# JohnVinyard/music-synthesis

Hardware: AMD Instinct MI355X
Metric: GAN train-step audio samples/sec (22.05 kHz, 8192-sample window) (higher is better)
Workload: dtype f32 storage and accumulate; multiplies on the 16-bit matrix pipe with split fp32 operands: block-scaled fp16 x 2 (22 significand bits, 3 products per multiply) in the atoms, the k5 layer, the grouped convs, the stride-8 transposed forward and the atom weight gradients; exact bf16 x 3 (6 products) or; 1 GPU; stage-2 GAN train step: alternating D/G trainer calls, MelGAN generator + 3-scale discriminator + feature-matching loss (BASELINE.json configs[2]); per_gpu_batch=32, global_batch=32, window=8192, mels=80, optimizer=FlatAdam(1e-4,(0.5,0.9)), parallelism=dp1, hipgraph=True

## Files before the change

### include/msynth.h

```cpp
#ifndef MSYNTH_H
#define MSYNTH_H

#include <stddef.h>
#include <stdint.h>

#ifdef __cplusplus
extern "C" {
#endif

#define MSYNTH_VERSION 200

typedef void* ms_stream_t;

enum ms_status {
    MS_OK = 0,
    MS_ERR_INVALID_ARG = -1,
    MS_ERR_UNSUPPORTED = -2,
    MS_ERR_WORKSPACE = -3,
    MS_ERR_LAUNCH = -4,
    MS_ERR_COMM = -5
};

enum ms_act { MS_ACT_NONE = 0, MS_ACT_LRELU = 1, MS_ACT_TANH = 2 };
enum ms_pad_mode { MS_PAD_ZERO = 0, MS_PAD_REFLECT = 1 };

int ms_version(void);
const char* ms_status_string(int status);

typedef struct ms_conv1d_desc {
    int32_t B, Cin, Lin, Cout, K, stride, pad, dil, groups;
    int32_t pad_mode;
    int32_t act;
    float slope;
    int32_t in_act;
} ms_conv1d_desc;

int ms_conv1d_out_len(const ms_conv1d_desc* d);

int ms_conv1d_fwd(const ms_conv1d_desc* d, const float* x, const float* w, const float* bias,
                  const float* residual, float* y, float* y_act, void* workspace,
                  size_t workspace_bytes, ms_stream_t stream);

int ms_conv1d_bwd_data(const ms_conv1d_desc* d, const float* gy, const float* y_act,
                       const float* w, const float* gx_add, float* gx, void* workspace,
                       size_t workspace_bytes, ms_stream_t stream);

int ms_conv1d_bwd_weight(const ms_conv1d_desc* d, const float* x, const float* gy,
                         const float* y_act, float* gw, float* gb, float beta, void* workspace,
                         size_t workspace_bytes, ms_stream_t stream);

#define MS_CONV_PARTS_MAX 3
typedef struct ms_conv1d_parts {
    int32_t count;
    int32_t reserved;
    int32_t B[MS_CONV_PARTS_MAX];
    int32_t Lin[MS_CONV_PARTS_MAX];
    const float* x[MS_CONV_PARTS_MAX];
    float* y[MS_CONV_PARTS_MAX];
    const float* gy[MS_CONV_PARTS_MAX];
    const float* y_act[MS_CONV_PARTS_MAX];
    const float* gx_add[MS_CONV_PARTS_MAX];
    float* gx[MS_CONV_PARTS_MAX];
} ms_conv1d_parts;
int ms_conv1d_parts_launches(const ms_conv1d_desc* d, const ms_conv1d_parts* parts, int which, int with_image);
size_t ms_conv1d_parts_workspace_bytes(const ms_conv1d_desc* d, const ms_conv1d_parts* parts, int which, int with_image);
int ms_conv1d_parts_fwd(const ms_conv1d_desc* d, const ms_conv1d_parts* parts, const float* w, const float* bias,
                        const void* image, void* workspace, size_t workspace_bytes, ms_stream_t stream);
int ms_conv1d_parts_bwd_data(const ms_conv1d_desc* d, const ms_conv1d_parts* parts, const float* w, const void* image_bwd,
                             void* workspace, size_t workspace_bytes, ms_stream_t stream);
int ms_conv1d_parts_bwd_weight(const ms_conv1d_desc* d, const ms_conv1d_parts* parts, float* gw, float* gb, float beta,
                               void* workspace, size_t workspace_bytes, ms_stream_t stream);

#define MS_WGRAD_MULTI_MAX 8
typedef struct ms_wgrad_multi_desc {
    int32_t count;
    int32_t reserved;
    ms_conv1d_desc conv[MS_WGRAD_MULTI_MAX];
    const float* x[MS_WGRAD_MULTI_MAX];
    const float* gy[MS_WGRAD_MULTI_MAX];
    const float* y_act[MS_WGRAD_MULTI_MAX];
    float* gw[MS_WGRAD_MULTI_MAX];
    float* gb[MS_WGRAD_MULTI_MAX];
    float beta[MS_WGRAD_MULTI_MAX];
    const float* xmax[MS_WGRAD_MULTI_MAX];
    const float* gmax[MS_WGRAD_MULTI_MAX];
    const uint16_t* y_signs[MS_WGRAD_MULTI_MAX];
} ms_wgrad_multi_desc;
size_t ms_conv1d_bwd_weight_multi_workspace_bytes(const ms_wgrad_multi_desc* d);
int ms_conv1d_bwd_weight_multi(const ms_wgrad_multi_desc* d, void* workspace, size_t workspace_bytes,
                               ms_stream_t stream);

typedef struct ms_atom_desc {
    int32_t B, C, L, dil;
    float slope;
} ms_atom_desc;
#define MS_ATOM_PACK_MAX 16
typedef struct ms_atom_pack_desc {
    int32_t count;
    int32_t reserved;
    int32_t C[MS_ATOM_PACK_MAX];
    const float* w0[MS_ATOM_PACK_MAX];
    const float* w1[MS_ATOM_PACK_MAX];
    void* image[MS_ATOM_PACK_MAX];
    int32_t backward[MS_ATOM_PACK_MAX];
} ms_atom_pack_desc;
size_t ms_residual_atom_image_bytes(int32_t C);
int ms_residual_atom_supported(const ms_atom_desc* d);
int ms_residual_atom_pack_multi(const ms_atom_pack_desc* d, ms_stream_t stream);
#define MS_ATOM_AMAX_N 1024
int ms_residual_atom_publishes_amax(void);
int ms_residual_atom_fwd(const ms_atom_desc* d, const float* x, const void* image, const float* b0, const float* b1,
                         float* y, float* t, float* y_act, float* amax, ms_stream_t stream);
int ms_residual_atom_bwd_supported(const ms_atom_desc* d);
int ms_residual_atom_bwd_data(const ms_atom_desc* d, const float* gy, const float* y_act, const float* t,
                              const void* image_bwd, float* gt, float* gx, float* amax, ms_stream_t stream);
// ... 225 lines not shown
```

### music-synthesis_amd/csrc/api.hip

```cpp
#include "ms_common.h"
#include <stdarg.h>
#include <stdio.h>
#include <stdlib.h>
#include <string.h>
#include <execinfo.h>
#include <signal.h>
#include <unistd.h>
#include "conv_mfma.h"
#include "gconv_mfma.h"
#include "conv_thin.h"

static thread_local int g_prof_on = 0, g_prof_launches = 0, g_prof_products = 0;
static thread_local double g_prof_us = 0.0;
static thread_local char g_prof_kernel[MS_PROFILE_NAME_MAX] = "";

void ms_note_kernel(int products, const char* fmt, ...) {
    if (!g_prof_on) return;
    va_list ap;
    va_start(ap, fmt);
    vsnprintf(g_prof_kernel, sizeof(g_prof_kernel), fmt, ap);
    va_end(ap);
    g_prof_products = products;
}

bool ms_name_or_note(char* name, int products, const char* fmt, ...) {
    if (!name && !g_prof_on) return false;
    va_list ap;
    va_start(ap, fmt);
    vsnprintf(name ? name : g_prof_kernel, MS_PROFILE_NAME_MAX, fmt, ap);
    va_end(ap);
    if (!name) g_prof_products = products;
    return name != nullptr;
}

bool ms_prof_on() { return g_prof_on != 0; }

void ms_prof_add(hipEvent_t e0, hipEvent_t e1) {
    float ms = 0.f;
    if (e0 && e1 && hipEventSynchronize(e1) == hipSuccess && hipEventElapsedTime(&ms, e0, e1) == hipSuccess) {
        g_prof_us += 1e3 * (double)ms;
        ++g_prof_launches;
    }
    if (e0) (void)hipEventDestroy(e0);
    if (e1) (void)hipEventDestroy(e1);
}

namespace {

bool make_conv(const ms_conv1d_desc* d, ConvP* p) {
    if (!d) return false;
    if (d->B <= 0 || d->Cin <= 0 || d->Lin <= 0 || d->Cout <= 0 || d->K <= 0 || d->stride <= 0 ||
        d->pad < 0 || d->dil <= 0 || d->groups <= 0)
        return false;
    if (d->Cin % d->groups || d->Cout % d->groups) return false;
    if (d->pad_mode != MS_PAD_ZERO && d->pad_mode != MS_PAD_REFLECT) return false;
    if (d->pad_mode == MS_PAD_REFLECT && d->pad >= d->Lin) return false;
    if (d->act < MS_ACT_NONE || d->act > MS_ACT_TANH) return false;
    const int eff = d->Lin + 2 * d->pad - d->dil * (d->K - 1) - 1;
    if (eff < 0) return false;
    p->B = d->B; p->Cin = d->Cin; p->Lin = d->Lin; p->Cout = d->Cout; p->K = d->K;
    p->stride = d->stride; p->pad = d->pad; p->dil = d->dil; p->groups = d->groups;
    p->Cg = d->Cin / d->groups; p->Og = d->Cout / d->groups;
// ... 275 lines not shown
            q.act = p.act;
            return pl.add(TD_CONV_MFMA, q, ws);
        }
        return pl.add(TD_CONV_DIRECT, q);
    }
    const size_t tail = msk_channel_sum_ws(p.Cin) + 32;
    if (mst_convt1_applicable(p)) pl.add(TW_THIN, p, mst_convt1_wgrad_ws(p) + tail, SHORT_WS);
    if (mswt8_applicable(p)) pl.add(TW_8, p, mswt8_ws(p) + tail, SHORT_WS | UNSUPPORTED);
    if (mswt2s_applicable(p)) pl.add(TW_2S, p, mswt2s_ws(p) + tail, SHORT_WS | UNSUPPORTED);
    if (msm_convt_bwd_applicable(p)) return pl.add(TW_MFMA, p, msm_convt_bwd_weight_ws(p) + tail);
    if (msm_bwd_weight_applicable(p)) return pl.add(TW_CONV_MFMA, p, msm_bwd_weight_ws(p) + tail);
    return pl.add(TW_CONV_DIRECT, p, msk_conv1d_bwd_weight_ws(p) + tail);
}

bool parts_ok(const ms_conv1d_desc* d, const ms_conv1d_parts* parts, ConvP* c) {
    if (!d || !parts || parts->count < 1 || parts->count > MS_CONV_PARTS_MAX) return false;
    ms_conv1d_desc d0 = *d;
    for (int i = 0; i < parts->count; ++i) {
        d0.B = parts->B[i]; d0.Lin = parts->Lin[i];
        ConvP p;
        if (!make_conv(&d0, &p)) return false;
        if (i == 0) *c = p;
    }
    return true;
}

ms_conv1d_desc part_desc(const ms_conv1d_desc* d, const ms_conv1d_parts* parts, int i) {
    ms_conv1d_desc di = *d;
    di.B = parts->B[i]; di.Lin = parts->Lin[i];
    return di;
}

Plan parts_plan(const ms_conv1d_desc* d, const ConvP& c, const ms_conv1d_parts* parts, int which, bool w, bool image) {
    Plan pl;
    if (parts->count >= 2 && !c.in_act) {
        if (w && msd_parts_applicable(c, parts, which))
            return pl.add(P_DISC, c, which == 2 ? msd_parts_bwd_weight_ws(c, parts) : 0);
        if (w && msg4_parts_applicable(c, parts)) return pl.add(P_G4, c);
        if (which == 2 && msw5_parts_applicable(c, parts)) return pl.add(P_K5, c, msw5_parts_ws(c, parts));
        if (which < 2 && image && ms5_parts_applicable(c, parts, which == 1))
            return pl.add(P_K5_IMG, c, ms5_parts_ws(c, parts, which == 1));
        if (which == 0 && w && msg3_parts_fwd_applicable(c, parts)) return pl.add(P_G3, c);
        if (which == 1 && w && msg3_parts_bwd_data_applicable(c, parts)) return pl.add(P_G3, c);
        if (which == 2 && msg3_parts_bwd_weight_applicable(c, parts)) return pl.add(P_G3, c, msg3_parts_bwd_weight_ws(c, parts));
    }
    size_t n = 0;
    for (int i = 0; i < parts->count; ++i) {
        const ms_conv1d_desc di = part_desc(d, parts, i);
        const size_t m = image && which < 2 && ms_conv1d_img_bytes(&di) ? ms_conv1d_img_workspace_bytes(&di, which)
                                                                        : ms_conv1d_workspace_bytes(&di, which);
        if (m > n) n = m;
    }
    return pl.add(P_EACH, c, n);
}

const char* route_name(Kind k, const ConvP& g) {
    switch (k) {
        case F_THIN_SHORT: case F_THIN: return mst_fwd_name(g);
        case F_SMALL: return mss_conv_name(g);
        case F_PAD4: case F_MFMA: return msm_fwd_name(g);
        case TD_CONV_MFMA: { ConvP c = g; c.act = MS_ACT_NONE; return msm_fwd_name(c, g.act); }
        case F_G4: return msg4_parts_name(0);
        case F_G3: return msg3_fwd_name(g);
        case F_G: return msg_fwd_name(g);
        case F_DIRECT: case TD_CONV_DIRECT: return msk_conv1d_fwd_direct_name(g);
        case D_PAD4: case D_MFMA: return msm_bwd_data_name(g);
        case D_G4: return msg4_parts_name(1);
        case D_G3: return msg3_bwd_data_name(g);
        case D_G: return msg_bwd_data_name(g);
        case D_THIN: return mst_bwd_data_name(g);
        case D_DIRECT: case TF_DIRECT: return msk_conv1d_bwd_data_direct_name(g);
        case W_THIN: return mst_bwd_weight_name(g);
        case W_SHORT: return msws_name(g);
        case W_32: return msw32_name(g);
        case W_K5: return msw5_name(g);
        case W_ROWS: return msw_bwd_weight_name(g);
        case W_MFMA: case TW_CONV_MFMA: return msm_bwd_weight_name(g);
        case W_G4: return msg4_parts_name(2);
        case W_G3: return msg3_bwd_weight_name(g);
        case W_G: return msg_bwd_weight_name(g);
        case W_DIRECT: case TW_CONV_DIRECT: return msk_conv1d_bwd_weight_direct_name(g);
        case TF_THIN: return mst_convt1_fwd_name();
        case TF_LANES: return mss_convt_name(g.stride);
        case TF_MFMA: return msm_convt_fwd_name(g);
        case TD_MFMA: return msm_convt_bwd_data_name(g);
        case TW_THIN: return mst_convt1_wgrad_name();
        case TW_8: return mswt8_name(g);
        case TW_2S: return mswt2s_name(g);
        case TW_MFMA: return msm_convt_bwd_weight_name(g);
        default: return "";
    }
}

template <class Launch>
int run(const Plan& pl, const void* ws, size_t ws_bytes, Launch launch) {
    for (int i = 0; i < pl.n; ++i) {
        const Route& r = pl.r[i];
        if ((r.declines & SHORT_WS) && (!ws || ws_bytes < r.ws)) continue;
        if ((r.declines & ALIGNED_WS) && (((uintptr_t)ws) & 15)) continue;
        if (ms_prof_on()) ms_note_kernel(0, "%s", route_name(r.kind, r.g));
        const int rc = launch(r.kind, r.g);
        if (rc != MS_ERR_UNSUPPORTED || !(r.declines & UNSUPPORTED)) return rc;
    }
    return MS_ERR_UNSUPPORTED;
}

// ... 68 lines not shown
    });
    if (rc != MS_OK || p.pad_mode != MS_PAD_REFLECT) return rc;
    p.pad_mode = MS_PAD_ZERO;
    return msk_reflect_fold_bwd(p, gy, y_act, w, gx, s);
}

int ms_conv1d_bwd_weight(const ms_conv1d_desc* d, const float* x, const float* gy,
                         const float* y_act, float* gw, float* gb, float beta, void* workspace,
                         size_t workspace_bytes, ms_stream_t stream) {
    ConvP p;
    if (!make_conv(d, &p) || !x || !gy || !gw) return MS_ERR_INVALID_ARG;
    if (beta != 0.f && beta != 1.f) return MS_ERR_INVALID_ARG;
    hipStream_t s = (hipStream_t)stream;
    const float* xa = p.in_act ? x : nullptr;
    const int xk = p.in_act ? MS_MOD_LRELU_FWD : 0;
    return run(conv_plan(p, 2, false, false), workspace, workspace_bytes, [&](Kind k, const ConvP& g) {
        switch (k) {
            case W_THIN: return mst_conv1d_bwd_weight(g, x, gy, y_act, gw, gb, beta, workspace, workspace_bytes, s);
            case W_SHORT: return msws_bwd_weight(g, x, gy, y_act, gw, gb, beta, workspace, workspace_bytes, s);
            case W_32: return msw32_bwd_weight(g, x, gy, y_act, gw, gb, beta, workspace, workspace_bytes, s);
            case W_K5: return msw5_bwd_weight(g, x, gy, y_act, gw, gb, beta, workspace, workspace_bytes, s);
            case W_ROWS: return msw_conv1d_bwd_weight(g, x, gy, y_act, gw, gb, beta, workspace, workspace_bytes, s);
            case W_MFMA:
                return msm_conv1d_bwd_weight(g, x, xa, xk, gy, y_act, g.act, gw, gb, beta, workspace, workspace_bytes, s);
            case W_G4: {
                const ms_conv1d_parts q = one_part(g, x, nullptr, gy, y_act);
                return msg4_parts_bwd_weight(g, &q, gw, gb, beta, s);
            }
            case W_G3: return msg3_conv1d_bwd_weight(g, x, gy, y_act, gw, gb, beta, workspace, workspace_bytes, s);
            case W_G: return msg_conv1d_bwd_weight(g, x, gy, y_act, gw, gb, beta, workspace, workspace_bytes, s);
            default:
                return msk_conv1d_bwd_weight_direct(g, x, xa, xk, gy, y_act, g.act, gw, gb, beta, workspace, workspace_bytes, s);
        }
    });
}

size_t ms_conv1d_workspace_bytes(const ms_conv1d_desc* d, int which) {
    ConvP p;
    if (!make_conv(d, &p) || which < 0 || which > 2) return 0;
    const size_t a = conv_plan(p, which, false, false).ws(), b = conv_plan(p, which, true, true).ws();
    return a > b ? a : b;
}

const char* ms_conv1d_kernel_name(const ms_conv1d_desc* d, int which) {
    ConvP p;
    if (!make_conv(d, &p) || which < 0 || which > 2) return "";
    const Plan pl = conv_plan(p, which, false, false);
    return pl.n ? route_name(pl.r[0].kind, pl.r[0].g) : "";
}

int ms_conv1d_parts_launches(const ms_conv1d_desc* d, const ms_conv1d_parts* parts, int which, int with_image) {
    ConvP c;
    if (!parts_ok(d, parts, &c) || which < 0 || which > 2) return MS_ERR_INVALID_ARG;
    return parts_plan(d, c, parts, which, true, with_image != 0).r[0].kind == P_EACH ? parts->count : 1;
}

size_t ms_conv1d_parts_workspace_bytes(const ms_conv1d_desc* d, const ms_conv1d_parts* parts, int which, int with_image) {
    ConvP c;
    if (!parts_ok(d, parts, &c) || which < 0 || which > 2) return 0;
    return parts_plan(d, c, parts, which, true, with_image != 0).ws();
}

int ms_conv1d_parts_fwd(const ms_conv1d_desc* d, const ms_conv1d_parts* parts, const float* w, const float* bias,
                        const void* image, void* workspace, size_t workspace_bytes, ms_stream_t stream) {
    ConvP c;
    if (!parts_ok(d, parts, &c) || (!w && !image)) return MS_ERR_INVALID_ARG;
    hipStream_t s = (hipStream_t)stream;
    return run(parts_plan(d, c, parts, 0, w, image), workspace, workspace_bytes, [&](Kind k, const ConvP&) {
        switch (k) {
            case P_DISC: return msd_parts_fwd(c, parts, w, bias, s);
            case P_G4: return msg4_parts_fwd(c, parts, w, bias, s);
            case P_K5_IMG: return ms5_parts_fwd(c, parts, image, bias, workspace, workspace_bytes, s);
            case P_G3: return msg3_parts_fwd(c, parts, w, bias, s);
            default: break;
        }
        for (int i = 0; i < parts->count; ++i) {
            const ms_conv1d_desc di = part_desc(d, parts, i);
            int rc = MS_ERR_UNSUPPORTED;
            if (image && ms_conv1d_img_bytes(&di))
                rc = ms_conv1d_img_fwd(&di, parts->x[i], image, bias, parts->y[i], workspace, workspace_bytes, stream);
            else if (w)
                rc = ms_conv1d_fwd(&di, parts->x[i], w, bias, nullptr, parts->y[i], nullptr, workspace, workspace_bytes, stream);
            if (rc != MS_OK) return rc;
        }
        return (int)MS_OK;
    });
}

int ms_conv1d_parts_bwd_data(const ms_conv1d_desc* d, const ms_conv1d_parts* parts, const float* w, const void* image_bwd,
                             void* workspace, size_t workspace_bytes, ms_stream_t stream) {
    ConvP c;
    if (!parts_ok(d, parts, &c) || (!w && !image_bwd)) return MS_ERR_INVALID_ARG;
    hipStream_t s = (hipStream_t)stream;
    return run(parts_plan(d, c, parts, 1, w, image_bwd), workspace, workspace_bytes, [&](Kind k, const ConvP&) {
        switch (k) {
            case P_DISC: return msd_parts_bwd_data(c, parts, w, s);
            case P_G4: return msg4_parts_bwd_data(c, parts, w, s);
            case P_K5_IMG: return ms5_parts_bwd_data(c, parts, image_bwd, workspace, workspace_bytes, s);
            case P_G3: return msg3_parts_bwd_data(c, parts, w, s);
            default: break;
        }
        for (int i = 0; i < parts->count; ++i) {
            const ms_conv1d_desc di = part_desc(d, parts, i);
            const float* ya = d->act == MS_ACT_NONE ? nullptr : parts->y_act[i];
            int rc = MS_ERR_UNSUPPORTED;
            if (image_bwd && ms_conv1d_img_bytes(&di))
                rc = ms_conv1d_img_bwd_data(&di, parts->gy[i], ya, image_bwd, parts->gx_add[i], parts->gx[i], workspace,
                                            workspace_bytes, stream);
            else if (w)
                rc = ms_conv1d_bwd_data(&di, parts->gy[i], ya, w, parts->gx_add[i], parts->gx[i], workspace, workspace_bytes,
                                        stream);
            if (rc != MS_OK) return rc;
        }
        return (int)MS_OK;
    });
}

int ms_conv1d_parts_bwd_weight(const ms_conv1d_desc* d, const ms_conv1d_parts* parts, float* gw, float* gb, float beta,
                               void* workspace, size_t workspace_bytes, ms_stream_t stream) {
    ConvP c;
    if (!parts_ok(d, parts, &c) || !gw || (beta != 0.f && beta != 1.f)) return MS_ERR_INVALID_ARG;
    hipStream_t s = (hipStream_t)stream;
    return run(parts_plan(d, c, parts, 2, true, false), workspace, workspace_bytes, [&](Kind k, const ConvP&) {
        switch (k) {
            case P_DISC: return msd_parts_bwd_weight(c, parts, gw, gb, beta, workspace, workspace_bytes, s);
            case P_G4: return msg4_parts_bwd_weight(c, parts, gw, gb, beta, s);
            case P_K5: return msw5_parts_bwd_weight(c, parts, gw, gb, beta, workspace, workspace_bytes, s);
            case P_G3: return msg3_parts_bwd_weight(c, parts, gw, gb, beta, workspace, workspace_bytes, s);
            default: break;
        }
        for (int i = 0; i < parts->count; ++i) {
            const ms_conv1d_desc di = part_desc(d, parts, i);
            const float* ya = d->act == MS_ACT_NONE ? nullptr : parts->y_act[i];
            const int rc = ms_conv1d_bwd_weight(&di, parts->x[i], parts->gy[i], ya, gw, gb, i == 0 ? beta : 1.f, workspace,
                                                workspace_bytes, stream);
            if (rc != MS_OK) return rc;
        }
        return (int)MS_OK;
    });
}

static int multi_convs(const ms_wgrad_multi_desc* d, ConvP* cs) {
    if (!d || d->count <= 0 || d->count > MS_WGRAD_MULTI_MAX) return 0;
    for (int i = 0; i < d->count; ++i)
        if (!make_conv(&d->conv[i], &cs[i])) return 0;
    return d->count;
}

size_t ms_conv1d_bwd_weight_multi_workspace_bytes(const ms_wgrad_multi_desc* d) {
    ConvP cs[MS_WGRAD_MULTI_MAX];
    const int n = multi_convs(d, cs);
    size_t need = n ? msw_multi_ws(cs, n) : 0;
    if (n && msw32_multi_ws(cs, n) > need) need = msw32_multi_ws(cs, n);
    for (int i = 0; i < n; ++i) {
        const size_t one = ms_conv1d_workspace_bytes(&d->conv[i], 2);
        if (one > need) need = one;
    }
    return need;
}

int ms_conv1d_bwd_weight_multi(const ms_wgrad_multi_desc* d, void* workspace, size_t workspace_bytes,
                               ms_stream_t stream) {
    ConvP cs[MS_WGRAD_MULTI_MAX];
    const int n = multi_convs(d, cs);
    if (!n) return MS_ERR_INVALID_ARG;
    for (int i = 0; i < n; ++i)
        if (!d->x[i] || !d->gy[i] || !d->gw[i] || (d->beta[i] != 0.f && d->beta[i] != 1.f)) return MS_ERR_INVALID_ARG;
    int nsig = 0;
    for (int i = 0; i < n; ++i) nsig += d->y_signs[i] ? 1 : 0;
    if (nsig != 0 && nsig != n) return MS_ERR_INVALID_ARG;
    const float* ya[MS_WGRAD_MULTI_MAX];
    for (int i = 0; i < n; ++i) ya[i] = nsig ? reinterpret_cast<const float*>(d->y_signs[i]) : d->y_act[i];
    int rc = msw_conv1d_bwd_weight_multi(cs, n, d->x, d->gy, ya, d->gw, d->gb, d->beta, d->xmax, d->gmax, nsig ? 1 : 0, workspace,
                                         workspace_bytes, (hipStream_t)stream);
    if (rc != MS_ERR_UNSUPPORTED) return rc;
    rc = msw32_bwd_weight_multi(cs, n, d->x, d->gy, ya, d->gw, d->gb, d->beta, nsig ? 1 : 0, workspace, workspace_bytes,
// ... 109 lines not shown
```

### music-synthesis_amd/csrc/disc_parts.hip

```cpp
#include "operand_split.h"
#include "gconv_mfma.h"
#include <stdint.h>
#include <stdlib.h>

namespace {

constexpr int NP = MS_CONV_PARTS_MAX;

struct DParts {
    int count, wg0[NP + 1];
    int B[NP], L[NP], tiles[NP];
    const float* a[NP];
    const float* b[NP];
    const float* c[NP];
    float* o[NP];
};

struct DPart {
    int B, L, tiles, wg;
    const float* a;
    const float* b;
    const float* c;
    float* o;
};
__device__ __forceinline__ DPart pick_part(const DParts& q, int wg) {
    DPart p{q.B[0], q.L[0], q.tiles[0], wg, q.a[0], q.b[0], q.c[0], q.o[0]};
#pragma unroll
    for (int k = 1; k < NP; ++k)
        if (k < q.count && wg >= q.wg0[k]) p = DPart{q.B[k], q.L[k], q.tiles[k], wg - q.wg0[k], q.a[k], q.b[k], q.c[k], q.o[k]};
    return p;
}

__device__ __forceinline__ float lrelu_grad(float g, float y, float slope) { return y > 0.f ? g : g * slope; }

constexpr int FK = 15, FPAD = 7, FC = 16, FT = 1024;

__device__ __forceinline__ void stage_thin_window(float* xs, const float* x, int B, int L, int b, int tile_t) {
    const auto rs = __builtin_amdgcn_make_buffer_rsrc(const_cast<float*>(x), 0, 4u * (unsigned)(B * L), 0x00020000);
    for (int i = threadIdx.x; i < (FT + 16) / 4; i += 256) {
        const int t = tile_t - 8 + 4 * i;
        *reinterpret_cast<f32x4*>(xs + 4 * i) = load_row4(rs, (unsigned)(b * L), t, L);
    }
    __syncthreads();
}

__global__ __launch_bounds__(256) void k_dfirst_fwd(DParts q, const float* __restrict__ w, const float* __restrict__ bias,
                                                   float slope) {
    __shared__ __attribute__((aligned(16))) float xs[FT + 16];
    const DPart p = pick_part(q, blockIdx.x);
    const int b = p.wg / p.tiles, tile_t = (p.wg - b * p.tiles) * FT;
    stage_thin_window(xs, p.a, p.B, p.L, b, tile_t);
    const int t0 = tile_t + 4 * threadIdx.x;
    if (t0 >= p.L) return;
    float win[20];
#pragma unroll
    for (int i = 0; i < 5; ++i) {
        const f32x4 v = *reinterpret_cast<const f32x4*>(xs + 4 * threadIdx.x + 4 * i);
        win[4 * i] = v[0]; win[4 * i + 1] = v[1]; win[4 * i + 2] = v[2]; win[4 * i + 3] = v[3];
    }
    const bool whole = t0 + 3 < p.L;
#pragma unroll 4
    for (int co = 0; co < FC; ++co) {
        float v[4];
        const float bv = bias ? bias[co] : 0.f;
#pragma unroll
        for (int e = 0; e < 4; ++e) v[e] = bv;
#pragma unroll
        for (int k = 0; k < FK; ++k) {
            const float wk = w[co * FK + k];
#pragma unroll
            for (int e = 0; e < 4; ++e) v[e] = fmaf(wk, win[1 + e + k], v[e]);
        }
#pragma unroll
        for (int e = 0; e < 4; ++e) v[e] = fmaxf(v[e], v[e] * slope);
        float* yr = p.o + ((size_t)b * FC + co) * p.L + t0;
        if (whole) {
            *reinterpret_cast<f32x4u*>(yr) = (f32x4u){v[0], v[1], v[2], v[3]};
        } else {
#pragma unroll
            for (int e = 0; e < 4; ++e)
                if (t0 + e < p.L) yr[e] = v[e];
        }
    }
}

__global__ __launch_bounds__(256) void k_dfirst_bwd_data(DParts q, const float* __restrict__ w, float slope) {
    __shared__ float red[4][256 + 4];
    const DPart p = pick_part(q, blockIdx.x);
    const int lane = threadIdx.x & 63, wid = threadIdx.x >> 6;
    const int b = p.wg / p.tiles, tile_t = (p.wg - b * p.tiles) * 256;
    const int t0 = tile_t + 4 * lane;
    const unsigned bytes = 4u * (unsigned)(p.B * FC * p.L);
    const auto rsG = __builtin_amdgcn_make_buffer_rsrc(const_cast<float*>(p.a), 0, bytes, 0x00020000);
    const auto rsY = __builtin_amdgcn_make_buffer_rsrc(const_cast<float*>(p.b), 0, bytes, 0x00020000);
    float acc[4] = {0.f, 0.f, 0.f, 0.f};
#pragma unroll
    for (int cc = 0; cc < 4; ++cc) {
        const int co = wid * 4 + cc;
        const unsigned row = (unsigned)((b * FC + co) * p.L);
        float win[20];
#pragma unroll
        for (int i = 0; i < 5; ++i) {
            const f32x4 g = load_row4(rsG, row, t0 - 8 + 4 * i, p.L);
            const f32x4 y = load_row4(rsY, row, t0 - 8 + 4 * i, p.L);
#pragma unroll
            for (int e = 0; e < 4; ++e) win[4 * i + e] = lrelu_grad(g[e], y[e], slope);
        }
#pragma unroll
        for (int k = 0; k < FK; ++k) {
            const float wk = w[co * FK + k];
#pragma unroll
            for (int e = 0; e < 4; ++e) acc[e] = fmaf(wk, win[8 + e + FPAD - k], acc[e]);
        }
    }
#pragma unroll
    for (int e = 0; e < 4; ++e) red[wid][4 * lane + e] = acc[e];
    __syncthreads();
    const int to = tile_t + threadIdx.x;
    if (to < p.L) {
        const int i = threadIdx.x;
        float v = (red[0][i] + red[1][i]) + (red[2][i] + red[3][i]);
        if (p.c) v += p.c[(size_t)b * p.L + to];
        p.o[(size_t)b * p.L + to] = v;
    }
}

__global__ __launch_bounds__(256) void k_dfirst_wgrad(DParts q, float slope, float* __restrict__ partial) {
    __shared__ __attribute__((aligned(16))) float xs[FT + 16];
    const int lane = threadIdx.x & 63, wid = threadIdx.x >> 6;
    float acc[4][FK], bsum[4];
#pragma unroll
    for (int cc = 0; cc < 4; ++cc) {
        bsum[cc] = 0.f;
#pragma unroll
        for (int k = 0; k < FK; ++k) acc[cc][k] = 0.f;
    }
    const int nunits = q.wg0[q.count];
    for (int unit = blockIdx.x; unit < nunits; unit += gridDim.x) {
        const DPart p = pick_part(q, unit);
        const int b = p.wg / p.tiles, tile_t = (p.wg - b * p.tiles) * FT;
        __syncthreads();
        stage_thin_window(xs, p.a, p.B, p.L, b, tile_t);
        const unsigned bytes = 4u * (unsigned)(p.B * FC * p.L);
        const auto rsG = __builtin_amdgcn_make_buffer_rsrc(const_cast<float*>(p.b), 0, bytes, 0x00020000);
        const auto rsY = __builtin_amdgcn_make_buffer_rsrc(const_cast<float*>(p.c), 0, bytes, 0x00020000);
#pragma unroll 1
        for (int pass = 0; pass < FT / 256; ++pass) {
            const int sl = pass * 256 + 4 * lane, t0 = tile_t + sl;
            if (tile_t + pass * 256 >= p.L) break;
            float win[20];
#pragma unroll
            for (int i = 0; i < 5; ++i) {
                const f32x4 v = *reinterpret_cast<const f32x4*>(xs + sl + 4 * i);
                win[4 * i] = v[0]; win[4 * i + 1] = v[1]; win[4 * i + 2] = v[2]; win[4 * i + 3] = v[3];
            }
            f32x4 g[4], y[4];
#pragma unroll
            for (int cc = 0; cc < 4; ++cc) {
                const unsigned row = (unsigned)((b * FC + wid * 4 + cc) * p.L);
                g[cc] = load_row4(rsG, row, t0, p.L);
                y[cc] = load_row4(rsY, row, t0, p.L);
            }
#pragma unroll
            for (int cc = 0; cc < 4; ++cc)
#pragma unroll
                for (int e = 0; e < 4; ++e) {
                    const float v = lrelu_grad(g[cc][e], y[cc][e], slope);
                    bsum[cc] += v;
#pragma unroll
                    for (int k = 0; k < FK; ++k) acc[cc][k] = fmaf(v, win[1 + e + k], acc[cc][k]);
                }
        }
    }
    float* prow = partial + (size_t)blockIdx.x * (FC * FK + FC);
#pragma unroll
    for (int cc = 0; cc < 4; ++cc) {
        const int co = wid * 4 + cc;
#pragma unroll
        for (int k = 0; k < FK; ++k) {
            const float r = ms_wave_sum(acc[cc][k]);
            if (lane == 0) prow[co * FK + k] = r;
        }
        const float r = ms_wave_sum(bsum[cc]);
        if (lane == 0) prow[FC * FK + co] = r;
    }
}

__global__ __launch_bounds__(256) void k_dparts_reduce(const float* __restrict__ partial, int nslabs, int stride, int nw,
                                                      int nb, float* __restrict__ gw, float* __restrict__ gb, float beta) {
    const int lane = threadIdx.x & 63, i = blockIdx.x * 4 + (threadIdx.x >> 6);
    if (i >= nw + nb) return;
    float s = 0.f;
    for (int z = lane; z < nslabs; z += 64) s += partial[(size_t)z * stride + i];
    s = ms_wave_sum(s);
    if (lane == 0 && (i < nw || gb)) {
        float* dst = i < nw ? gw + i : gb + (i - nw);
        *dst = (beta != 0.f ? beta * *dst : 0.f) + s;
    }
}

constexpr int JL = 32, JP = 33;

__device__ __forceinline__ void stage_rows(float* lds, const float* __restrict__ src, int L) {
    const int nv = 64 * L;
    const float invL = 1.f / (float)L;
    for (int v = threadIdx.x; v < nv; v += 256) {
        const f32x4 x = *reinterpret_cast<const f32x4*>(src + 4 * v);
        int r = (int)(((float)(4 * v) + 0.5f) * invL);
        int t = 4 * v - r * L;
#pragma unroll
        for (int e = 0; e < 4; ++e) {
            lds[r * JP + t] = x[e];
            if (++t == L) { t = 0; ++r; }
        }
    }
}

__global__ __launch_bounds__(256) void k_djudge_fwd(DParts q, int C, const float* __restrict__ w, const float* __restrict__ bias) {
    __shared__ __attribute__((aligned(16))) float rows[256 * JP];
    __shared__ float red[4][JL];
    const DPart p = pick_part(q, blockIdx.x);
    const int b = p.wg, L = p.L, tid = threadIdx.x, lane = tid & 63, wid = tid >> 6;
    float acc[JL];
#pragma unroll
    for (int t = 0; t < JL; ++t) acc[t] = 0.f;
    for (int c0 = 0; c0 < C; c0 += 256) {
        __syncthreads();
        stage_rows(rows, p.a + ((size_t)b * C + c0) * L, L);
        __syncthreads();
        const float w0 = w[(c0 + tid) * 3], w1 = w[(c0 + tid) * 3 + 1], w2 = w[(c0 + tid) * 3 + 2];
        float v[JL + 2];
        v[0] = 0.f;
#pragma unroll
        for (int t = 0; t < JL; ++t) v[t + 1] = t < L ? rows[tid * JP + t] : 0.f;
        v[JL + 1] = 0.f;
#pragma unroll
        for (int t = 0; t < JL; ++t) acc[t] = fmaf(w2, v[t + 2], fmaf(w1, v[t + 1], fmaf(w0, v[t], acc[t])));
    }
// ... 39 lines not shown
    __shared__ float gj[JL + 2];
    __shared__ float red[4];
    const int chunks = C / 256, tid = threadIdx.x;
    const int chunk = blockIdx.x % chunks, slab = blockIdx.x / chunks;
    const int c0 = chunk * 256;
    float a0 = 0.f, a1 = 0.f, a2 = 0.f, bs = 0.f;
    const int nrows = q.wg0[q.count];
    for (int row = slab; row < nrows; row += nslabs) {
        const DPart p = pick_part(q, row);
        const int b = p.wg, L = p.L;
        __syncthreads();
        stage_rows(rows, p.a + ((size_t)b * C + c0) * L, L);
        if (tid < JL + 2) {
            const int t = tid - 1;
            gj[tid] = (t >= 0 && t < L) ? p.b[(size_t)b * L + t] : 0.f;
        }
        __syncthreads();
        for (int t = 0; t < L; ++t) {
            const float x = rows[tid * JP + t];
            a0 = fmaf(x, gj[t + 2], a0);
            a1 = fmaf(x, gj[t + 1], a1);
            a2 = fmaf(x, gj[t], a2);
        }
        if (chunk == 0 && tid < L) bs += gj[tid + 1];
    }
    float* prow = partial + (size_t)slab * (C * 3 + 1);
    prow[(c0 + tid) * 3] = a0; prow[(c0 + tid) * 3 + 1] = a1; prow[(c0 + tid) * 3 + 2] = a2;
    if (chunk == 0) {
        const float tot = ms_block_sum(bs, red);
        if (tid == 0) prow[C * 3] = tot;
    }
}

bool is_first(const ConvP& c) {
    return c.groups == 1 && c.stride == 1 && c.dil == 1 && c.pad_mode == MS_PAD_ZERO && !c.in_act && c.Cin == 1 && c.Cout == FC &&
           c.K == FK && c.pad == FPAD && c.act == MS_ACT_LRELU && c.slope >= 0.f && c.slope <= 1.f;
}
bool is_judge(const ConvP& c) {
    return c.groups == 1 && c.stride == 1 && c.dil == 1 && c.pad_mode == MS_PAD_ZERO && !c.in_act && c.Cout == 1 && c.K == 3 &&
           c.pad == 1 && c.act == MS_ACT_NONE && c.Cin % 256 == 0 && c.Cin >= 256 && c.Cin <= 4096;
}

bool table(const ConvP& c, const ms_conv1d_parts* parts, int tile, int chan, DParts* q) {
    if (!parts || parts->count < 1 || parts->count > NP) return false;
    q->count = parts->count;
    q->wg0[0] = 0;
    for (int i = 0; i < NP; ++i) {
        const bool on = i < parts->count;
        if (on && (parts->B[i] <= 0 || parts->Lin[i] <= 0)) return false;
        if (on && (long long)parts->B[i] * chan * parts->Lin[i] * 4 >= (1ll << 31)) return false;
        q->B[i] = on ? parts->B[i] : 0; q->L[i] = on ? parts->Lin[i] : 1;
        q->tiles[i] = on ? (tile ? ms_ceil_div(parts->Lin[i], tile) : 1) : 1;
        q->wg0[i + 1] = q->wg0[i] + q->B[i] * q->tiles[i];
        q->a[i] = q->b[i] = q->c[i] = nullptr; q->o[i] = nullptr;
    }
    return true;
}

constexpr int FIRST_WGS = 512;
constexpr int JUDGE_SLABS = 48;

}

bool msd_parts_applicable(const ConvP& c, const ms_conv1d_parts* parts, int which) {
    if (!ms_switch_on("MSYNTH_DTHIN")) return false;
    if (!parts || parts->count < 1 || parts->count > NP) return false;
    if (is_first(c)) return true;
    if (!is_judge(c)) return false;
    for (int i = 0; i < parts->count; ++i) {
        if (parts->Lin[i] > JL) return false;
        const uintptr_t a = which == 1 ? (uintptr_t)parts->gx[i] | (uintptr_t)parts->gx_add[i] : (uintptr_t)parts->x[i];
        if (a & 15) return false;
    }
    return true;
}

size_t msd_parts_bwd_weight_ws(const ConvP& c, const ms_conv1d_parts* parts) {
    (void)parts;
    if (is_first(c)) return (size_t)FIRST_WGS * (FC * FK + FC) * sizeof(float);
    return (size_t)JUDGE_SLABS * (c.Cin * 3 + 1) * sizeof(float);
}

int msd_parts_fwd(const ConvP& c, const ms_conv1d_parts* parts, const float* w, const float* bias, hipStream_t s) {
    DParts q;
    const bool first = is_first(c);
    if (!table(c, parts, first ? FT : 0, first ? FC : c.Cin, &q)) return MS_ERR_INVALID_ARG;
    for (int i = 0; i < q.count; ++i) {
        if (!parts->x[i] || !parts->y[i]) return MS_ERR_INVALID_ARG;
        q.a[i] = parts->x[i]; q.o[i] = parts->y[i];
    }
    if (first) {
        ms_note_kernel(0, "k_dfirst_fwd");
        hipLaunchKernelGGL(k_dfirst_fwd, dim3(q.wg0[q.count]), dim3(256), 0, s, q, w, bias, c.slope);
    } else {
        ms_note_kernel(0, "k_djudge_fwd");
        hipLaunchKernelGGL(k_djudge_fwd, dim3(q.wg0[q.count]), dim3(256), 0, s, q, c.Cin, w, bias);
    }
    MS_CHECK_LAUNCH();
    return MS_OK;
}

int msd_parts_bwd_data(const ConvP& c, const ms_conv1d_parts* parts, const float* w, hipStream_t s) {
    DParts q;
    const bool first = is_first(c);
    if (!table(c, parts, first ? 256 : 0, first ? FC : c.Cin, &q)) return MS_ERR_INVALID_ARG;
    for (int i = 0; i < q.count; ++i) {
        if (!parts->gy[i] || !parts->gx[i] || (first && !parts->y_act[i])) return MS_ERR_INVALID_ARG;
        q.a[i] = parts->gy[i]; q.b[i] = parts->y_act[i]; q.c[i] = parts->gx_add[i]; q.o[i] = parts->gx[i];
    }
    if (first) {
        ms_note_kernel(0, "k_dfirst_bwd_data");
        hipLaunchKernelGGL(k_dfirst_bwd_data, dim3(q.wg0[q.count]), dim3(256), 0, s, q, w, c.slope);
    } else {
        const int chunks = c.Cin / 256;
        for (int i = 0; i < NP; ++i) q.wg0[i + 1] = q.wg0[i] + q.B[i] * chunks;
        ms_note_kernel(0, "k_djudge_bwd_data");
        hipLaunchKernelGGL(k_djudge_bwd_data, dim3(q.wg0[q.count]), dim3(256), 0, s, q, c.Cin, w);
    }
    MS_CHECK_LAUNCH();
    return MS_OK;
}

int msd_parts_bwd_weight(const ConvP& c, const ms_conv1d_parts* parts, float* gw, float* gb, float beta, void* ws,
                         size_t ws_bytes, hipStream_t s) {
    DParts q;
    const bool first = is_first(c);
    if (!ws || ws_bytes < msd_parts_bwd_weight_ws(c, parts)) return MS_ERR_WORKSPACE;
    if (!table(c, parts, first ? FT : 0, first ? FC : c.Cin, &q)) return MS_ERR_INVALID_ARG;
    float* partial = (float*)ws;
    if (first) {
        for (int i = 0; i < q.count; ++i) {
            if (!parts->x[i] || !parts->gy[i] || !parts->y_act[i]) return MS_ERR_INVALID_ARG;
            q.a[i] = parts->x[i]; q.b[i] = parts->gy[i]; q.c[i] = parts->y_act[i];
        }
        const int units = q.wg0[q.count];
        const int grid = units < FIRST_WGS ? units : FIRST_WGS;
        ms_note_kernel(0, "k_dfirst_wgrad");
        hipLaunchKernelGGL(k_dfirst_wgrad, dim3(grid), dim3(256), 0, s, q, c.slope, partial);
        MS_CHECK_LAUNCH();
        const int nw = FC * FK, nb = FC;
        hipLaunchKernelGGL(k_dparts_reduce, dim3(ms_ceil_div(nw + nb, 4)), dim3(256), 0, s, partial, grid, nw + nb, nw, nb, gw, gb,
                           beta);
    } else {
        for (int i = 0; i < q.count; ++i) {
            if (!parts->x[i] || !parts->gy[i]) return MS_ERR_INVALID_ARG;
            q.a[i] = parts->x[i]; q.b[i] = parts->gy[i];
        }
        const int rows = q.wg0[q.count], chunks = c.Cin / 256;
        const int slabs = rows < JUDGE_SLABS ? rows : JUDGE_SLABS;
        ms_note_kernel(0, "k_djudge_wgrad");
        hipLaunchKernelGGL(k_djudge_wgrad, dim3(slabs * chunks), dim3(256), 0, s, q, c.Cin, slabs, partial);
        MS_CHECK_LAUNCH();
        const int nw = c.Cin * 3, nb = 1;
        hipLaunchKernelGGL(k_dparts_reduce, dim3(ms_ceil_div(nw + nb, 4)), dim3(256), 0, s, partial, slabs, nw + nb, nw, nb, gw, gb,
                           beta);
    }
    MS_CHECK_LAUNCH();
    return MS_OK;
}
```

### music-synthesis_amd/csrc/gconv_mfma.h

```cpp
#pragma once
#include "ms_common.h"

bool msg_fwd_applicable(const ConvP& p);
const char* msg_fwd_name(const ConvP& p);
int msg_conv1d_fwd(const ConvP& p, const float* x, const float* w, const float* bias, float* y,
                   hipStream_t s);

bool msg_bwd_data_applicable(const ConvP& p);
const char* msg_bwd_data_name(const ConvP& p);
int msg_conv1d_bwd_data(const ConvP& p, const float* gy, const float* y_act, const float* w,
                        const float* gx_add, float* gx, hipStream_t s);

bool msg_bwd_weight_applicable(const ConvP& p);
size_t msg_bwd_weight_ws(const ConvP& p);
const char* msg_bwd_weight_name(const ConvP& p);
int msg_conv1d_bwd_weight(const ConvP& p, const float* x, const float* gy, const float* y_act,
                          float* gw, float* gb, float beta, void* ws, size_t ws_bytes, hipStream_t s);
int msg_wgrad_gridx(const ConvP& p);
int msg_reduce_slabs(const ConvP& p, const float* partial, size_t stride, int nslabs, float* gw, float* gb,
                     float beta, hipStream_t s);

bool msg3_fwd_applicable(const ConvP& p);
const char* msg3_fwd_name(const ConvP& p);
int msg3_conv1d_fwd(const ConvP& p, const float* x, const float* w, const float* bias, float* y,
                    hipStream_t s);
const char* msg3_bwd_weight_name(const ConvP& p);
bool msg3_bwd_weight_applicable(const ConvP& p);
int msg3_conv1d_bwd_weight(const ConvP& p, const float* x, const float* gy, const float* y_act,
                           float* gw, float* gb, float beta, void* ws, size_t ws_bytes, hipStream_t s);
bool msg3_bwd_data_applicable(const ConvP& p);
const char* msg3_bwd_data_name(const ConvP& p);
int msg3_conv1d_bwd_data(const ConvP& p, const float* gy, const float* y_act, const float* w,
                         const float* gx_add, float* gx, hipStream_t s);

bool msg3_parts_fwd_applicable(const ConvP& c, const ms_conv1d_parts* parts);
int msg3_parts_fwd(const ConvP& c, const ms_conv1d_parts* parts, const float* w, const float* bias, hipStream_t s);
bool msg3_parts_bwd_data_applicable(const ConvP& c, const ms_conv1d_parts* parts);
int msg3_parts_bwd_data(const ConvP& c, const ms_conv1d_parts* parts, const float* w, hipStream_t s);
bool msg3_parts_bwd_weight_applicable(const ConvP& c, const ms_conv1d_parts* parts);
size_t msg3_parts_bwd_weight_ws(const ConvP& c, const ms_conv1d_parts* parts);
int msg3_parts_bwd_weight(const ConvP& c, const ms_conv1d_parts* parts, float* gw, float* gb, float beta, void* ws,
                          size_t ws_bytes, hipStream_t s);
bool ms5_parts_applicable(const ConvP& c, const ms_conv1d_parts* parts, bool backward);
size_t ms5_parts_ws(const ConvP& c, const ms_conv1d_parts* parts, bool backward);
int ms5_parts_fwd(const ConvP& c, const ms_conv1d_parts* parts, const void* image, const float* bias, void* ws, size_t ws_bytes,
                  hipStream_t s);
int ms5_parts_bwd_data(const ConvP& c, const ms_conv1d_parts* parts, const void* image_bwd, void* ws, size_t ws_bytes,
                       hipStream_t s);
bool msw5_parts_applicable(const ConvP& c, const ms_conv1d_parts* parts);
size_t msw5_parts_ws(const ConvP& c, const ms_conv1d_parts* parts);
int msw5_parts_bwd_weight(const ConvP& c, const ms_conv1d_parts* parts, float* gw, float* gb, float beta, void* ws,
                          size_t ws_bytes, hipStream_t s);
bool msd_parts_applicable(const ConvP& c, const ms_conv1d_parts* parts, int which);
size_t msd_parts_bwd_weight_ws(const ConvP& c, const ms_conv1d_parts* parts);
int msd_parts_fwd(const ConvP& c, const ms_conv1d_parts* parts, const float* w, const float* bias, hipStream_t s);
int msd_parts_bwd_data(const ConvP& c, const ms_conv1d_parts* parts, const float* w, hipStream_t s);
int msd_parts_bwd_weight(const ConvP& c, const ms_conv1d_parts* parts, float* gw, float* gb, float beta, void* ws,
                         size_t ws_bytes, hipStream_t s);
bool msg4_parts_applicable(const ConvP& c, const ms_conv1d_parts* parts);
const char* msg4_parts_name(int which);
int msg4_parts_fwd(const ConvP& c, const ms_conv1d_parts* parts, const float* w, const float* bias, hipStream_t s);
int msg4_parts_bwd_data(const ConvP& c, const ms_conv1d_parts* parts, const float* w, hipStream_t s);
int msg4_parts_bwd_weight(const ConvP& c, const ms_conv1d_parts* parts, float* gw, float* gb, float beta, hipStream_t s);
```

### music-synthesis_amd/csrc/gconv_split.hip

```cpp
#include "operand_split.h"
#include "gconv_mfma.h"
#include <stdint.h>
#include <stdlib.h>

namespace {

constexpr int GK = 41, GS = 4, GCG = 4;

__device__ __forceinline__ float wave_max_dpp(float m) {
    m = fmaxf(m, __builtin_bit_cast(float, __builtin_amdgcn_update_dpp(0, __builtin_bit_cast(int, m), 0xB1, 0xF, 0xF, true)));
    m = fmaxf(m, __builtin_bit_cast(float, __builtin_amdgcn_update_dpp(0, __builtin_bit_cast(int, m), 0x4E, 0xF, 0xF, true)));
    m = fmaxf(m, __builtin_bit_cast(float, __builtin_amdgcn_update_dpp(0, __builtin_bit_cast(int, m), 0x141, 0xF, 0xF, true)));
    m = fmaxf(m, __builtin_bit_cast(float, __builtin_amdgcn_update_dpp(0, __builtin_bit_cast(int, m), 0x140, 0xF, 0xF, true)));
    const int b = __builtin_bit_cast(int, m);
    const float r0 = __builtin_bit_cast(float, __builtin_amdgcn_readlane(b, 0)), r1 = __builtin_bit_cast(float, __builtin_amdgcn_readlane(b, 16));
    const float r2 = __builtin_bit_cast(float, __builtin_amdgcn_readlane(b, 32)), r3 = __builtin_bit_cast(float, __builtin_amdgcn_readlane(b, 48));
    return fmaxf(fmaxf(r0, r1), fmaxf(r2, r3));
}
constexpr int NG = 6;

template <int RB>
struct GF {
    static constexpr int NR = 16 / RB;
    static constexpr int TS = 64 / RB;
    static constexpr int SUBP = NR + 3;
    static constexpr int NQR = 4 * SUBP;
    static constexpr int RP = RB == 1 ? 80 : (RB == 2 ? 56 : 28);
    static constexpr int ROWS = 4 * RB;
    static constexpr int PIECE_BYTES = ROWS * RP * 8;
    static constexpr int WAVE_BYTES = 2 * PIECE_BYTES;
    static constexpr int NIT = (ROWS * NQR + 63) / 64;
    static_assert(NQR <= RP, "row pitch");
    static_assert(NQR < RP || (ROWS * NQR) % 64 == 0, "a spare quad for the lanes without an item");
};

extern __shared__ __attribute__((aligned(16))) unsigned char g3_smem[];

template <int RB, bool VEC, bool VOUT>
__device__ __forceinline__ void gconv_fwd_body(const ConvP& p, int spr, int nseg, int nunits,
                                               const float* __restrict__ x,
                                               const float* __restrict__ w,
                                               const float* __restrict__ bias,
                                               float* __restrict__ y, int bx, int nbx) {
    using C = GF<RB>;
    unsigned char* const lds = g3_smem;
    const int tid = threadIdx.x, lane = tid & 63, wid = tid >> 6;
    const int g = blockIdx.y;
    const int n = lane & 15, kg = lane >> 4;
    const int sgl = n / C::NR, np = n % C::NR;
    const unsigned wv_off = wid * C::WAVE_BYTES;
    const unsigned lw = (unsigned)(uintptr_t)lds + wv_off;
    const unsigned rb0 = lw + ((kg * RB + sgl) * C::RP + np) * 8;

    int it_lds[C::NIT];
    unsigned it_x[C::NIT];
    int it_qs[C::NIT];
    unsigned it_c[C::NIT];
#pragma unroll
    for (int i = 0; i < C::NIT; ++i) {
        const int idx = lane + 64 * i;
        const int row = idx / C::NQR, Q = idx - row * C::NQR;
        const int sg = row >> 2, ci = row & 3;
        const bool act = row < C::ROWS;
        it_lds[i] = act ? ((ci * RB + sg) * C::RP + (Q & 3) * C::SUBP + (Q >> 2)) * 8 : C::NQR * 8;
        it_x[i] = (unsigned)(ci * p.Lin);
        it_qs[i] = act ? 4 * Q + sg : -4;
        it_c[i] = act ? (unsigned)(ci * p.Lin + 4 * Q) * 4u : 0xF0000000u;
    }
    const int wstride = nbx * 4;
    const int sstride = wstride * RB;
    const int dsb = sstride / spr, dst = sstride - dsb * spr;
    struct Cur { int seg, b, ts; };
    auto advance = [&](Cur& c) {
        c.seg += sstride; c.b += dsb; c.ts += dst;
        if (c.ts >= spr) { c.ts -= spr; ++c.b; }
    };

    const auto rsX = __builtin_amdgcn_make_buffer_rsrc(const_cast<float*>(x), 0, 4u * (unsigned)(p.B * p.Cin * p.Lin), 0x00020000);
    auto gload = [&](auto& xr, const Cur& c) {
        if (RB == 1) {
            const int s0 = c.ts * (C::TS * GS) - p.pad;
            if (c.seg < nseg && s0 >= 0 && s0 + 4 * C::NQR <= p.Lin) {
                const unsigned ub = (unsigned)__builtin_amdgcn_readfirstlane(((c.b * p.Cin + g * GCG) * p.Lin + s0) * 4);
#pragma unroll
                for (int i = 0; i < C::NIT; ++i)
                    xr[i] = __builtin_bit_cast(f32x4, __builtin_amdgcn_raw_buffer_load_b128(rsX, it_c[i], ub, 0));
                return;
            }
        }
#pragma unroll
        for (int i = 0; i < C::NIT; ++i) {
            const int sg = RB == 1 ? 0 : (it_qs[i] & 3), Q4 = it_qs[i] & ~3;
            int ts = c.ts + sg, b = c.b;
            if (spr == 1) { b += ts; ts = 0; }
            else if (ts >= spr) { ts -= spr; ++b; }
            const bool segok = c.seg + sg < nseg && it_qs[i] >= 0;
// ... 77 lines not shown
    _Pragma("unroll") for (int par = 0; par < 2; ++par) {                                                       \
        const int c0 = 2 * (H_) + par, c1 = c0 + 1;                                                             \
        _Pragma("unroll") for (int pc = 0; pc < 2; ++pc)                                                        \
            asm volatile("ds_read2_b64 %0, %1 offset0:%2 offset1:%3"                                            \
                         : "=v"(f[buf][par][pc])                                                                \
                         : "v"(rbo[pc]), "n"((c0 & 3) * C::SUBP + (c0 >> 2)), "n"((c1 & 3) * C::SUBP + (c1 >> 2))); \
    }
        MS_G3_READ(0, 0);
#pragma unroll
        for (int H = 0; H <= NG; ++H) {
            const int cur = H & 1;
            if (H < NG) {
                MS_G3_READ(H + 1, cur ^ 1);
                asm volatile("s_waitcnt lgkmcnt(4)"
                             : "+v"(f[cur][0][0]), "+v"(f[cur][0][1]), "+v"(f[cur][1][0]), "+v"(f[cur][1][1]));
            } else {
                asm volatile("s_waitcnt lgkmcnt(0)"
                             : "+v"(f[cur][0][0]), "+v"(f[cur][0][1]), "+v"(f[cur][1][0]), "+v"(f[cur][1][1]));
            }
            const f16x8 f0h = __builtin_bit_cast(f16x8, f[cur][0][0]), f0l = __builtin_bit_cast(f16x8, f[cur][0][1]);
            const f16x8 f1h = __builtin_bit_cast(f16x8, f[cur][1][0]), f1l = __builtin_bit_cast(f16x8, f[cur][1][1]);
            if (H < NG) {
                acc[0] = __builtin_amdgcn_mfma_f32_16x16x32_f16(A[H][0], f0l, acc[0], 0, 0, 0);
                acc[1] = __builtin_amdgcn_mfma_f32_16x16x32_f16(A[H][0], f1l, acc[1], 0, 0, 0);
            }
            if (H >= 1) {
                acc[2] = __builtin_amdgcn_mfma_f32_16x16x32_f16(A[H - 1][0], f0l, acc[2], 0, 0, 0);
                acc[3] = __builtin_amdgcn_mfma_f32_16x16x32_f16(A[H - 1][0], f1l, acc[3], 0, 0, 0);
            }
            if (H < NG) {
                acc[0] = __builtin_amdgcn_mfma_f32_16x16x32_f16(A[H][0], f0h, acc[0], 0, 0, 0);
                acc[1] = __builtin_amdgcn_mfma_f32_16x16x32_f16(A[H][0], f1h, acc[1], 0, 0, 0);
            }
            if (H >= 1) {
                acc[2] = __builtin_amdgcn_mfma_f32_16x16x32_f16(A[H - 1][0], f0h, acc[2], 0, 0, 0);
                acc[3] = __builtin_amdgcn_mfma_f32_16x16x32_f16(A[H - 1][0], f1h, acc[3], 0, 0, 0);
            }
            if (H < NG) {
                acc[0] = __builtin_amdgcn_mfma_f32_16x16x32_f16(A[H][1], f0h, acc[0], 0, 0, 0);
                acc[1] = __builtin_amdgcn_mfma_f32_16x16x32_f16(A[H][1], f1h, acc[1], 0, 0, 0);
            }
            if (H >= 1) {
                acc[2] = __builtin_amdgcn_mfma_f32_16x16x32_f16(A[H - 1][1], f0h, acc[2], 0, 0, 0);
                acc[3] = __builtin_amdgcn_mfma_f32_16x16x32_f16(A[H - 1][1], f1h, acc[3], 0, 0, 0);
            }
        }
#undef MS_G3_READ

        int ets = ep.ts + sgl, eb = ep.b;
        if (spr == 1) { eb += ets; ets = 0; }
        else if (ets >= spr) { ets -= spr; ++eb; }
        const bool eok = ep.seg + sgl < nseg;
        const int t = ets * C::TS + 4 * np;
        if (eok && t < p.Lout) {
            float* yr = y + ((size_t)eb * p.Cout + (size_t)g * p.Og + kg * 4) * p.Lout + t;
#pragma unroll
            for (int r = 0; r < 4; ++r) {
                if (!rok[r]) continue;
                float v[4];
#pragma unroll
                for (int s = 0; s < 4; ++s) {
                    const float pre = fmaf(acc[s][r], kscale, bq[r]);
                    v[s] = fmaxf(pre, pre * eslope);
                }
                if (VOUT) {
                    *reinterpret_cast<float4*>(yr + (size_t)r * p.Lout) = make_float4(v[0], v[1], v[2], v[3]);
                } else if (t + 3 < p.Lout) {
                    *reinterpret_cast<f32x4u*>(yr + (size_t)r * p.Lout) = (f32x4u){v[0], v[1], v[2], v[3]};
                } else {
#pragma unroll
                    for (int s = 0; s < 4; ++s)
                        if (t + s < p.Lout) yr[(size_t)r * p.Lout + s] = v[s];
                }
            }
        }
        advance(ep);
    };

    for (; unit < nunits; unit += wstride) {
        float um = 0.f;
#pragma unroll
        for (int i = 0; i < C::NIT; ++i)
#pragma unroll
            for (int e = 0; e < 4; ++e) um = fmaxf(um, fabsf(xp[i][e]));
        float S, invS;
        block_scale(wave_max_dpp(um), S, invS);
#pragma unroll
        for (int i = 0; i < C::NIT; ++i) stage_item(xp[i], it_lds[i], S);
        __builtin_amdgcn_fence(__ATOMIC_RELEASE, "wavefront");
        __builtin_amdgcn_wave_barrier();
        if (unit + wstride < nunits) gload(xp, ld);
        advance(ld);
        unit_mfma_store(invS * iWS);
        __builtin_amdgcn_fence(__ATOMIC_ACQ_REL, "wavefront");
        __builtin_amdgcn_wave_barrier();
    }
}

template <int RB, bool VEC, bool VOUT>
__global__ __launch_bounds__(256, 2) void k_gconv_split_fwd(ConvP p, int spr, int nseg, int nunits,
                                                           const float* __restrict__ x,
                                                           const float* __restrict__ w,
                                                           const float* __restrict__ bias,
                                                           float* __restrict__ y) {
    gconv_fwd_body<RB, VEC, VOUT>(p, spr, nseg, nunits, x, w, bias, y, blockIdx.x, gridDim.x);
}

struct G3Parts {
    ConvP p;
    int count, bx0[MS_CONV_PARTS_MAX + 1];
    int B[MS_CONV_PARTS_MAX], Lin[MS_CONV_PARTS_MAX], Lout[MS_CONV_PARTS_MAX];
    int u0[MS_CONV_PARTS_MAX], u1[MS_CONV_PARTS_MAX], u2[MS_CONV_PARTS_MAX];
    const float* a[MS_CONV_PARTS_MAX];
    const float* b[MS_CONV_PARTS_MAX];
    const float* c[MS_CONV_PARTS_MAX];
    float* o[MS_CONV_PARTS_MAX];
};

__device__ __forceinline__ int g3_part_of(const G3Parts& q, int bx) {
    int i = 0;
#pragma unroll
    for (int k = 1; k < MS_CONV_PARTS_MAX; ++k)
        if (k < q.count && bx >= q.bx0[k]) i = k;
    return __builtin_amdgcn_readfirstlane(i);
}

__device__ __forceinline__ ConvP g3_part_conv(const G3Parts& q, int i) {
    ConvP p = q.p;
    p.B = q.B[i]; p.Lin = q.Lin[i]; p.Lout = q.Lout[i];
    return p;
}

template <int RB0, int RB1, int RB2>
__global__ __launch_bounds__(256, 2) void k_gconv_split_fwd_parts(G3Parts q, const float* __restrict__ w,
                                                                 const float* __restrict__ bias) {
    const int bx = blockIdx.x, i = g3_part_of(q, bx);
    const ConvP p = g3_part_conv(q, i);
    const int rbx = bx - q.bx0[i], nbx = q.bx0[i + 1] - q.bx0[i];
    if (i == 0) gconv_fwd_body<RB0, true, true>(p, q.u0[0], q.u1[0], q.u2[0], q.a[0], w, bias, q.o[0], rbx, nbx);
    else if (i == 1) gconv_fwd_body<RB1, false, false>(p, q.u0[1], q.u1[1], q.u2[1], q.a[1], w, bias, q.o[1], rbx, nbx);
    else gconv_fwd_body<RB2, false, false>(p, q.u0[2], q.u1[2], q.u2[2], q.a[2], w, bias, q.o[2], rbx, nbx);
}

constexpr int WU = 64;
constexpr int WXQ = 75;
constexpr int WXROW = 608;
constexpr int WX_PIECE = GCG * WXROW;
constexpr int WG_PIECE = 8 * 16 * 16;
constexpr int W_WAVE = 3 * (WG_PIECE + WX_PIECE);
constexpr int WNP = 2;
constexpr int NKT = 3;

template <bool VEC>
__device__ __forceinline__ void gconv_wgrad_body(const ConvP& p, const float* __restrict__ x,
                                                 const float* __restrict__ gy,
                                                 const float* __restrict__ y_act,
                                                 float* __restrict__ partial, size_t partial_stride, int bx, int nbx, int slab) {
    unsigned char* const lds = g3_smem;
    const int tid = threadIdx.x, lane = tid & 63, wid = tid >> 6;
    const int g = blockIdx.y;
    const int kind = y_act ? p.act : MS_ACT_NONE;
    unsigned char* gimg = lds + wid * W_WAVE;
    unsigned char* ximg = gimg + WNP * WG_PIECE;

    const int tq = lane & 15, co0 = lane >> 4;
    const int g_tb = tq >> 1;
    int x_lds[5];
    unsigned x_c[5];
#pragma unroll
    for (int i = 0; i < 5; ++i) {
        const int idx = lane + 64 * i;
        const int ci = idx / WXQ, Q = idx - ci * WXQ;
        const bool act = ci < GCG;
        x_lds[i] = act ? ci * WXROW + Q * 8 : 3 * WXROW + WXQ * 8;
        x_c[i] = act ? (unsigned)(ci * p.Lin + 4 * Q) : 0x3C000000u;
    }
    const unsigned g_bytes = 4u * (unsigned)(p.B * p.Cout * p.Lout);
    const auto rsX = __builtin_amdgcn_make_buffer_rsrc(const_cast<float*>(x), 0, 4u * (unsigned)(p.B * p.Cin * p.Lin), 0x00020000);
    const auto rsG = __builtin_amdgcn_make_buffer_rsrc(const_cast<float*>(gy), 0, g_bytes, 0x00020000);
    const auto rsA = __builtin_amdgcn_make_buffer_rsrc(const_cast<float*>(y_act ? y_act : gy), 0, g_bytes, 0x00020000);

    const int tiles = (p.Lout + WU - 1) / WU;
    const int nunits = p.B * tiles;
    const int ustride = nbx * 4;
    const int db = ustride / tiles, dt = ustride - db * tiles;

    unsigned g_c[4];
#pragma unroll
    for (int i = 0; i < 4; ++i) g_c[i] = co0 + 4 * i < p.Og ? (unsigned)((co0 + 4 * i) * p.Lout + 4 * tq) * 4u : OOB;
    f32x4 gv[4], ga[4], xv[5];
    auto gload = [&](int b, int ti) {
        const int t0 = ti * WU, u0 = t0 * GS - p.pad;
        const unsigned gbase = (unsigned)((b * p.Cout + g * p.Og) * p.Lout + t0);
        const unsigned xbase = (unsigned)((b * p.Cin + g * GCG) * p.Lin);
        if (t0 + WU <= p.Lout && u0 >= 0 && u0 + 4 * WXQ <= p.Lin) {
            const unsigned gs = (unsigned)__builtin_amdgcn_readfirstlane((int)(gbase * 4u));
            const unsigned xs = (unsigned)__builtin_amdgcn_readfirstlane((int)((xbase + (unsigned)u0) * 4u));
#pragma unroll
            for (int i = 0; i < 4; ++i) {
                gv[i] = __builtin_bit_cast(f32x4, __builtin_amdgcn_raw_buffer_load_b128(rsG, g_c[i], gs, 0));
                ga[i] = __builtin_bit_cast(f32x4, __builtin_amdgcn_raw_buffer_load_b128(rsA, g_c[i], gs, 0));
            }
#pragma unroll
            for (int i = 0; i < 5; ++i)
                xv[i] = __builtin_bit_cast(f32x4, __builtin_amdgcn_raw_buffer_load_b128(
                                                      rsX, x_c[i] < 0x3C000000u ? x_c[i] * 4u : OOB, xs, 0));
            return;
        }
#pragma unroll
        for (int i = 0; i < 4; ++i) {
            const int co = co0 + 4 * i;
            const unsigned off = gbase + (unsigned)(co * p.Lout + 4 * tq);
            if (VEC) {
                const bool ok = co < p.Og && t0 + 4 * tq < p.Lout;
                const unsigned vo = ok ? off * 4u : OOB;
                gv[i] = __builtin_bit_cast(f32x4, __builtin_amdgcn_raw_buffer_load_b128(rsG, vo, 0, 0));
                ga[i] = __builtin_bit_cast(f32x4, __builtin_amdgcn_raw_buffer_load_b128(rsA, vo, 0, 0));
            } else {
                const bool ok = co < p.Og && t0 + 4 * tq < p.Lout;
                const unsigned vo = ok ? off * 4u : OOB;
                gv[i] = __builtin_bit_cast(f32x4, __builtin_amdgcn_raw_buffer_load_b128(rsG, vo, 0, 0));
                ga[i] = __builtin_bit_cast(f32x4, __builtin_amdgcn_raw_buffer_load_b128(rsA, vo, 0, 0));
#pragma unroll
                for (int e = 1; e < 4; ++e)
                    if (t0 + 4 * tq + e >= p.Lout) { gv[i][e] = 0.f; ga[i][e] = 0.f; }
            }
        }
#pragma unroll
        for (int i = 0; i < 5; ++i) {
            const int Q4 = 4 * ((lane + 64 * i) % WXQ);
            const int sidx = u0 + Q4;
            if (VEC) {
                const bool ok = x_c[i] < 0x3C000000u && sidx >= 0 && sidx < p.Lin;
                xv[i] = __builtin_bit_cast(f32x4, __builtin_amdgcn_raw_buffer_load_b128(
                                                      rsX, ok ? (xbase + x_c[i] + (unsigned)u0) * 4u : OOB, 0, 0));
            } else {
                const bool ok = x_c[i] < 0x3C000000u && sidx >= 0 && sidx < p.Lin;
                xv[i] = __builtin_bit_cast(f32x4, __builtin_amdgcn_raw_buffer_load_b128(
                                                      rsX, ok ? (xbase + x_c[i] + (unsigned)u0) * 4u : OOB, 0, 0));
#pragma unroll
                for (int e = 1; e < 4; ++e) xv[i][e] = sidx + e < p.Lin ? xv[i][e] : 0.f;
            }
        }
    };

    f32x4 acc[GCG][NKT];
#pragma unroll
    for (int c = 0; c < GCG; ++c)
#pragma unroll
        for (int j = 0; j < NKT; ++j) acc[c][j] = (f32x4){0.f, 0.f, 0.f, 0.f};
    float Sg = 0.f, Sx = 0.f;
    float Sg_lo = 0.f, Sx_lo = 0.f;
    float bsum[4] = {0.f, 0.f, 0.f, 0.f};

    const int m = lane & 15, kg = lane >> 4;
    const unsigned char* a_rd0 = gimg + (kg * 16 + (m ^ kg)) * 16;
    const unsigned char* a_rd1 = gimg + 1024 + (kg * 16 + (m ^ kg ^ 4)) * 16;
    const unsigned b_rd = (unsigned)(uintptr_t)ximg + 64 * kg + 8 * ((lane & 15) >> 2) + 8 * (lane & 3);

    int unit = bx * 4 + wid;
    int b = unit / tiles, ti = unit - b * tiles;
    if (unit < nunits) gload(b, ti);
    for (; unit < nunits; unit += ustride) {
        {
            float mg = 0.f, mx = 0.f;
#pragma unroll
            for (int i = 0; i < 4; ++i)
#pragma unroll
                for (int k = 0; k < 4; ++k) mg = fmaxf(mg, fabsf(gv[i][k]));
#pragma unroll
            for (int i = 0; i < 5; ++i)
#pragma unroll
                for (int k = 0; k < 4; ++k) mx = fmaxf(mx, fabsf(xv[i][k]));
            mg = wave_max_dpp(mg); mx = wave_max_dpp(mx);
            float nSg = Sg, nSx = Sx, inv;
            if (mg > 0.f && !(mg * Sg >= 256.f && mg * Sg < 32768.f)) block_scale(mg * 4.f, nSg, inv);
            if (mx > 0.f && !(mx * Sx >= 256.f && mx * Sx < 32768.f)) block_scale(mx * 4.f, nSx, inv);
            if (nSg == 0.f) nSg = 1.f;
            if (nSx == 0.f) nSx = 1.f;
            if (Sg_lo != 0.f) nSg = fminf(nSg, Sg_lo * 0x1p30f);
            if (Sx_lo != 0.f) nSx = fminf(nSx, Sx_lo * 0x1p30f);
            if (mg > 0.f) Sg_lo = Sg_lo == 0.f ? nSg : fminf(Sg_lo, nSg);
            if (mx > 0.f) Sx_lo = Sx_lo == 0.f ? nSx : fminf(Sx_lo, nSx);
            if ((nSg != Sg || nSx != Sx) && Sg != 0.f) {
                const float ratio = (nSg / Sg) * (nSx / Sx);
#pragma unroll
                for (int c = 0; c < GCG; ++c)
#pragma unroll
                    for (int j = 0; j < NKT; ++j) acc[c][j] *= ratio;
            }
            Sg = nSg; Sx = nSx;
        }
#pragma unroll
        for (int i = 0; i < 4; ++i) {
            float e[4];
#pragma unroll
            for (int k = 0; k < 4; ++k) e[k] = ms_act_grad(gv[i][k], ga[i][k], kind, p.slope);
            bsum[i] += (e[0] + e[1]) + (e[2] + e[3]);
            unsigned h0, l0, h1, l1;
            split_pair(e[0] * Sg, e[1] * Sg, h0, l0);
            split_pair(e[2] * Sg, e[3] * Sg, h1, l1);
            unsigned char* d = gimg + (g_tb * 16 + ((co0 + 4 * i) ^ g_tb)) * 16 + (tq & 1) * 8;
            *reinterpret_cast<uint2*>(d) = make_uint2(h0, h1);
            *reinterpret_cast<uint2*>(d + WG_PIECE) = make_uint2(l0, l1);
        }
#pragma unroll
        for (int i = 0; i < 5; ++i) {
            unsigned h0, l0, h1, l1;
            split_pair(xv[i][0] * Sx, xv[i][1] * Sx, h0, l0);
            split_pair(xv[i][2] * Sx, xv[i][3] * Sx, h1, l1);
            unsigned char* d = ximg + x_lds[i];
            *reinterpret_cast<uint2*>(d) = make_uint2(h0, h1);
            *reinterpret_cast<uint2*>(d + WX_PIECE) = make_uint2(l0, l1);
        }
        __builtin_amdgcn_fence(__ATOMIC_RELEASE, "wavefront");
        __builtin_amdgcn_wave_barrier();
        const int tvalid = min(WU, p.Lout - ti * WU);
        int nb = b + db, nti = ti + dt;
        if (nti >= tiles) { nti -= tiles; ++nb; }
        if (unit + ustride < nunits) gload(nb, nti);

        const int niter = tvalid > 32 ? 2 * GCG : GCG;
        f16x8 A[2][WNP];
#pragma unroll
        for (int step = 0; step < 2; ++step)
#pragma unroll
            for (int pc = 0; pc < WNP; ++pc)
                A[step][pc] = *reinterpret_cast<const f16x8*>((step ? a_rd1 : a_rd0) + pc * WG_PIECE);
        u32x2 Bl[2][WNP][NKT], Bh[2][WNP][NKT];
#define MS_W3_READ(it_, pc)                                                                                   \
    _Pragma("unroll") for (int j = 0; j < NKT; ++j) {                                                         \
        asm volatile("ds_read_b64_tr_b16 %0, %1 offset:%2"                                                    \
                     : "=v"(Bl[(it_) & 1][pc][j])                                                             \
                     : "v"(b_rd), "n"((pc) * WX_PIECE + ((it_) & 3) * WXROW + ((it_) >> 2) * 256 + j * 32));  \
        asm volatile("ds_read_b64_tr_b16 %0, %1 offset:%2"                                                    \
                     : "=v"(Bh[(it_) & 1][pc][j])                                                             \
                     : "v"(b_rd), "n"((pc) * WX_PIECE + ((it_) & 3) * WXROW + ((it_) >> 2) * 256 + j * 32 + 32)); \
    }
#define MS_W3_WAIT(cnt, it_, pc)                                                                              \
    asm volatile("s_waitcnt lgkmcnt(" #cnt ")"                                                                \
                 : "+v"(Bl[(it_) & 1][pc][0]), "+v"(Bl[(it_) & 1][pc][1]), "+v"(Bl[(it_) & 1][pc][2]),        \
                   "+v"(Bh[(it_) & 1][pc][0]), "+v"(Bh[(it_) & 1][pc][1]), "+v"(Bh[(it_) & 1][pc][2]))
#define MS_W3_MMA(dst, it_, pa, pb)                                                                           \
    _Pragma("unroll") for (int j = 0; j < NKT; ++j) {                                                         \
        const u32x4 bv = {Bl[(it_) & 1][pb][j][0], Bl[(it_) & 1][pb][j][1], Bh[(it_) & 1][pb][j][0],          \
                          Bh[(it_) & 1][pb][j][1]};                                                           \
        dst[(it_) & 3][j] = __builtin_amdgcn_mfma_f32_16x16x32_f16(                                           \
            A[(it_) >> 2][pa], __builtin_bit_cast(f16x8, bv), dst[(it_) & 3][j], 0, 0, 0);                    \
    }
#define MS_W3_ITER(it_)                                                                                       \
// ... 28 lines not shown
#pragma unroll
        for (int c = 0; c < GCG; ++c)
#pragma unroll
            for (int j = 0; j < NKT; ++j)
#pragma unroll
                for (int r = 0; r < 4; ++r) acc[c][j][r] *= kfin;
    }
    __syncthreads();
    static_assert((4 * GCG * NKT * 4 * 64 + 64) * 4 <= 4 * W_WAVE, "reduction scratch fits the staging images");
    float* red = reinterpret_cast<float*>(lds);
#pragma unroll
    for (int c = 0; c < GCG; ++c)
#pragma unroll
        for (int j = 0; j < NKT; ++j)
#pragma unroll
            for (int r = 0; r < 4; ++r) red[(((wid * GCG + c) * NKT + j) * 4 + r) * 64 + lane] = acc[c][j][r];
    float* redb = red + 4 * GCG * NKT * 4 * 64;
#pragma unroll
    for (int i = 0; i < 4; ++i) {
        float v = bsum[i];
        v += __shfl_xor(v, 1, 64);
        v += __shfl_xor(v, 2, 64);
        v += __shfl_xor(v, 4, 64);
        v += __shfl_xor(v, 8, 64);
        if ((lane & 15) == 0) redb[wid * 16 + co0 + 4 * i] = v;
    }
    __syncthreads();
    float* part = partial + (size_t)slab * partial_stride;
    const int J = GCG * GK;
    {
        const int c = wid;
#pragma unroll
        for (int j = 0; j < NKT; ++j) {
            const int kk = j * 16 + (lane & 15);
#pragma unroll
            for (int r = 0; r < 4; ++r) {
                float v = 0.f;
#pragma unroll
                for (int wv = 0; wv < 4; ++wv) v += red[(((wv * GCG + c) * NKT + j) * 4 + r) * 64 + lane];
                const int co = (lane >> 4) * 4 + r;
                if (kk < GK && co < p.Og) part[(size_t)(g * p.Og + co) * J + c * GK + kk] = v;
            }
        }
    }
    if (wid == 0 && lane < 16 && lane < p.Og)
        part[(size_t)p.Cout * J + g * p.Og + lane] = (redb[lane] + redb[16 + lane]) + (redb[32 + lane] + redb[48 + lane]);
}

template <bool VEC>
__global__ __launch_bounds__(256, 2) void k_gconv_split_wgrad(ConvP p, const float* __restrict__ x,
                                                             const float* __restrict__ gy,
                                                             const float* __restrict__ y_act,
                                                             float* __restrict__ partial, size_t partial_stride) {
    gconv_wgrad_body<VEC>(p, x, gy, y_act, partial, partial_stride, blockIdx.x, gridDim.x, blockIdx.x);
}

__global__ __launch_bounds__(256, 2) void k_gconv_split_wgrad_parts(G3Parts q, float* __restrict__ partial, size_t partial_stride) {
    const int bx = blockIdx.x, i = g3_part_of(q, bx);
    const ConvP p = g3_part_conv(q, i);
    const int rbx = bx - q.bx0[i], nbx = q.bx0[i + 1] - q.bx0[i];
    if (i == 0) gconv_wgrad_body<true>(p, q.a[0], q.b[0], q.c[0], partial, partial_stride, rbx, nbx, bx);
    else gconv_wgrad_body<false>(p, q.a[i], q.b[i], q.c[i], partial, partial_stride, rbx, nbx, bx);
}

constexpr int BQ = 48;
constexpr int BNP = 64;
constexpr int BOCT = BNP * 16 + 32;
constexpr int B_PIECE = 2 * BOCT;
constexpr int B_WAVE = 2 * B_PIECE;
constexpr int BJ = 6;

template <bool VEC, bool VOUT>
__device__ __forceinline__ void gconv_bwd_data_body(const ConvP& p, int tiles, int nunits,
                                                    const float* __restrict__ gy,
                                                    const float* __restrict__ y_act,
                                                    const float* __restrict__ w,
                                                    const float* __restrict__ gx_add,
                                                    float* __restrict__ gx, int bx, int nbx) {
    unsigned char* const lds = g3_smem;
    const int tid = threadIdx.x, lane = tid & 63, wid = tid >> 6;
    const int g = blockIdx.y;
    const int kind = y_act ? p.act : MS_ACT_NONE;
    unsigned char* img = lds + wid * B_WAVE;
    const int n = lane & 15, kg = lane >> 4;
    const int oct = kg >> 1, tp = kg & 1;
    const int wstride = nbx * 4;
    const int db = wstride / tiles, dt = wstride - db * tiles;

    const int cq = lane & 3, pq = lane >> 2;
    unsigned char* wr = img + (cq >> 1) * BOCT + (4 * pq) * 16 + (cq & 1) * 8;
    const unsigned g_bytes = 4u * (unsigned)(p.B * p.Cout * p.Lout);
    const auto rsG = __builtin_amdgcn_make_buffer_rsrc(const_cast<float*>(gy), 0, g_bytes, 0x00020000);
    const auto rsA = __builtin_amdgcn_make_buffer_rsrc(const_cast<float*>(y_act ? y_act : gy), 0, g_bytes, 0x00020000);
    unsigned g_c[4];
#pragma unroll
    for (int k = 0; k < 4; ++k) g_c[k] = (unsigned)((4 * cq + k) * p.Lout + 4 * pq) * 4u;
    f32x4 gv[4], ga[4];
    auto gload = [&](int b, int ti) {
        const int ws = ti * BQ - 8;
        const unsigned base = (unsigned)((b * p.Cout + g * 16) * p.Lout);
        if (ws >= 0 && ws + BNP <= p.Lout) {
            const unsigned sb = (unsigned)__builtin_amdgcn_readfirstlane((int)((base + (unsigned)ws) * 4u));
#pragma unroll
            for (int k = 0; k < 4; ++k) {
                gv[k] = __builtin_bit_cast(f32x4, __builtin_amdgcn_raw_buffer_load_b128(rsG, g_c[k], sb, 0));
                ga[k] = __builtin_bit_cast(f32x4, __builtin_amdgcn_raw_buffer_load_b128(rsA, g_c[k], sb, 0));
            }
            return;
        }
        const int t = ws + 4 * pq;
#pragma unroll
        for (int k = 0; k < 4; ++k) {
            const unsigned off = base + (unsigned)((4 * cq + k) * p.Lout);
            if (VEC) {
                const unsigned vo = (t >= 0 && t < p.Lout) ? (off + (unsigned)t) * 4u : OOB;
                gv[k] = __builtin_bit_cast(f32x4, __builtin_amdgcn_raw_buffer_load_b128(rsG, vo, 0, 0));
                ga[k] = __builtin_bit_cast(f32x4, __builtin_amdgcn_raw_buffer_load_b128(rsA, vo, 0, 0));
            } else {
                const unsigned vo = (t >= 0 && t < p.Lout) ? (off + (unsigned)t) * 4u : OOB;
                gv[k] = __builtin_bit_cast(f32x4, __builtin_amdgcn_raw_buffer_load_b128(rsG, vo, 0, 0));
                ga[k] = __builtin_bit_cast(f32x4, __builtin_amdgcn_raw_buffer_load_b128(rsA, vo, 0, 0));
#pragma unroll
                for (int e = 1; e < 4; ++e)
                    if (t + e >= p.Lout) { gv[k][e] = 0.f; ga[k][e] = 0.f; }
            }
        }
    };
    int unit = bx * 4 + wid;
    int b = unit / tiles, ti = unit - b * tiles;
    if (unit < nunits) gload(b, ti);

    f16x8 A[BJ][2];
    float iWS = 1.f;
    {
        const int ci = n >> 2, r = n & 3;
        float wall[BJ][8];
        float wm = 0.f;
#pragma unroll
        for (int J = 0; J < BJ; ++J) {
            const int tap = r + 4 * (2 * J + tp);
            const bool ok = tap < GK;
#pragma unroll
            for (int e = 0; e < 8; ++e) {
                const float v = w[((size_t)(g * 16 + 8 * oct + e) * GCG + ci) * GK + (ok ? tap : 0)];
                wall[J][e] = ok ? v : 0.f;
                wm = fmaxf(wm, fabsf(wall[J][e]));
            }
        }
        float WS;
        weight_scale(wave_max_dpp(wm), WS, iWS);
#pragma unroll
        for (int J = 0; J < BJ; ++J) {
            u32x4 h, l;
#pragma unroll
            for (int q = 0; q < 4; ++q) {
                unsigned hh, ll;
                split_pair(wall[J][2 * q] * WS, wall[J][2 * q + 1] * WS, hh, ll);
                h[q] = hh; l[q] = ll;
            }
            A[J][0] = __builtin_bit_cast(f16x8, h);
            A[J][1] = __builtin_bit_cast(f16x8, l);
        }
    }
    const unsigned rd = (unsigned)(uintptr_t)img + oct * BOCT + (n + 3 - tp) * 16;
    const int Lq = (p.Lin + GS - 1) / GS;

    for (; unit < nunits; unit += wstride) {
        float um = 0.f;
#pragma unroll
        for (int k = 0; k < 4; ++k)
#pragma unroll
            for (int j = 0; j < 4; ++j) um = fmaxf(um, fabsf(gv[k][j]));
        float S, invS;
        block_scale(wave_max_dpp(um), S, invS);
#pragma unroll
        for (int j = 0; j < 4; ++j) {
            float e[4];
#pragma unroll
            for (int k = 0; k < 4; ++k) e[k] = ms_act_grad(gv[k][j], ga[k][j], kind, p.slope) * S;
            unsigned h0, l0, h1, l1;
            split_pair(e[0], e[1], h0, l0);
            split_pair(e[2], e[3], h1, l1);
            *reinterpret_cast<uint2*>(wr + j * 16) = make_uint2(h0, h1);
            *reinterpret_cast<uint2*>(wr + j * 16 + B_PIECE) = make_uint2(l0, l1);
        }
        __builtin_amdgcn_fence(__ATOMIC_RELEASE, "wavefront");
        __builtin_amdgcn_wave_barrier();
        const int q0 = ti * BQ;
        const size_t rowoff = ((size_t)b * p.Cin + (size_t)g * GCG + kg) * p.Lin;
        f32x4 addv[3];
        if (VOUT && gx_add) {
#pragma unroll
            for (int tq = 0; tq < 3; ++tq) {
                const int sidx = (q0 + tq * 16 + n) * GS;
                addv[tq] = *reinterpret_cast<const f32x4*>(gx_add + (sidx < p.Lin ? rowoff + sidx : 0));
            }
        }
        int nb = b + db, nti = ti + dt;
        if (nti >= tiles) { nti -= tiles; ++nb; }
        if (unit + wstride < nunits) gload(nb, nti);

        f32x4 acc[3];
#pragma unroll
        for (int tq = 0; tq < 3; ++tq) acc[tq] = (f32x4){0.f, 0.f, 0.f, 0.f};
        u32x4 Bf[2][2][3];
#define MS_B3_READ(J_, pc)                                                                                    \
    _Pragma("unroll") for (int tq = 0; tq < 3; ++tq)                                                          \
        asm volatile("ds_read_b128 %0, %1 offset:%2"                                                          \
                     : "=v"(Bf[(J_) & 1][pc][tq])                                                             \
                     : "v"(rd), "n"((pc) * B_PIECE + tq * 256 + (BJ - 1 - (J_)) * 32));
#define MS_B3_WAIT(cnt, J_, pc)                                                                               \
    asm volatile("s_waitcnt lgkmcnt(" #cnt ")"                                                                \
                 : "+v"(Bf[(J_) & 1][pc][0]), "+v"(Bf[(J_) & 1][pc][1]), "+v"(Bf[(J_) & 1][pc][2]))
#define MS_B3_MMA(dst, J_, pa, pb)                                                                            \
    _Pragma("unroll") for (int tq = 0; tq < 3; ++tq)                                                          \
        dst[tq] = __builtin_amdgcn_mfma_f32_16x16x32_f16(                                                     \
            A[J_][pa], __builtin_bit_cast(f16x8, Bf[(J_) & 1][pb][tq]), dst[tq], 0, 0, 0);
#define MS_B3_STEP(J_, last)                                                                                  \
    MS_B3_WAIT(3, J_, 1);                                                                                     \
    MS_B3_MMA(acc, J_, 0, 1);                                                                                 \
    if (!(last)) { MS_B3_READ((J_) + 1, 1); MS_B3_WAIT(3, J_, 0); } else { MS_B3_WAIT(0, J_, 0); }            \
    MS_B3_MMA(acc, J_, 1, 0);                                                                                 \
    MS_B3_MMA(acc, J_, 0, 0);                                                                                 \
    if (!(last)) { MS_B3_READ((J_) + 1, 0); }
        MS_B3_READ(0, 1);
        MS_B3_READ(0, 0);
        MS_B3_STEP(0, false) MS_B3_STEP(1, false) MS_B3_STEP(2, false)
        MS_B3_STEP(3, false) MS_B3_STEP(4, false) MS_B3_STEP(5, true)
#undef MS_B3_STEP
#undef MS_B3_MMA
#undef MS_B3_WAIT
#undef MS_B3_READ
        const float kscale = invS * iWS;
#pragma unroll
        for (int tq = 0; tq < 3; ++tq)
#pragma unroll
            for (int rr = 0; rr < 4; ++rr) acc[tq][rr] *= kscale;
        __builtin_amdgcn_fence(__ATOMIC_ACQ_REL, "wavefront");
        __builtin_amdgcn_wave_barrier();
#pragma unroll
        for (int tq = 0; tq < 3; ++tq) {
            const int sidx = (q0 + tq * 16 + n) * GS;
            if (q0 + tq * 16 + n >= Lq || sidx >= p.Lin) continue;
            if (VOUT) {
                f32x4 v = acc[tq];
                if (gx_add) v += addv[tq];
                *reinterpret_cast<f32x4*>(gx + rowoff + sidx) = v;
            } else if (sidx + 3 < p.Lin) {
                f32x4 v = acc[tq];
                if (gx_add) {
                    const f32x4u a4 = *reinterpret_cast<const f32x4u*>(gx_add + rowoff + sidx);
                    v += (f32x4){a4[0], a4[1], a4[2], a4[3]};
                }
                *reinterpret_cast<f32x4u*>(gx + rowoff + sidx) = (f32x4u){v[0], v[1], v[2], v[3]};
            } else {
#pragma unroll
                for (int rr = 0; rr < 4; ++rr) {
                    if (sidx + rr < p.Lin) {
                        float v = acc[tq][rr];
                        if (gx_add) v += gx_add[rowoff + sidx + rr];
                        gx[rowoff + sidx + rr] = v;
                    }
                }
            }
        }
        b = nb; ti = nti;
    }
}

template <bool VEC, bool VOUT>
__global__ __launch_bounds__(256, 2) void k_gconv_split_bwd_data(ConvP p, int tiles, int nunits,
                                                                const float* __restrict__ gy,
                                                                const float* __restrict__ y_act,
                                                                const float* __restrict__ w,
                                                                const float* __restrict__ gx_add,
                                                                float* __restrict__ gx) {
    gconv_bwd_data_body<VEC, VOUT>(p, tiles, nunits, gy, y_act, w, gx_add, gx, blockIdx.x, gridDim.x);
}

__global__ __launch_bounds__(256, 2) void k_gconv_split_bwd_data_parts(G3Parts q, const float* __restrict__ w) {
    const int bx = blockIdx.x, i = g3_part_of(q, bx);
    const ConvP p = g3_part_conv(q, i);
    const int rbx = bx - q.bx0[i], nbx = q.bx0[i + 1] - q.bx0[i];
    if (i == 0) gconv_bwd_data_body<true, true>(p, q.u0[0], q.u1[0], q.a[0], q.b[0], w, q.c[0], q.o[0], rbx, nbx);
    else gconv_bwd_data_body<false, false>(p, q.u0[i], q.u1[i], q.a[i], q.b[i], w, q.c[i], q.o[i], rbx, nbx);
}

int pick_rb(int Lout) {
    if (Lout <= 16) return 4;
    if (Lout <= 32) return 2;
    if (Lout <= 64) return 1;
    const int w64 = ms_ceil_div(Lout, 64) * 64, w32 = ms_ceil_div(Lout, 32) * 32, w16 = ms_ceil_div(Lout, 16) * 16;
    if (w64 * 100 <= w16 * 106) return 1;
    if (w32 * 100 <= w16 * 106) return 2;
    return 4;
}

}

bool msg3_fwd_applicable(const ConvP& p) {
    return ms_switch_on("MSYNTH_GCONV3") && p.K == GK && p.stride == GS && p.Cg == GCG && p.dil == 1 && p.pad_mode == MS_PAD_ZERO &&
           p.Og <= 16 && p.groups <= 65535 &&
           (p.act == MS_ACT_NONE || (p.act == MS_ACT_LRELU && p.slope >= 0.f && p.slope <= 1.f)) &&
           (long long)p.B * p.Cin * p.Lin * 4 < (1ll << 31) &&
           (long long)p.B * p.Cout * p.Lout < (1ll << 31);
}

const char* msg3_fwd_name(const ConvP&) { return "k_gconv_split_fwd"; }

template <int RB>
constexpr size_t g3_fwd_lds() { return 4 * (size_t)GF<RB>::WAVE_BYTES; }
static size_t g3_fwd_lds_rt(int rb) { return rb == 1 ? g3_fwd_lds<1>() : (rb == 2 ? g3_fwd_lds<2>() : g3_fwd_lds<4>()); }

int msg3_conv1d_fwd(const ConvP& p, const float* x, const float* w, const float* bias, float* y,
                    hipStream_t s) {
    const int rb = pick_rb(p.Lout);
    const int ts = 64 / rb;
    const int spr = ms_ceil_div(p.Lout, ts), nseg = p.B * spr, nunits = ms_ceil_div(nseg, rb);
    const int target_waves = 2048;
    const long long total_units = (long long)nunits * p.groups;
    const int upw = (int)((total_units + target_waves - 1) / target_waves);
    const int gxn = ms_ceil_div(nunits, 4 * (upw > 0 ? upw : 1));
    const dim3 grid(gxn, p.groups);
    const bool vec = p.Lin % 4 == 0 && p.pad % 4 == 0 && (((uintptr_t)x) & 15) == 0;
    const bool vout = p.Lout % 4 == 0 && (((uintptr_t)y) & 15) == 0;
#define MS_G3(RBV, V, VO)                                                                                                    \
    do {                                                                                                                     \
        ms_note_kernel(3, "k_gconv_split_fwd<%d, %s, %s>", RBV, V ? "true" : "false", VO ? "true" : "false");               \
        hipLaunchKernelGGL((k_gconv_split_fwd<RBV, V, VO>), grid, dim3(256), g3_fwd_lds<RBV>(), s, p, spr, nseg, nunits, x, w, \
                           bias, y);                                                                                         \
    } while (0)
#define MS_G3V(RBV)                                   \
    do {                                              \
        if (vec && vout) MS_G3(RBV, true, true);      \
        else if (vec) MS_G3(RBV, true, false);        \
        else if (vout) MS_G3(RBV, false, true);       \
        else MS_G3(RBV, false, false);                \
    } while (0)
    if (rb == 1) MS_G3V(1);
    else if (rb == 2) MS_G3V(2);
    else MS_G3V(4);
#undef MS_G3V
#undef MS_G3
    MS_CHECK_LAUNCH();
    return MS_OK;
}

namespace {

bool g3_parts_table(const ConvP& c, const ms_conv1d_parts* parts, G3Parts* q) {
    if (!parts || parts->count < 2 || parts->count > MS_CONV_PARTS_MAX) return false;
    q->p = c;
    q->count = parts->count;
    for (int i = 0; i < parts->count; ++i) {
        if (parts->B[i] <= 0 || parts->Lin[i] <= 0) return false;
        const int eff = parts->Lin[i] + 2 * c.pad - c.dil * (c.K - 1) - 1;
        if (eff < 0) return false;
        q->B[i] = parts->B[i]; q->Lin[i] = parts->Lin[i]; q->Lout[i] = eff / c.stride + 1;
    }
    for (int i = parts->count; i < MS_CONV_PARTS_MAX; ++i) {
        q->B[i] = q->Lin[i] = q->Lout[i] = q->u0[i] = q->u1[i] = q->u2[i] = 0;
        q->a[i] = q->b[i] = q->c[i] = nullptr; q->o[i] = nullptr;
    }
    return true;
}

ConvP g3_host_part(const ConvP& c, const G3Parts& q, int i) {
    ConvP p = c;
    p.B = q.B[i]; p.Lin = q.Lin[i]; p.Lout = q.Lout[i];
    return p;
}

bool al16(const void* a) { return (((uintptr_t)a) & 15) == 0; }

}

bool msg3_parts_fwd_applicable(const ConvP& c, const ms_conv1d_parts* parts) {
    G3Parts q;
    if (!g3_parts_table(c, parts, &q) || q.count != 3) return false;
    for (int i = 0; i < q.count; ++i)
        if (!msg3_fwd_applicable(g3_host_part(c, q, i)) || !parts->x[i] || !parts->y[i]) return false;
    if (q.Lin[0] % 4 || c.pad % 4 || q.Lout[0] % 4 || !al16(parts->x[0]) || !al16(parts->y[0])) return false;
    const int r0 = pick_rb(q.Lout[0]), r1 = pick_rb(q.Lout[1]), r2 = pick_rb(q.Lout[2]);
    return (r0 == 1 && r1 == 1 && r2 == 2) || (r0 == 1 && r1 == 2 && r2 == 4) || (r0 == 1 && r1 == 4 && r2 == 1) ||
           (r0 == 2 && r1 == 2 && r2 == 4);
}

int msg3_parts_fwd(const ConvP& c, const ms_conv1d_parts* parts, const float* w, const float* bias, hipStream_t s) {
    G3Parts q;
    if (!g3_parts_table(c, parts, &q)) return MS_ERR_INVALID_ARG;
    int rb[MS_CONV_PARTS_MAX], nunits[MS_CONV_PARTS_MAX];
    long long total_units = 0;
    size_t lds = 0;
    for (int i = 0; i < q.count; ++i) {
        rb[i] = pick_rb(q.Lout[i]);
        const int ts = 64 / rb[i];
        const int spr = ms_ceil_div(q.Lout[i], ts), nseg = q.B[i] * spr;
        nunits[i] = ms_ceil_div(nseg, rb[i]);
        q.u0[i] = spr; q.u1[i] = nseg; q.u2[i] = nunits[i];
        q.a[i] = parts->x[i]; q.o[i] = parts->y[i];
        total_units += (long long)nunits[i] * c.groups;
        if (g3_fwd_lds_rt(rb[i]) > lds) lds = g3_fwd_lds_rt(rb[i]);
    }
    const int upw = (int)((total_units + 2047) / 2048);
    q.bx0[0] = 0;
    for (int i = 0; i < q.count; ++i) q.bx0[i + 1] = q.bx0[i] + ms_ceil_div(nunits[i], 4 * (upw > 0 ? upw : 1));
    for (int i = q.count; i < MS_CONV_PARTS_MAX; ++i) q.bx0[i + 1] = q.bx0[q.count];
    const dim3 grid(q.bx0[q.count], c.groups);
    ms_note_kernel(3, "k_gconv_split_fwd_parts<%d, %d, %d>", rb[0], rb[1], rb[2]);
#define MS_G3P(A, B_, C_) \
    hipLaunchKernelGGL((k_gconv_split_fwd_parts<A, B_, C_>), grid, dim3(256), lds, s, q, w, bias)
    if (rb[0] == 1 && rb[1] == 1 && rb[2] == 2) MS_G3P(1, 1, 2);
    else if (rb[0] == 1 && rb[1] == 2 && rb[2] == 4) MS_G3P(1, 2, 4);
    else if (rb[0] == 1 && rb[1] == 4 && rb[2] == 1) MS_G3P(1, 4, 1);
    else if (rb[0] == 2 && rb[1] == 2 && rb[2] == 4) MS_G3P(2, 2, 4);
    else return MS_ERR_UNSUPPORTED;
#undef MS_G3P
    MS_CHECK_LAUNCH();
    return MS_OK;
}

bool msg3_bwd_weight_applicable(const ConvP& p) {
    return ms_switch_on("MSYNTH_GCONV3") && p.K == GK && p.stride == GS && p.Cg == GCG && p.dil == 1 && p.pad_mode == MS_PAD_ZERO &&
           p.Og <= 16 && p.groups <= 65535 && (long long)p.B * p.Cin * p.Lin * 4 < (1ll << 30) &&
           (long long)p.B * p.Cout * p.Lout * 4 < (1ll << 31);
}

const char* msg3_bwd_weight_name(const ConvP&) { return "k_gconv_split_wgrad"; }

int msg3_conv1d_bwd_weight(const ConvP& p, const float* x, const float* gy, const float* y_act,
                           float* gw, float* gb, float beta, void* ws, size_t ws_bytes, hipStream_t s) {
    if (!ws || ws_bytes < msg_bwd_weight_ws(p)) return MS_ERR_WORKSPACE;
    const int gxn = msg_wgrad_gridx(p);
    const size_t stride = (size_t)p.Cout * GCG * GK + p.Cout;
    float* partial = (float*)ws;
    const bool vec = p.Lin % 4 == 0 && p.pad % 4 == 0 && p.Lout % 4 == 0 && (((uintptr_t)x) & 15) == 0 &&
                     (((uintptr_t)gy) & 15) == 0 && (!y_act || (((uintptr_t)y_act) & 15) == 0);
    ms_note_kernel(3, "k_gconv_split_wgrad<%s>", vec ? "true" : "false");
    if (vec) hipLaunchKernelGGL((k_gconv_split_wgrad<true>), dim3(gxn, p.groups), dim3(256), 4 * W_WAVE, s, p, x, gy, y_act, partial, stride);
    else hipLaunchKernelGGL((k_gconv_split_wgrad<false>), dim3(gxn, p.groups), dim3(256), 4 * W_WAVE, s, p, x, gy, y_act, partial, stride);
    MS_CHECK_LAUNCH();
    return msg_reduce_slabs(p, partial, stride, gxn, gw, gb, beta, s);
}

namespace {
int g3_wgrad_parts_columns(const ConvP& c, const G3Parts& q, int* cols) {
    const size_t slab = ((size_t)c.Cout * GCG * GK + c.Cout) * sizeof(float);
    long long chunks[MS_CONV_PARTS_MAX], total = 0;
    for (int i = 0; i < q.count; ++i) {
        chunks[i] = ms_ceil_div(q.B[i] * ms_ceil_div(q.Lout[i], WU), 4);
        total += chunks[i];
    }
    int gx = ms_ceil_div(512, c.groups);
    const size_t cap = (size_t)32 << 20;
    while (gx > q.count && (size_t)gx * slab > cap) --gx;
    if (gx < q.count) gx = q.count;
    int sum = 0;
    for (int i = 0; i < q.count; ++i) {
        long long n = (chunks[i] * gx + total - 1) / total;
        if (n < 1) n = 1;
        if (n > chunks[i]) n = chunks[i];
        cols[i] = (int)n;
        sum += cols[i];
    }
    return sum;
}
}

bool msg3_parts_bwd_weight_applicable(const ConvP& c, const ms_conv1d_parts* parts) {
    G3Parts q;
    if (!g3_parts_table(c, parts, &q)) return false;
    for (int i = 0; i < q.count; ++i)
        if (!msg3_bwd_weight_applicable(g3_host_part(c, q, i)) || !parts->x[i] || !parts->gy[i]) return false;
    return q.Lin[0] % 4 == 0 && c.pad % 4 == 0 && q.Lout[0] % 4 == 0 && al16(parts->x[0]) && al16(parts->gy[0]) &&
           (!parts->y_act[0] || al16(parts->y_act[0]));
}

size_t msg3_parts_bwd_weight_ws(const ConvP& c, const ms_conv1d_parts* parts) {
    G3Parts q;
    int cols[MS_CONV_PARTS_MAX];
    if (!g3_parts_table(c, parts, &q)) return 0;
    return (size_t)g3_wgrad_parts_columns(c, q, cols) * ((size_t)c.Cout * GCG * GK + c.Cout) * sizeof(float);
}

int msg3_parts_bwd_weight(const ConvP& c, const ms_conv1d_parts* parts, float* gw, float* gb, float beta, void* ws,
                          size_t ws_bytes, hipStream_t s) {
    G3Parts q;
    int cols[MS_CONV_PARTS_MAX];
    if (!g3_parts_table(c, parts, &q)) return MS_ERR_INVALID_ARG;
    const int gxn = g3_wgrad_parts_columns(c, q, cols);
    const size_t stride = (size_t)c.Cout * GCG * GK + c.Cout;
    if (!ws || ws_bytes < (size_t)gxn * stride * sizeof(float)) return MS_ERR_WORKSPACE;
    q.bx0[0] = 0;
    for (int i = 0; i < q.count; ++i) {
        q.bx0[i + 1] = q.bx0[i] + cols[i];
        q.a[i] = parts->x[i]; q.b[i] = parts->gy[i]; q.c[i] = c.act == MS_ACT_NONE ? nullptr : parts->y_act[i];
    }
    for (int i = q.count; i < MS_CONV_PARTS_MAX; ++i) q.bx0[i + 1] = q.bx0[q.count];
    ms_note_kernel(3, "k_gconv_split_wgrad_parts");
    hipLaunchKernelGGL(k_gconv_split_wgrad_parts, dim3(gxn, c.groups), dim3(256), 4 * W_WAVE, s, q, (float*)ws, stride);
    MS_CHECK_LAUNCH();
    return msg_reduce_slabs(c, (float*)ws, stride, gxn, gw, gb, beta, s);
}

bool msg3_bwd_data_applicable(const ConvP& p) {
    return ms_switch_on("MSYNTH_GCONV3") && p.K == GK && p.stride == GS && p.Cg == GCG && p.dil == 1 && p.pad == 20 &&
           p.pad_mode == MS_PAD_ZERO && p.Og == 16 && p.groups <= 65535 &&
           (long long)p.B * p.Cout * p.Lout * 4 < (1ll << 31);
}

const char* msg3_bwd_data_name(const ConvP&) { return "k_gconv_split_bwd_data"; }

int msg3_conv1d_bwd_data(const ConvP& p, const float* gy, const float* y_act, const float* w,
                         const float* gx_add, float* gx, hipStream_t s) {
    const int Lq = ms_ceil_div(p.Lin, GS);
    const int tiles = ms_ceil_div(Lq, BQ), nunits = p.B * tiles;
    const long long total_units = (long long)nunits * p.groups;
    const int upw = (int)((total_units + 2047) / 2048);
    const int gxn = ms_ceil_div(nunits, 4 * (upw > 0 ? upw : 1));
    const dim3 grid(gxn, p.groups);
    const bool vec = p.Lout % 4 == 0 && (((uintptr_t)gy) & 15) == 0 && (!y_act || (((uintptr_t)y_act) & 15) == 0);
    const bool vout = p.Lin % 4 == 0 && (((uintptr_t)gx) & 15) == 0 && (!gx_add || (((uintptr_t)gx_add) & 15) == 0);
#define MS_B3(V, VO)                                                                                                              \
    do {                                                                                                                          \
        ms_note_kernel(3, "k_gconv_split_bwd_data<%s, %s>", V ? "true" : "false", VO ? "true" : "false");                        \
        hipLaunchKernelGGL((k_gconv_split_bwd_data<V, VO>), grid, dim3(256), 4 * B_WAVE, s, p, tiles, nunits, gy, y_act, w, gx_add, \
                           gx);                                                                                                   \
    } while (0)
    if (vec && vout) MS_B3(true, true);
    else if (vec) MS_B3(true, false);
    else if (vout) MS_B3(false, true);
    else MS_B3(false, false);
#undef MS_B3
    MS_CHECK_LAUNCH();
    return MS_OK;
}

bool msg3_parts_bwd_data_applicable(const ConvP& c, const ms_conv1d_parts* parts) {
    G3Parts q;
    if (!g3_parts_table(c, parts, &q)) return false;
    for (int i = 0; i < q.count; ++i)
        if (!msg3_bwd_data_applicable(g3_host_part(c, q, i)) || !parts->gy[i] || !parts->gx[i]) return false;
    return q.Lout[0] % 4 == 0 && q.Lin[0] % 4 == 0 && al16(parts->gy[0]) && al16(parts->gx[0]) &&
           (!parts->y_act[0] || al16(parts->y_act[0])) && (!parts->gx_add[0] || al16(parts->gx_add[0]));
}

int msg3_parts_bwd_data(const ConvP& c, const ms_conv1d_parts* parts, const float* w, hipStream_t s) {
    G3Parts q;
    if (!g3_parts_table(c, parts, &q)) return MS_ERR_INVALID_ARG;
    int nunits[MS_CONV_PARTS_MAX];
    long long total_units = 0;
    for (int i = 0; i < q.count; ++i) {
        const int Lq = ms_ceil_div(q.Lin[i], GS);
        const int tiles = ms_ceil_div(Lq, BQ);
        nunits[i] = q.B[i] * tiles;
        q.u0[i] = tiles; q.u1[i] = nunits[i]; q.u2[i] = 0;
        q.a[i] = parts->gy[i]; q.b[i] = c.act == MS_ACT_NONE ? nullptr : parts->y_act[i]; q.c[i] = parts->gx_add[i];
        q.o[i] = parts->gx[i];
        total_units += (long long)nunits[i] * c.groups;
    }
    const int upw = (int)((total_units + 2047) / 2048);
    q.bx0[0] = 0;
    for (int i = 0; i < q.count; ++i) q.bx0[i + 1] = q.bx0[i] + ms_ceil_div(nunits[i], 4 * (upw > 0 ? upw : 1));
    for (int i = q.count; i < MS_CONV_PARTS_MAX; ++i) q.bx0[i + 1] = q.bx0[q.count];
    ms_note_kernel(3, "k_gconv_split_bwd_data_parts");
    hipLaunchKernelGGL(k_gconv_split_bwd_data_parts, dim3(q.bx0[q.count], c.groups), dim3(256), 4 * B_WAVE, s, q, w);
    MS_CHECK_LAUNCH();
    return MS_OK;
}
```

### music-synthesis_amd/csrc/operand_split.h

```cpp
#pragma once
#include "ms_common.h"

namespace {

typedef float f32x16 __attribute__((ext_vector_type(16)));
typedef float f32x4 __attribute__((ext_vector_type(4)));
typedef float f32x4u __attribute__((ext_vector_type(4), aligned(4)));
typedef float f32x2 __attribute__((ext_vector_type(2)));
typedef __bf16 bf16x2 __attribute__((ext_vector_type(2)));
typedef __bf16 bf16x8 __attribute__((ext_vector_type(8)));
typedef _Float16 f16x2 __attribute__((ext_vector_type(2)));
typedef _Float16 f16x8 __attribute__((ext_vector_type(8)));
typedef unsigned u32x4 __attribute__((ext_vector_type(4)));
typedef unsigned u32x2 __attribute__((ext_vector_type(2)));

template <int NP> __host__ __device__ constexpr int xrs() { return NP * 32 + 16; }

__host__ __device__ __forceinline__ void split_pair(float a, float b, unsigned& h, unsigned& m, unsigned& l) {
    const f32x2 v = {a, b};
    const bf16x2 hi = __builtin_convertvector(v, bf16x2);
    const f32x2 r1 = v - __builtin_convertvector(hi, f32x2);
    const bf16x2 mi = __builtin_convertvector(r1, bf16x2);
    const f32x2 r2 = r1 - __builtin_convertvector(mi, f32x2);
    const bf16x2 lo = __builtin_convertvector(r2, bf16x2);
// ... 24 lines not shown
        o[1] = make_uint2(m0, m1);
        o[2] = make_uint2(l0, l1);
    } else {
        unsigned a[2], b[2];
        split_pair(e[0], e[1], a[0], a[1]);
        split_pair(e[2], e[3], b[0], b[1]);
        o[0] = make_uint2(a[0], b[0]);
        o[1] = make_uint2(a[1], b[1]);
    }
}

template <int TOP>
__host__ __device__ __forceinline__ void pow2_scale(float m, float& S, float& invS) {
    const unsigned eb = (__builtin_bit_cast(unsigned, m) >> 23) & 0xFFu;
    const bool ok = eb >= 16u && eb <= 250u;
    S = ok ? __builtin_bit_cast(float, (254u + TOP - eb) << 23) : 1.f;
    invS = ok ? __builtin_bit_cast(float, (eb - TOP) << 23) : 1.f;
}
__host__ __device__ __forceinline__ void block_scale(float m, float& S, float& invS) { pow2_scale<14>(m, S, invS); }
__host__ __device__ __forceinline__ void weight_scale(float m, float& S, float& invS) { pow2_scale<12>(m, S, invS); }

__device__ __forceinline__ float wave_max(float v) {
#pragma unroll
    for (int o = 32; o > 0; o >>= 1) v = fmaxf(v, __shfl_xor(v, o, 64));
    return v;
}

__device__ __forceinline__ float weight_max16(const float* __restrict__ pm) {
    float m = 0.f;
#pragma unroll
    for (int i = 0; i < 16; ++i) m = fmaxf(m, pm[i]);
    return m;
}
__device__ __forceinline__ float weight_max256(const float* __restrict__ pm) {
    __shared__ float wmax_s;
    if (threadIdx.x < 64) {
        const float m = wave_max(fmaxf(fmaxf(pm[threadIdx.x], pm[threadIdx.x + 64]), fmaxf(pm[threadIdx.x + 128], pm[threadIdx.x + 192])));
        if (threadIdx.x == 0) wmax_s = m;
    }
    __syncthreads();
    return wmax_s;
}

constexpr unsigned OOB = 0xF0000000u;

__device__ __forceinline__ f32x4 load_row4(__amdgpu_buffer_rsrc_t rs, unsigned row_elems, int t, int L) {
    const bool any = t >= 0 && t < L;
    f32x4 v = __builtin_bit_cast(f32x4, __builtin_amdgcn_raw_buffer_load_b128(rs, any ? (row_elems + (unsigned)t) * 4u : OOB, 0, 0));
#pragma unroll
    for (int e = 1; e < 4; ++e) v[e] = t + e < L ? v[e] : 0.f;
    return v;
}

}
```

### music-synthesis_amd/featuresynth/_ops/graph.py

```python
import contextlib
import os

import torch

from . import lib as L
from . import prims as P

G_UPSAMPLE = ((8, 4), (8, 4), (2, 1), (2, 1))
DILATIONS = (1, 3, 9)
G_NPARAMS = 2 + 4 * (2 + 12) + 2
D_LAYERS = ((1, 7, 1), (4, 20, 4), (4, 20, 16), (4, 20, 64), (4, 20, 256), (1, 2, 1))
D_NPARAMS = 14


class GradSink:

    def __init__(self, n, dests=None, acc=None):
        self.t = list(dests) if dests is not None else [None] * n
        self.acc = list(acc) if acc is not None else [False] * n

    def pair(self, i):
        return self.t[i], self.t[i + 1], (self.acc[i] and self.t[i] is not None)

    def put(self, i, gw, gb):
# ... 318 lines not shown
        fn()
    fork.join()
    if fork_b is not fork:
        fork_b.join()
    assert i == 0
    return sink, gx



def pack_k5_image(x_shape, params, backward=False):
    w = params[10]
    B = x_shape[0]
    if tuple(w.shape[1:]) != (w.shape[0], 5) or params[11].data_ptr() % 16:
        return None
    d = L.ConvDesc(B, w.shape[1], 32, w.shape[0], 5, 1, 2, 1, 1, L.PAD_ZERO, L.ACT_LRELU, P.SLOPE, L.ACT_NONE)
    if not P.conv_img_bytes(d):
        return None
    return P.conv_img_pack(d, w, backward=backward)


def pack_k5_image_pair(x_shape, params):
    w = params[10]
    if tuple(w.shape[1:]) != (w.shape[0], 5) or params[11].data_ptr() % 16:
        return None, None
    d = L.ConvDesc(x_shape[0], w.shape[1], 32, w.shape[0], 5, 1, 2, 1, 1, L.PAD_ZERO, L.ACT_LRELU, P.SLOPE, L.ACT_NONE)
    if not P.conv_img_bytes(d):
        return None, None
    return P.conv_img_pack2(d, w)


def fork_aux(device):
    if not _may_fork(device):
        return False
    aux_stream(device).wait_stream(torch.cuda.current_stream(device))
    return True


def pack_k5_images_aside(x_shape, params, device, forked_at=None):
    if not (_may_fork(device) if forked_at is None else forked_at):
        return pack_k5_image_pair(x_shape, params) + (None,)
    main, aux = torch.cuda.current_stream(device), aux_stream(device)
    if forked_at is None:
        aux.wait_stream(main)
    with forked(aux):
        f, b = pack_k5_image_pair(x_shape, params)
        ev = torch.cuda.Event()
        ev.record(aux)
    for t in (f, b):
        if t is not None:
            t.record_stream(main)
    return f, b, ev


D_HEAD_PARAM = 10


_SIDE_STREAMS = {}


def aux_stream(device):
    key = (device.index, "aux")
    if key not in _SIDE_STREAMS:
        _SIDE_STREAMS[key] = torch.cuda.Stream(device=device)
    return _SIDE_STREAMS[key]


def _side_streams(device, n):
    key = (device.index, n, _FORK_DEPTH)
    if key not in _SIDE_STREAMS:
        _SIDE_STREAMS[key] = [torch.cuda.Stream(device=device) for _ in range(n)]
    return _SIDE_STREAMS[key]


def begin_step():
    _FORKED_SINCE_JOIN.clear()


def join_side_streams(device):
    main = torch.cuda.current_stream(device)
    capturing = torch.cuda.is_current_stream_capturing()
    for st in list(_FORKED_SINCE_JOIN):
        if st.device != device:
            continue
        _FORKED_SINCE_JOIN.discard(st)
        if st == main:
            continue
        if capturing:
            with torch.cuda.stream(st):
                if not torch.cuda.is_current_stream_capturing():
                    continue
        main.wait_stream(st)


def _on_aux(device):
    return _FORK_DEPTH == 0 and torch.cuda.current_stream(device) == aux_stream(device)


def _concurrent_scales():
    return os.environ.get("MSYNTH_STREAMS", "1") != "0"


def melgan_forward(x, params, scales=2, k5_image=None):
    if len(params) != D_NPARAMS:
        raise RuntimeError("discriminator expects %d parameter tensors, got %d" % (D_NPARAMS, len(params)))
    L.require(x, "discriminator input")
    if x.dim() != 3 or x.shape[1] != 1:
        raise RuntimeError("discriminator input must be (B, 1, L), got %s" % (tuple(x.shape),))
    xs = [x]
    for s in range(scales):
        xs.append(P.avg_pool_fwd(xs[-1]))
    n = len(xs)
    if k5_image is None:
        k5_image = pack_k5_image(x.shape, params)
    feats, tapes = [[] for _ in range(n)], [[] for _ in range(n)]
    hs = xs
    for li, (stride, pad, groups) in enumerate(D_LAYERS):
        w, b = params[2 * li], params[2 * li + 1]
        ds = [P.conv_desc(h.shape, w.shape, stride=stride, pad=pad, groups=groups, act=L.ACT_LRELU)[0] for h in hs]
        img = k5_image if (li == 5 and k5_image is not None and P.conv_img_bytes(ds[0])) else None
        ys = P.conv1d_parts_fwd(hs, w, b, ds[0], image=img)
        for s in range(n):
            tapes[s].append((ds[s], hs[s], ys[s]))
            feats[s].append(ys[s])
        hs = ys
    w, b = params[12], params[13]
    djs = [P.conv_desc(h.shape, w.shape, pad=1)[0] for h in hs]
    js = P.conv1d_parts_fwd(hs, w, b, djs[0])
    for s in range(n):
        tapes[s].append((djs[s], hs[s], js[s]))
    return feats, js, (tapes, xs)


def melgan_backward(ctx, params, g_feats, g_judges, sink=None, need_gx=True, need_wgrad=True, cut=None,
                          k5_image_bwd=None):
    tapes, xs = ctx
    n = len(tapes)
    sink = sink if sink is not None else GradSink(D_NPARAMS)
    k5_bwd = k5_image_bwd if k5_image_bwd is not None else pack_k5_image(xs[0].shape, params, backward=True)

    def own(s, li):
        return g_feats[s][li] if (g_feats is not None and g_feats[s] is not None and li >= 0) else None

    mode = os.environ.get("MSYNTH_DWGSTREAM", "2")
    fork = _WgradFork(xs[0].device) if (need_wgrad and mode != "0") else None
    fork2 = _WgradFork(xs[0].device, 1) if (fork is not None and mode == "2" and cut is None) else None

    def wgrad(slot, live, xs_, gys, yas, d, w_shape):
        gw, gb, acc = sink.pair(slot)
        a, b_, c = [xs_[s] for s in live], [gys[s] for s in live], (None if yas is None else [yas[s] for s in live])

        def go():
            sink.put(slot, *P.conv1d_parts_bwd_weight(a, b_, c, d, w_shape, gw, gb, acc))
        if fork is not None:
            (fork2 if (fork2 is not None and slot < D_HEAD_PARAM) else fork).run(go, *(a + b_ + (c or [])))
        else:
            go()

    g = [None] * n
    live = [s for s in range(n) if g_judges is not None and g_judges[s] is not None]
    if live:
        dj = tapes[live[0]][6][0]
        h5 = [tapes[s][6][1] for s in range(n)]
        if need_wgrad:
            wgrad(12, live, h5, g_judges, None, dj, params[12].shape)
        outs = P.conv1d_parts_bwd_data([g_judges[s] for s in live], None, params[12], dj, [h5[s].shape for s in live],
                                       gx_adds=[own(s, 5) for s in live])
        for s, o in zip(live, outs):
            g[s] = o
    for s in range(n):
        if g[s] is None:
            g[s] = own(s, 5)
    for li in range(5, -1, -1):
        live = [s for s in range(n) if g[s] is not None]
        prev = [own(s, li - 1) if li > 0 else None for s in range(n)]
        if live:
            d = tapes[live[0]][li][0]
            hin = [tapes[s][li][1] for s in range(n)]
            h = [tapes[s][li][2] for s in range(n)]
            if need_wgrad:
                wgrad(2 * li, live, hin, g, h, d, params[2 * li].shape)
            if li > 0 or need_gx:
                img = k5_bwd if (li == 5 and k5_bwd is not None and P.conv_img_bytes(d)) else None
                outs = P.conv1d_parts_bwd_data([g[s] for s in live], [h[s] for s in live], params[2 * li], d,
                                               [hin[s].shape for s in live], gx_adds=[prev[s] for s in live], image_bwd=img)
                for s, o in zip(live, outs):
                    g[s] = o
            else:
                for s in live:
                    g[s] = None
        for s in range(n):
            if s not in live:
                g[s] = prev[s]
        if li == 5 and cut is not None:
            if fork is not None:
                fork.join()
            cut()
    if fork is not None:
        fork.join()
    if fork2 is not None:
        fork2.join()
    gx_next = None
    for s in range(n - 1, -1, -1):
        gx = g[s]
        if gx_next is not None and need_gx:
            B = gx_next.shape[0]
            gx = P.avg_pool_bwd(gx_next, (B,) + tuple(xs[s].shape[1:]), gx_add=gx)
        gx_next = gx
    return (gx_next if need_gx else None), sink
```

### music-synthesis_amd/featuresynth/_ops/lib.py

```python
import ctypes
import os

import torch

_HERE = os.path.dirname(os.path.abspath(__file__))
LIB_PATH = os.environ.get("MSYNTH_LIB") or os.path.join(os.path.dirname(_HERE), "_lib", "libmsynth_hip.so")

ACT_NONE, ACT_LRELU, ACT_TANH = 0, 1, 2
PAD_ZERO, PAD_REFLECT = 0, 1

_c_int = ctypes.c_int32
_c_i64 = ctypes.c_int64
_c_f = ctypes.c_float
_vp = ctypes.c_void_p
_sz = ctypes.c_size_t


class ConvDesc(ctypes.Structure):
    _fields_ = [(n, _c_int) for n in ("B", "Cin", "Lin", "Cout", "K", "stride", "pad", "dil",
                                      "groups", "pad_mode", "act")] + [("slope", _c_f), ("in_act", _c_int)]


class ConvTDesc(ctypes.Structure):
    _fields_ = [(n, _c_int) for n in ("B", "Cin", "Lin", "Cout", "K", "stride", "pad", "act")] + \
               [("slope", _c_f), ("in_act", _c_int)]


L1_MULTI_MAX = 24


class L1MultiDesc(ctypes.Structure):
    _fields_ = [("count", _c_int), ("reserved", _c_int),
                ("r", _vp * L1_MULTI_MAX), ("f", _vp * L1_MULTI_MAX), ("gf", _vp * L1_MULTI_MAX),
                ("n", ctypes.c_int64 * L1_MULTI_MAX), ("w", _c_f * L1_MULTI_MAX)]


JUDGE_MULTI_MAX = 8
JUDGE_MULTI_NMAX = 1 << 20
JUDGE_HINGE_D, JUDGE_NEG_MEAN = 0, 1


class JudgeMultiDesc(ctypes.Structure):
    _fields_ = [("count", _c_int), ("kind", _c_int),
                ("r", _vp * JUDGE_MULTI_MAX), ("f", _vp * JUDGE_MULTI_MAX),
                ("gr", _vp * JUDGE_MULTI_MAX), ("gf", _vp * JUDGE_MULTI_MAX),
                ("n", ctypes.c_int64 * JUDGE_MULTI_MAX)]


CONV_PARTS_MAX = 3


class ConvParts(ctypes.Structure):
    _fields_ = [("count", _c_int), ("reserved", _c_int), ("B", _c_int * CONV_PARTS_MAX), ("Lin", _c_int * CONV_PARTS_MAX),
                ("x", _vp * CONV_PARTS_MAX), ("y", _vp * CONV_PARTS_MAX), ("gy", _vp * CONV_PARTS_MAX),
                ("y_act", _vp * CONV_PARTS_MAX), ("gx_add", _vp * CONV_PARTS_MAX), ("gx", _vp * CONV_PARTS_MAX)]


WGRAD_MULTI_MAX = 8


class WgradMultiDesc(ctypes.Structure):
    _fields_ = [("count", _c_int), ("reserved", _c_int),
                ("conv", ConvDesc * WGRAD_MULTI_MAX),
                ("x", _vp * WGRAD_MULTI_MAX), ("gy", _vp * WGRAD_MULTI_MAX), ("y_act", _vp * WGRAD_MULTI_MAX),
                ("gw", _vp * WGRAD_MULTI_MAX), ("gb", _vp * WGRAD_MULTI_MAX),
                ("beta", _c_f * WGRAD_MULTI_MAX),
                ("xmax", _vp * WGRAD_MULTI_MAX), ("gmax", _vp * WGRAD_MULTI_MAX), ("y_signs", _vp * WGRAD_MULTI_MAX)]


ATOM_AMAX_N = 1024


ATOM_PACK_MAX = 16


class AtomDesc(ctypes.Structure):
    _fields_ = [("B", _c_int), ("C", _c_int), ("L", _c_int), ("dil", _c_int), ("slope", _c_f)]


STACK_MAX = 3


class StackDesc(ctypes.Structure):
    _fields_ = [("B", _c_int), ("C", _c_int), ("L", _c_int), ("count", _c_int), ("dil", _c_int * STACK_MAX),
                ("slope", _c_f)]


class AtomPackDesc(ctypes.Structure):
    _fields_ = [("count", _c_int), ("reserved", _c_int), ("C", _c_int * ATOM_PACK_MAX),
                ("w0", _vp * ATOM_PACK_MAX), ("w1", _vp * ATOM_PACK_MAX), ("image", _vp * ATOM_PACK_MAX),
                ("backward", _c_int * ATOM_PACK_MAX)]


LINES_MAX_PHASES, LINES_MAX_TAPS = 2, 3


class LinesDesc(ctypes.Structure):
    _fields_ = [("B", _c_int), ("H", _c_int), ("C", _c_int), ("W", _c_int), ("phases", _c_int), ("taps", _c_int),
                ("dy", _c_int * (LINES_MAX_PHASES * LINES_MAX_TAPS))]


WN_MULTI_MAX = 64


class WnMultiDesc(ctypes.Structure):
    _fields_ = [("count", _c_int), ("reserved", _c_int),
                ("v", _vp * WN_MULTI_MAX), ("g", _vp * WN_MULTI_MAX), ("out", _vp * WN_MULTI_MAX),
                ("gv", _vp * WN_MULTI_MAX), ("gg", _vp * WN_MULTI_MAX),
# ... 86 lines not shown
    "ms_l1_mean_fwd": (_c_int, [_vp, _vp, _c_i64, _vp, _vp, _sz, _vp]),
    "ms_l1_mean_bwd": (_c_int, [_vp, _vp, _c_i64, _vp, _c_f, _vp, _c_int, _vp]),
    "ms_l1_mean_multi_workspace_bytes": (_sz, [ctypes.POINTER(L1MultiDesc)]),
    "ms_l1_mean_multi_fwd": (_c_int, [ctypes.POINTER(L1MultiDesc), _vp, _vp, _sz, _vp]),
    "ms_l1_mean_multi_bwd": (_c_int, [ctypes.POINTER(L1MultiDesc), _vp, _c_f, _vp]),
    "ms_l1_mean_multi_fwd_bwd_workspace_bytes": (_sz, [ctypes.POINTER(L1MultiDesc)]),
    "ms_l1_mean_multi_fwd_bwd": (_c_int, [ctypes.POINTER(L1MultiDesc), _vp, _c_f, _vp, _sz, _vp]),
    "ms_ls_g_fwd": (_c_int, [_vp, _c_i64, _vp, _vp, _sz, _vp]),
    "ms_ls_g_bwd": (_c_int, [_vp, _c_i64, _vp, _c_f, _vp, _vp]),
    "ms_ls_d_fwd": (_c_int, [_vp, _vp, _c_i64, _vp, _vp, _sz, _vp]),
    "ms_ls_d_bwd": (_c_int, [_vp, _vp, _c_i64, _vp, _c_f, _vp, _vp, _vp]),
    "ms_weighted_sum": (_c_int, [_vp, _vp, _c_int, _vp, _vp]),
    "ms_adam_step": (_c_int, [_vp, _vp, _vp, _vp, _c_i64, _c_f, _c_f, _c_f, _c_f, _c_f, _vp, _vp]),
    "ms_audio2mel_frames": (_c_int, [_c_int, _c_int, _c_int]),
    "ms_audio2mel_fwd": (_c_int, [_vp, _c_int, _c_int, _vp, _c_int, _c_int, _vp, _c_int, _vp, _vp]),
    "ms_audio2mel_bwd_workspace_bytes": (_sz, [_c_int, _c_int, _c_int, _c_int]),
    "ms_audio2mel_bwd": (_c_int, [_vp, _c_int, _c_int, _vp, _c_int, _c_int, _vp, _c_int, _vp, _vp, _vp, _sz, _vp]),
    "ms_stft_frames": (_c_int, [_c_int, _c_int, _c_int]),
    "ms_stft_mag_fwd": (_c_int, [_vp, _c_int, _c_int, _vp, _c_int, _c_int, _c_f, _vp, _vp]),
    "ms_stft_mag_bwd_workspace_bytes": (_sz, [_c_int, _c_int, _c_int, _c_int]),
    "ms_stft_mag_bwd": (_c_int, [_vp, _c_int, _c_int, _vp, _c_int, _c_int, _c_f, _vp, _vp, _vp, _sz, _vp]),
    "ms_stft_pair_loss_workspace_bytes": (_sz, [_c_i64]),
    "ms_stft_pair_loss_target": (_c_int, [_vp, _c_i64, _vp, _vp, _sz, _vp]),
    "ms_stft_pair_loss_fwd": (_c_int, [_vp, _vp, _c_i64, _vp, _c_f, _c_f, _vp, _vp, _vp, _sz, _vp]),
    "ms_stft_pair_loss_bwd": (_c_int, [_vp, _vp, _c_i64, _vp, _vp, _c_f, _c_f, _vp, _vp]),
    "ms_resample_sinc_fwd": (_c_int, [_vp, _c_int, _c_int, _vp, _c_int, ctypes.c_double, _vp, _vp, _c_int, _c_int, _vp]),
    "ms_peak_normalize": (_c_int, [_vp, _c_int, _c_int, _c_f, _vp, _vp]),
    "ms_comm_unique_id": (_c_int, [_vp]),
    "ms_comm_init": (_c_int, [_vp, _c_int, _c_int, ctypes.POINTER(_vp)]),
    "ms_comm_world": (_c_int, [_vp]),
    "ms_comm_rank": (_c_int, [_vp]),
    "ms_allreduce_f32": (_c_int, [_vp, _vp, _c_i64, _vp]),
    "ms_comm_destroy": (_c_int, [_vp]),
    "ms_comm_last_error": (ctypes.c_char_p, []),
}
COMM_ID_BYTES = 128

BAND_MAX = 8


class BandDesc(ctypes.Structure):
    _fields_ = [("count", _c_int), ("lowest", _c_int), ("size", _c_int * BAND_MAX), ("data", _vp * BAND_MAX)]


BAND_SIGNATURES = {
    "ms_band_supported": (_c_int, [_c_int, ctypes.POINTER(BandDesc)]),
    "ms_band_workspace_bytes": (_sz, [_c_int, _c_int, ctypes.POINTER(BandDesc)]),
    "ms_band_decompose_fwd": (_c_int, [_vp, _c_int, _c_int, ctypes.POINTER(BandDesc), _vp, _sz, _vp]),
    "ms_band_decompose_bwd": (_c_int, [ctypes.POINTER(BandDesc), _c_int, _c_int, _vp, _vp, _sz, _vp]),
    "ms_band_recompose_fwd": (_c_int, [ctypes.POINTER(BandDesc), _c_int, _c_int, _vp, _vp, _sz, _vp]),
    "ms_band_recompose_bwd": (_c_int, [_vp, _c_int, _c_int, ctypes.POINTER(BandDesc), _vp, _sz, _vp]),
}

_LIB = None


def load():
    global _LIB
    if _LIB is None:
        if not os.path.exists(LIB_PATH):
            raise RuntimeError(
                "featuresynth (MI355X build): %s is missing; build it with "
                "`make -C music-synthesis_amd/csrc` or __graft_entry__.build(). There is no CPU "
                "or PyTorch fallback for the hot path." % LIB_PATH)
        lib = ctypes.CDLL(LIB_PATH)
        for name, (res, args) in list(SIGNATURES.items()) + list(BAND_SIGNATURES.items()):
            fn = getattr(lib, name)
            fn.restype = res
            fn.argtypes = args
        _LIB = lib
    return _LIB


def check(rc, what):
    if rc != 0:
        msg = load().ms_status_string(rc)
        raise RuntimeError("%s failed: %s (ms_status %d)" % (what, msg.decode() if msg else "?", rc))


def ptr(t):
    return None if t is None else t.data_ptr()


def require(t, name):
    if not isinstance(t, torch.Tensor):
        raise RuntimeError("%s: expected a torch.Tensor, got %r" % (name, type(t)))
    if not t.is_cuda:
        raise RuntimeError(
            "%s: featuresynth (MI355X build) only runs on a HIP device tensor; got device %s. "
            "There is no CPU fallback." % (name, t.device))
    if t.dtype != torch.float32:
        raise RuntimeError("%s: expected float32, got %s" % (name, t.dtype))
    if not t.is_contiguous():
        raise RuntimeError("%s: expected a contiguous tensor" % name)
    return t


def stream():
    return torch.cuda.current_stream().cuda_stream


def workspace(nbytes, device):
    if nbytes <= 0:
        return None
    return torch.empty(int(nbytes), dtype=torch.uint8, device=device)


PROFILE = None


def profile_begin():
    global PROFILE
    PROFILE = []
    load().ms_profile_kernels(1)


def profile_end(calibrate=False):
    global PROFILE
    rec, PROFILE = PROFILE, None
# ... 40 lines not shown
```

### music-synthesis_amd/featuresynth/_ops/prims.py

```python
import os

import numpy as np
import ctypes

import torch

from . import lib as L
from .. import _workload as W


_WHICH = {"fwd": 0, "bwd_data": 1, "bwd_weight": 2}


def _ccost(d, which, **kw):
    return lambda: dict(W.conv_cost(d.B, d.Cin, d.Lin, d.Cout, d.K, d.stride, d.pad, d.dil, d.groups,
                                    which, **kw),
                        geom=(d.B, d.Cin, d.Lin, d.Cout, d.K, d.stride, d.dil, d.groups),
                        kernel=L.load().ms_conv1d_kernel_name(d, _WHICH[which]).decode())


def _tcost(d, which, abi_which, **kw):
    m = W.convt_as_conv(d.B, d.Cin, d.Lin, d.Cout, d.K, d.stride, d.pad)
    return lambda: dict(W.conv_cost(which=which, **m, **kw),
                        geom=(d.B, d.Cin, d.Lin, d.Cout, d.K, d.stride, 1, 1),
# ... 98 lines not shown
            continue
        md = L.WgradMultiDesc()
        md.count = len(chunk)
        costs = []
        keep = []
        for k, job in enumerate(chunk):
            (x, gy, ya, d, w_shape, gw, gb, acc), bounds = job[:8], job[8:]
            L.require(gy, "conv1d grad_output"); L.require(x, "conv1d input")
            if len(bounds) == 2 and bounds[0] is not None and bounds[1] is not None:
                md.xmax[k], md.gmax[k] = bounds[0].data_ptr(), bounds[1].data_ptr()
                keep += list(bounds)
            if gw is None:
                gw = torch.empty(tuple(w_shape), dtype=torch.float32, device=gy.device)
                acc = False
            if gb is None:
                gb = (torch.zeros if acc else torch.empty)((d.Cout,), dtype=torch.float32, device=gy.device)
            md.conv[k] = d
            md.x[k], md.gy[k] = x.data_ptr(), gy.data_ptr()
            if is_signs(ya):
                md.y_signs[k] = ya.data_ptr()
            else:
                md.y_act[k] = L.ptr(ya)
            md.gw[k], md.gb[k], md.beta[k] = gw.data_ptr(), gb.data_ptr(), 1.0 if acc else 0.0
            costs.append(_ccost(d, "bwd_weight", act_read=ya is not None))
            out.append((gw, gb))
        nws = lib.ms_conv1d_bwd_weight_multi_workspace_bytes(md)
        ws = L.workspace(nws, chunk[0][1].device)

        def cost(costs=costs):
            cs = [c() for c in costs]
            tot = dict(cs[0])
            tot["flops"] = sum(c["flops"] for c in cs)
            tot["bytes"] = sum(c["bytes"] for c in cs)
            tot["batched"] = len(cs)
            return tot
        L.call("ms_conv1d_bwd_weight_multi", cost, md, L.ptr(ws), nws, L.stream())
    return out


def _part_desc(d, B, Lin):
    return L.ConvDesc(B, d.Cin, Lin, d.Cout, d.K, d.stride, d.pad, d.dil, d.groups, d.pad_mode, d.act, d.slope, d.in_act)


def _parts_cost(d, shapes, which, name, **kw):
    def cost():
        cs = [W.conv_cost(B, d.Cin, Lin, d.Cout, d.K, d.stride, d.pad, d.dil, d.groups, which, **kw) for B, Lin in shapes]
        nw = 4 * (d.Cout * (d.Cin // d.groups) * d.K + d.Cout)
        return {"flops": sum(c["flops"] for c in cs), "bytes": sum(c["bytes"] for c in cs) - (len(cs) - 1) * nw,
                "geom": ("parts", tuple(shapes), d.Cin, d.Cout, d.K, d.stride, d.dil, d.groups),
                "kernel": L.load().ms_conv1d_kernel_name(_part_desc(d, *shapes[0]), _WHICH[which]).decode(), "parts": len(cs)}
    return cost


def conv1d_parts_fwd(xs, w, b, d, image=None):
    if not 1 <= len(xs) <= L.CONV_PARTS_MAX:
        raise RuntimeError("conv1d_parts: 1 .. %d parts" % L.CONV_PARTS_MAX)
    L.require(w, "conv1d weight")
    if b is not None:
        L.require(b, "conv1d bias")
    parts = L.ConvParts()
    parts.count = len(xs)
    ys, shapes = [], []
    for i, x in enumerate(xs):
        L.require(x, "conv1d input")
        if x.dim() != 3 or x.shape[1] != d.Cin:
            raise RuntimeError("conv1d_parts: input %d is %s, expected (B, %d, L)" % (i, tuple(x.shape), d.Cin))
        B, Lin = int(x.shape[0]), int(x.shape[2])
        lo = L.load().ms_conv1d_out_len(_part_desc(d, B, Lin))
        if lo <= 0:
            raise RuntimeError("conv1d_parts: invalid geometry for part %d: %s" % (i, tuple(x.shape)))
        y = torch.empty((B, d.Cout, lo), dtype=torch.float32, device=x.device)
        parts.B[i], parts.Lin[i], parts.x[i], parts.y[i] = B, Lin, x.data_ptr(), y.data_ptr()
        ys.append(y); shapes.append((B, Lin))
    lib = L.load()
    nws = lib.ms_conv1d_parts_workspace_bytes(d, parts, 0, 1 if image is not None else 0)
    ws = L.workspace(nws, xs[0].device)
    L.call("ms_conv1d_parts_fwd", _parts_cost(d, shapes, "fwd", "fwd"), d, parts, w.data_ptr(), L.ptr(b), L.ptr(image),
           L.ptr(ws), nws, L.stream())
    return ys


def conv1d_parts_bwd_data(gys, y_acts, w, d, in_shapes, gx_adds=None, image_bwd=None):
    n = len(gys)
    parts = L.ConvParts()
    parts.count = n
    gxs, shapes = [], []
    for i in range(n):
        gy = L.require(gys[i], "conv1d grad_output")
        B, Lin = int(gy.shape[0]), int(in_shapes[i][-1])
        ya = y_acts[i] if (y_acts is not None and d.act != L.ACT_NONE) else None
        if ya is not None:
            L.require(ya, "conv1d saved output")
            if ya.shape[0] < B or tuple(ya.shape[1:]) != tuple(gy.shape[1:]):
                raise RuntimeError("conv1d_parts: saved output %s does not cover gradient %s" % (tuple(ya.shape), tuple(gy.shape)))
        ga = gx_adds[i] if gx_adds is not None else None
        gx = torch.empty((B, d.Cin, Lin), dtype=torch.float32, device=gy.device)
        if ga is not None:
            L.require(ga, "conv1d gx_add")
            if ga.shape != gx.shape:
                raise RuntimeError("conv1d_parts: gx_add %s != input gradient %s" % (tuple(ga.shape), tuple(gx.shape)))
        parts.B[i], parts.Lin[i] = B, Lin
        parts.gy[i], parts.y_act[i], parts.gx_add[i], parts.gx[i] = gy.data_ptr(), L.ptr(ya), L.ptr(ga), gx.data_ptr()
        gxs.append(gx); shapes.append((B, Lin))
    lib = L.load()
    nws = lib.ms_conv1d_parts_workspace_bytes(d, parts, 1, 1 if image_bwd is not None else 0)
    ws = L.workspace(nws, gys[0].device)
    L.call("ms_conv1d_parts_bwd_data", _parts_cost(d, shapes, "bwd_data", "bwd_data", act_read=d.act != L.ACT_NONE,
                                                   extra_reads=int(gx_adds is not None and any(g is not None for g in gx_adds))),
           d, parts, w.data_ptr(), L.ptr(image_bwd), L.ptr(ws), nws, L.stream())
    return gxs


def conv1d_parts_bwd_weight(xs, gys, y_acts, d, w_shape, gw=None, gb=None, accumulate=False):
    n = len(gys)
    dev_ = gys[0].device
    if gw is None:
        gw = torch.empty(tuple(w_shape), dtype=torch.float32, device=dev_)
        accumulate = False
    if gb is None:
        gb = (torch.zeros if accumulate else torch.empty)((d.Cout,), dtype=torch.float32, device=dev_)
    parts = L.ConvParts()
    parts.count = n
    shapes = []
    for i in range(n):
        gy, x = L.require(gys[i], "conv1d grad_output"), L.require(xs[i], "conv1d input")
        B, Lin = int(gy.shape[0]), int(x.shape[2])
        if x.shape[0] < B or x.shape[1] != d.Cin:
            raise RuntimeError("conv1d_parts: input %s does not cover gradient %s" % (tuple(x.shape), tuple(gy.shape)))
        ya = y_acts[i] if (y_acts is not None and d.act != L.ACT_NONE) else None
        if ya is not None and (ya.shape[0] < B or tuple(ya.shape[1:]) != tuple(gy.shape[1:])):
            raise RuntimeError("conv1d_parts: saved output %s does not cover gradient %s" % (tuple(ya.shape), tuple(gy.shape)))
        parts.B[i], parts.Lin[i] = B, Lin
        parts.x[i], parts.gy[i], parts.y_act[i] = x.data_ptr(), gy.data_ptr(), L.ptr(ya)
        shapes.append((B, Lin))
    lib = L.load()
    nws = lib.ms_conv1d_parts_workspace_bytes(d, parts, 2, 0)
    ws = L.workspace(nws, dev_)
    L.call("ms_conv1d_parts_bwd_weight", _parts_cost(d, shapes, "bwd_weight", "bwd_weight", act_read=d.act != L.ACT_NONE),
           d, parts, gw.data_ptr(), gb.data_ptr(), 1.0 if accumulate else 0.0, L.ptr(ws), nws, L.stream())
    return gw, gb


def conv_img_bytes(d):
    return int(L.load().ms_conv1d_img_bytes(d))


def conv_img_pack(d, w, backward=False):
    L.require(w, "conv1d weight")
    img = torch.empty(conv_img_bytes(d), dtype=torch.uint8, device=w.device)
    L.call("ms_conv1d_img_pack", _scost(w.numel(), 1, 1.5), d, w.data_ptr(), 1 if backward else 0, img.data_ptr(), L.stream())
    return img


def conv_img_pack2(d, w):
    L.require(w, "conv1d weight")
    img = torch.empty(conv_img_bytes(d), dtype=torch.uint8, device=w.device)
    imgb = torch.empty(conv_img_bytes(d), dtype=torch.uint8, device=w.device)
    L.call("ms_conv1d_img_pack2", _scost(w.numel(), 1, 2.5), d, w.data_ptr(), img.data_ptr(), imgb.data_ptr(), L.stream())
    return img, imgb


def conv1d_img_fwd(x, image, b, d, lout, out=None):
    L.require(x, "conv1d input")
    y = _out(out, (d.B, d.Cout, lout), x.device, "conv1d output")
    nws = L.load().ms_conv1d_img_workspace_bytes(d, 0)
    ws = L.workspace(nws, x.device)

    def cost():
        return dict(W.conv_cost(d.B, d.Cin, d.Lin, d.Cout, d.K, d.stride, d.pad, d.dil, d.groups, "fwd"),
                    geom=(d.B, d.Cin, d.Lin, d.Cout, d.K, d.stride, d.dil, d.groups))
    L.call("ms_conv1d_img_fwd", cost, d, x.data_ptr(), image.data_ptr(), L.ptr(b), y.data_ptr(), L.ptr(ws), nws, L.stream())
    return y


def conv1d_img_bwd_data(gy, y_act, image_bwd, d, gx_add=None):
    L.require(gy, "conv1d grad_output")
    gx = torch.empty((d.B, d.Cin, d.Lin), dtype=torch.float32, device=gy.device)
    nws = L.load().ms_conv1d_img_workspace_bytes(d, 1)
    ws = L.workspace(nws, gy.device)

    def cost():
        return dict(W.conv_cost(d.B, d.Cin, d.Lin, d.Cout, d.K, d.stride, d.pad, d.dil, d.groups, "bwd_data",
                                act_read=y_act is not None, extra_reads=int(gx_add is not None)),
                    geom=(d.B, d.Cin, d.Lin, d.Cout, d.K, d.stride, d.dil, d.groups))
    L.call("ms_conv1d_img_bwd_data", cost, d, gy.data_ptr(), L.ptr(y_act), image_bwd.data_ptr(), L.ptr(gx_add), gx.data_ptr(),
           L.ptr(ws), nws, L.stream())
    return gx


def atom_supported(B, C, Lg, dil):
    return bool(L.load().ms_residual_atom_supported(L.AtomDesc(B, C, Lg, dil, SLOPE)))
# ... 721 lines not shown
```

### music-synthesis_amd/featuresynth/_workload.py

```python

G_UPS = ((512, 256, 16, 8, 4), (256, 128, 16, 8, 4), (128, 64, 4, 2, 1), (64, 32, 4, 2, 1))
D_MAIN = ((1, 16, 15, 1, 7, 1), (16, 64, 41, 4, 20, 4), (64, 256, 41, 4, 20, 16),
          (256, 1024, 41, 4, 20, 64), (1024, 1024, 41, 4, 20, 256), (1024, 1024, 5, 1, 2, 1))
F32 = 4


def conv_out_len(lin, k, stride, pad, dil=1):
    return (lin + 2 * pad - dil * (k - 1) - 1) // stride + 1


def conv_cost(B, Cin, Lin, Cout, K, stride, pad, dil, groups, which, extra_reads=0, extra_writes=0,
              act_read=False):
    Lout = conv_out_len(Lin, K, stride, pad, dil)
    macs = B * Cout * Lout * (Cin // groups) * K
    nin, nout, nw = B * Cin * Lin, B * Cout * Lout, Cout * (Cin // groups) * K + Cout
    if which == "fwd":
        elems = nin + nout + nw + (extra_reads + extra_writes) * nout
    elif which == "bwd_data":
        elems = nout + (nout if act_read else 0) + nin + nw + extra_reads * nin
    else:
        elems = nin + nout + (nout if act_read else 0) + nw
    return {"flops": 2 * macs, "bytes": F32 * elems}


def convt_as_conv(B, Cin, Lin, Cout, K, stride, pad):
    Lout = (Lin - 1) * stride - 2 * pad + K
    return dict(B=B, Cin=Cout, Lin=Lout, Cout=Cin, K=K, stride=stride, pad=pad, dil=1, groups=1)


def _atom(B, C, L, d, mode, out):
    c0 = dict(B=B, Cin=C, Lin=L, Cout=C, K=3, stride=1, pad=d, dil=d, groups=1)
    c1 = dict(B=B, Cin=C, Lin=L, Cout=C, K=3, stride=1, pad=1, dil=1, groups=1)
    if mode == "fwd":
        out.append(("atom%d.conv0.fwd" % C, conv_cost(which="fwd", **c0)))
        out.append(("atom%d.conv1.fwd" % C, conv_cost(which="fwd", extra_reads=1, **c1)))
    elif mode == "fwd_train":
        out.append(("atom%d.conv0.fwd" % C, conv_cost(which="fwd", **c0)))
        out.append(("atom%d.conv1.fwd" % C, conv_cost(which="fwd", extra_reads=1, extra_writes=1, **c1)))
    else:
        out.append(("atom%d.conv1.bwd_weight" % C, conv_cost(which="bwd_weight", act_read=True, **c1)))
        out.append(("atom%d.conv1.bwd_data" % C, conv_cost(which="bwd_data", act_read=True, **c1)))
        out.append(("atom%d.conv0.bwd_weight" % C, conv_cost(which="bwd_weight", act_read=True, **c0)))
        out.append(("atom%d.conv0.bwd_data" % C, conv_cost(which="bwd_data", act_read=True, extra_reads=1, **c0)))


def generator_launches(B, mels, T, mode):
    out = []
    L = T
    first = dict(B=B, Cin=mels, Lin=L, Cout=512, K=7, stride=1, pad=3, dil=1, groups=1)
    stages = []
    for cin, cout, k, s, p in G_UPS:
        stages.append((cin, cout, k, s, p, L))
        L = (L - 1) * s - 2 * p + k
    last = dict(B=B, Cin=32, Lin=L, Cout=1, K=7, stride=1, pad=3, dil=1, groups=1)
    if mode != "bwd":
        out.append(("g.first.fwd", conv_cost(which="fwd", **first)))
        for cin, cout, k, s, p, lin in stages:
            m = convt_as_conv(B, cin, lin, cout, k, s, p)
            out.append(("g.convT%d.fwd" % cout, conv_cost(which="bwd_data", **m)))
            for d in (1, 3, 9):
                _atom(B, cout, m["Lin"], d, mode, out)
        out.append(("g.last.fwd", conv_cost(which="fwd", **last)))
    else:
        out.append(("g.last.bwd_weight", conv_cost(which="bwd_weight", act_read=True, **last)))
        out.append(("g.last.bwd_data", conv_cost(which="bwd_data", act_read=True, **last)))
        for cin, cout, k, s, p, lin in reversed(stages):
            m = convt_as_conv(B, cin, lin, cout, k, s, p)
            for d in (9, 3, 1):
                _atom(B, cout, m["Lin"], d, "bwd", out)
            out.append(("g.convT%d.bwd_weight" % cout, conv_cost(which="bwd_weight", act_read=True, **m)))
            out.append(("g.convT%d.bwd_data" % cout, conv_cost(which="fwd", extra_reads=1, **m)))
        out.append(("g.first.bwd_weight", conv_cost(which="bwd_weight", act_read=True, **first)))
    return out


def discriminator_launches(B, L0, mode, need_gx=False, feat_grads=False):
    out = []
    L = L0
    for s in range(3):
        if s:
            lp = (L + 4 - 4) // 2 + 1
            out.append(("d.pool.%s" % mode, {"flops": 4 * B * lp, "bytes": F32 * B * (L + lp)}))
            L = lp
        l = L
        geo = []
        for cin, cout, k, st, p, g in D_MAIN:
            geo.append(dict(B=B, Cin=cin, Lin=l, Cout=cout, K=k, stride=st, pad=p, dil=1, groups=g))
            l = conv_out_len(l, k, st, p)
        judge = dict(B=B, Cin=1024, Lin=l, Cout=1, K=3, stride=1, pad=1, dil=1, groups=1)
        if mode == "fwd":
            for i, c in enumerate(geo):
                out.append(("d.main%d.fwd" % i, conv_cost(which="fwd", **c)))
            out.append(("d.judge.fwd", conv_cost(which="fwd", **judge)))
        else:
            out.append(("d.judge.bwd_data", conv_cost(which="bwd_data", extra_reads=int(feat_grads), **judge)))
            for i in range(5, -1, -1):
                if not need_gx or True:
                    pass
                if i > 0 or need_gx:
                    out.append(("d.main%d.bwd_data" % i,
                                conv_cost(which="bwd_data", act_read=True,
                                          extra_reads=int(feat_grads and i > 0), **geo[i])))
    return out


def discriminator_wgrad_launches(B, L0):
    out = []
    L = L0
    for s in range(3):
        if s:
            L = (L + 4 - 4) // 2 + 1
        l = L
        for i, (cin, cout, k, st, p, g) in enumerate(D_MAIN):
            out.append(("d.main%d.bwd_weight" % i,
                        conv_cost(B, cin, l, cout, k, st, p, 1, g, "bwd_weight", act_read=True)))
            l = conv_out_len(l, k, st, p)
        out.append(("d.judge.bwd_weight", conv_cost(B, 1024, l, 1, 3, 1, 1, 1, 1, "bwd_weight")))
    return out


def feature_elems(B, L0):
    tot, L = 0, L0
    for s in range(3):
        if s:
            L = (L + 4 - 4) // 2 + 1
        l = L
        for cin, cout, k, st, p, g in D_MAIN:
            l = conv_out_len(l, k, st, p)
            tot += B * cout * l
    return tot


def d_step_launches(B, mels=80, T=32):
    L0 = T * 256
    out = generator_launches(B, mels, T, "fwd")
    for _ in range(2):
        out += discriminator_launches(B, L0, "fwd")
    for _ in range(2):
        out += discriminator_launches(B, L0, "bwd", need_gx=False)
        out += discriminator_wgrad_launches(B, L0)
    nparam = 5637953
    out.append(("adam.D", {"flops": 12 * nparam, "bytes": 7 * F32 * nparam}))
    return out


def g_step_launches(B, mels=80, T=32):
    L0 = T * 256
    out = generator_launches(B, mels, T, "fwd_train")
    out += discriminator_launches(B, L0, "fwd")
    out += discriminator_launches(B, L0, "fwd")
    fe = feature_elems(B, L0)
    out.append(("loss.l1.fwd", {"flops": 3 * fe, "bytes": 2 * F32 * fe}))
    out.append(("loss.l1.bwd", {"flops": 2 * fe, "bytes": 3 * F32 * fe}))
    out += discriminator_launches(B, L0, "bwd", need_gx=True, feat_grads=True)
    out += generator_launches(B, mels, T, "bwd")
    nparam = 4519937 + (mels - 80) * 512 * 7
    out.append(("adam.G", {"flops": 12 * nparam, "bytes": 7 * F32 * nparam}))
    return out


SIGN_WORDS = 1.0 / 32
STACK_FUSED_MAX_C = 64


def _atom_fused(B, C, L, d, mode, out):
    n = B * C * L
    c0 = conv_cost(B, C, L, C, 3, 1, d, d, 1, "fwd")
    fl, wb = 2 * c0["flops"], F32 * 2 * (3 * C * C + C)
    if mode == "fwd":
        out.append(("atom%d.fwd" % C, {"flops": fl, "bytes": int(F32 * n * 2) + wb}))
    elif mode == "fwd_train":
        out.append(("atom%d.fwd_train" % C, {"flops": fl, "bytes": int(F32 * n * (3 + 2 * SIGN_WORDS)) + wb}))
    else:
        out.append(("atom%d.bwd_data" % C, {"flops": fl, "bytes": int(F32 * n * (3 + 2 * SIGN_WORDS)) + wb}))
        for nm in ("conv1", "conv0"):
            out.append(("atom%d.%s.bwd_weight" % (C, nm),
                        {"flops": c0["flops"], "bytes": int(F32 * n * (2 + SIGN_WORDS)) + wb // 2}))


def fused_generator_launches(B, mels, T, mode):
    out = []
    for name, c in generator_launches(B, mels, T, mode):
        if not name.startswith("atom"):
            out.append((name, c))
    L = T
    atoms = []
    for cin, cout, k, s, p in G_UPS:
        L = (L - 1) * s - 2 * p + k
        if mode == "fwd" and cout <= STACK_FUSED_MAX_C:
            n = B * cout * L
            fl = sum(2 * conv_cost(B, cout, L, cout, 3, 1, d, d, 1, "fwd")["flops"] for d in (1, 3, 9))
            atoms.append(("stack%d.fwd" % cout, {"flops": fl, "bytes": F32 * n * 2 + 3 * F32 * 2 * (3 * cout * cout + cout)}))
            continue
        for d in ((1, 3, 9) if mode != "bwd" else (9, 3, 1)):
            _atom_fused(B, cout, L, d, mode, atoms)
    return out + atoms


def fused_d_step_launches(B, mels=80, T=32):
    L0 = T * 256
    out = fused_generator_launches(B, mels, T, "fwd")
    out += discriminator_launches(2 * B, L0, "fwd")
    out += discriminator_launches(2 * B, L0, "bwd", need_gx=False)
    out += discriminator_wgrad_launches(2 * B, L0)
    nparam = 5637953
    out.append(("adam.D", {"flops": 12 * nparam, "bytes": 7 * F32 * nparam}))
    return out


def fused_g_step_launches(B, mels=80, T=32):
    L0 = T * 256
    out = fused_generator_launches(B, mels, T, "fwd_train")
    out += discriminator_launches(B, L0, "fwd")
    out += discriminator_launches(B, L0, "fwd")
    fe = feature_elems(B, L0)
    out.append(("loss.l1.fwd_bwd", {"flops": 5 * fe, "bytes": 3 * F32 * fe}))
    out += discriminator_launches(B, L0, "bwd", need_gx=True, feat_grads=True)
    out += fused_generator_launches(B, mels, T, "bwd")
    nparam = 4519937 + (mels - 80) * 512 * 7
    out.append(("adam.G", {"flops": 12 * nparam, "bytes": 7 * F32 * nparam}))
    return out


SURVEY_MB_PER_ELEMENT_PER_CALL = 135.0


REAL_UPS = ((512, 256, 16, 8, 4), (256, 128, 16, 8, 4), (128, 64, 4, 2, 1), (64, 32, 4, 2, 1))


def _resblock(B, C, L, d, mode, out):
    sc = dict(B=B, Cin=C, Lin=L, Cout=C, K=1, stride=1, pad=0, dil=1, groups=1)
    c3 = dict(B=B, Cin=C, Lin=L, Cout=C, K=3, stride=1, pad=d, dil=d, groups=1)
    if mode in ("fwd", "fwd_train"):
        out.append(("res%d.shortcut.fwd" % C, conv_cost(which="fwd", **sc)))
        out.append(("res%d.conv3.fwd" % C, conv_cost(which="fwd", **c3)))
        out.append(("res%d.conv1.fwd" % C, conv_cost(which="fwd", extra_reads=1, **sc)))
    else:
        out.append(("res%d.conv1.bwd_weight" % C, conv_cost(which="bwd_weight", **sc)))
        out.append(("res%d.conv1.bwd_data" % C, conv_cost(which="bwd_data", **sc)))
        out.append(("res%d.conv3.bwd_weight" % C, conv_cost(which="bwd_weight", act_read=True, **c3)))
        out.append(("res%d.conv3.bwd_data" % C, conv_cost(which="bwd_data", act_read=True, **c3)))
        out.append(("res%d.shortcut.bwd_weight" % C, conv_cost(which="bwd_weight", **sc)))
        out.append(("res%d.shortcut.bwd_data" % C, conv_cost(which="bwd_data", extra_reads=1, **sc)))


def real_generator_launches(B, mels, T, mode):
    out = []
    L = T
    first = dict(B=B, Cin=mels, Lin=L, Cout=512, K=7, stride=1, pad=3, dil=1, groups=1)
    stages = []
    for cin, cout, k, s, p in REAL_UPS:
        stages.append((cin, cout, k, s, p, L))
        L = (L - 1) * s - 2 * p + k
    last = dict(B=B, Cin=32, Lin=L, Cout=1, K=7, stride=1, pad=3, dil=1, groups=1)
    if mode != "bwd":
        out.append(("g.first.fwd", conv_cost(which="fwd", **first)))
        for cin, cout, k, s, p, lin in stages:
            m = convt_as_conv(B, cin, lin, cout, k, s, p)
            out.append(("g.convT%d.fwd" % cout, conv_cost(which="bwd_data", **m)))
            for d in (1, 3, 9):
                _resblock(B, cout, m["Lin"], d, mode, out)
        out.append(("g.last.fwd", conv_cost(which="fwd", **last)))
    else:
        out.append(("g.last.bwd_weight", conv_cost(which="bwd_weight", act_read=True, **last)))
        out.append(("g.last.bwd_data", conv_cost(which="bwd_data", act_read=True, **last)))
        for cin, cout, k, s, p, lin in reversed(stages):
            m = convt_as_conv(B, cin, lin, cout, k, s, p)
            for d in (9, 3, 1):
                _resblock(B, cout, m["Lin"], d, "bwd", out)
            out.append(("g.convT%d.bwd_weight" % cout, conv_cost(which="bwd_weight", act_read=True, **m)))
# ... 123 lines not shown
```

Baseline: 104.9 million samples/s.

## Store discriminator leaky-ReLU activation signs as bitmasks for backward passes

The discriminator's first layers' forward kernels now also write one bit per output element recording whether the activation was positive. The backward-data and weight-gradient kernels read these packed sign words instead of the full fp32 activations to compute the leaky-ReLU gradient. This cuts activation reads in backward by roughly 32x for those layers, at the cost of an extra small write and lane-OR in forward. It also adds API plumbing and validation for the sign buffers.

```diff
diff --git a/include/msynth.h b/include/msynth.h
--- a/include/msynth.h
+++ b/include/msynth.h
@@ -61,6 +61,7 @@
     const float* y_act[MS_CONV_PARTS_MAX];
     const float* gx_add[MS_CONV_PARTS_MAX];
     float* gx[MS_CONV_PARTS_MAX];
+    uint32_t* y_signs[MS_CONV_PARTS_MAX];
 } ms_conv1d_parts;
 int ms_conv1d_parts_launches(const ms_conv1d_desc* d, const ms_conv1d_parts* parts, int which, int with_image);
 size_t ms_conv1d_parts_workspace_bytes(const ms_conv1d_desc* d, const ms_conv1d_parts* parts, int which, int with_image);
diff --git a/include/msynth_dsigns.h b/include/msynth_dsigns.h
--- /dev/null
+++ b/include/msynth_dsigns.h
@@ -0,0 +1,16 @@
+#ifndef MSYNTH_DSIGNS_H
+#define MSYNTH_DSIGNS_H
+
+#include "msynth.h"
+
+#ifdef __cplusplus
+extern "C" {
+#endif
+
+int ms_conv1d_parts_signs_supported(const ms_conv1d_desc* d, const ms_conv1d_parts* parts, int which);
+
+#ifdef __cplusplus
+}
+#endif
+
+#endif
diff --git a/music-synthesis_amd/csrc/api.hip b/music-synthesis_amd/csrc/api.hip
--- a/music-synthesis_amd/csrc/api.hip
+++ b/music-synthesis_amd/csrc/api.hip
@@ -8,6 +8,7 @@
 #include <unistd.h>
 #include "conv_mfma.h"
 #include "gconv_mfma.h"
+#include "msynth_dsigns.h"
 #include "conv_thin.h"
 
 static thread_local int g_prof_on = 0, g_prof_launches = 0, g_prof_products = 0;
@@ -389,6 +390,25 @@
         if (m > n) n = m;
     }
     return pl.add(P_EACH, c, n);
+}
+
+int parts_signs(const ms_conv1d_parts* parts) {
+    int n = 0;
+    for (int i = 0; i < parts->count; ++i) n += parts->y_signs[i] ? 1 : 0;
+    return n == 0 ? 0 : (n == parts->count ? 1 : -1);
+}
+
+bool plan_takes_signs(const Plan& pl, const ConvP& c, const ms_conv1d_parts* parts) {
+    for (int i = 0; i < parts->count; ++i)
+        if (((uintptr_t)parts->y_signs[i]) & 3) return false;
+    const Kind k = pl.r[0].kind;
+    return (k == P_G3 && msg3_parts_take_signs(c)) || (k == P_DISC && msd_parts_take_signs(c));
+}
+
+int check_signs(const Plan& pl, const ConvP& c, const ms_conv1d_parts* parts) {
+    const int sg = parts_signs(parts);
+    if (sg < 0) return MS_ERR_INVALID_ARG;
+    return (sg && !plan_takes_signs(pl, c, parts)) ? MS_ERR_UNSUPPORTED : MS_OK;
 }
 
 const char* route_name(Kind k, const ConvP& g) {
@@ -563,13 +583,21 @@
 int ms_conv1d_parts_launches(const ms_conv1d_desc* d, const ms_conv1d_parts* parts, int which, int with_image) {
     ConvP c;
     if (!parts_ok(d, parts, &c) || which < 0 || which > 2) return MS_ERR_INVALID_ARG;
-    return parts_plan(d, c, parts, which, true, with_image != 0).r[0].kind == P_EACH ? parts->count : 1;
+    const Plan pl = parts_plan(d, c, parts, which, true, with_image != 0);
+    if (const int rc = check_signs(pl, c, parts)) return rc;
+    return pl.r[0].kind == P_EACH ? parts->count : 1;
 }
 
 size_t ms_conv1d_parts_workspace_bytes(const ms_conv1d_desc* d, const ms_conv1d_parts* parts, int which, int with_image) {
     ConvP c;
     if (!parts_ok(d, parts, &c) || which < 0 || which > 2) return 0;
     return parts_plan(d, c, parts, which, true, with_image != 0).ws();
+}
+
+int ms_conv1d_parts_signs_supported(const ms_conv1d_desc* d, const ms_conv1d_parts* parts, int which) {
+    ConvP c;
+    if (!parts_ok(d, parts, &c) || which < 0 || which > 2) return 0;
+    return plan_takes_signs(parts_plan(d, c, parts, which, true, false), c, parts) ? 1 : 0;
 }
 
 int ms_conv1d_parts_fwd(const ms_conv1d_desc* d, const ms_conv1d_parts* parts, const float* w, const float* bias,
@@ -577,7 +605,9 @@
     ConvP c;
     if (!parts_ok(d, parts, &c) || (!w && !image)) return MS_ERR_INVALID_ARG;
     hipStream_t s = (hipStream_t)stream;
-    return run(parts_plan(d, c, parts, 0, w, image), workspace, workspace_bytes, [&](Kind k, const ConvP&) {
+    const Plan pl = parts_plan(d, c, parts, 0, w, image);
+    if (const int rc = check_signs(pl, c, parts)) return rc;
+    return run(pl, workspace, workspace_bytes, [&](Kind k, const ConvP&) {
         switch (k) {
             case P_DISC: return msd_parts_fwd(c, parts, w, bias, s);
             case P_G4: return msg4_parts_fwd(c, parts, w, bias, s);
@@ -603,7 +633,9 @@
     ConvP c;
     if (!parts_ok(d, parts, &c) || (!w && !image_bwd)) return MS_ERR_INVALID_ARG;
     hipStream_t s = (hipStream_t)stream;
-    return run(parts_plan(d, c, parts, 1, w, image_bwd), workspace, workspace_bytes, [&](Kind k, const ConvP&) {
+    const Plan pl = parts_plan(d, c, parts, 1, w, image_bwd);
+    if (const int rc = check_signs(pl, c, parts)) return rc;
+    return run(pl, workspace, workspace_bytes, [&](Kind k, const ConvP&) {
         switch (k) {
             case P_DISC: return msd_parts_bwd_data(c, parts, w, s);
             case P_G4: return msg4_parts_bwd_data(c, parts, w, s);
@@ -632,7 +664,9 @@
     ConvP c;
     if (!parts_ok(d, parts, &c) || !gw || (beta != 0.f && beta != 1.f)) return MS_ERR_INVALID_ARG;
     hipStream_t s = (hipStream_t)stream;
-    return run(parts_plan(d, c, parts, 2, true, false), workspace, workspace_bytes, [&](Kind k, const ConvP&) {
+    const Plan pl = parts_plan(d, c, parts, 2, true, false);
+    if (const int rc = check_signs(pl, c, parts)) return rc;
+    return run(pl, workspace, workspace_bytes, [&](Kind k, const ConvP&) {
         switch (k) {
             case P_DISC: return msd_parts_bwd_weight(c, parts, gw, gb, beta, workspace, workspace_bytes, s);
             case P_G4: return msg4_parts_bwd_weight(c, parts, gw, gb, beta, s);
diff --git a/music-synthesis_amd/csrc/disc_parts.hip b/music-synthesis_amd/csrc/disc_parts.hip
--- a/music-synthesis_amd/csrc/disc_parts.hip
+++ b/music-synthesis_amd/csrc/disc_parts.hip
@@ -14,6 +14,7 @@
     const float* b[NP];
     const float* c[NP];
     float* o[NP];
+    uint32_t* sg[NP];
 };
 
 struct DPart {
@@ -22,16 +23,25 @@
     const float* b;
     const float* c;
     float* o;
+    uint32_t* sg;
 };
 __device__ __forceinline__ DPart pick_part(const DParts& q, int wg) {
-    DPart p{q.B[0], q.L[0], q.tiles[0], wg, q.a[0], q.b[0], q.c[0], q.o[0]};
+    DPart p{q.B[0], q.L[0], q.tiles[0], wg, q.a[0], q.b[0], q.c[0], q.o[0], q.sg[0]};
 #pragma unroll
     for (int k = 1; k < NP; ++k)
-        if (k < q.count && wg >= q.wg0[k]) p = DPart{q.B[k], q.L[k], q.tiles[k], wg - q.wg0[k], q.a[k], q.b[k], q.c[k], q.o[k]};
+        if (k < q.count && wg >= q.wg0[k]) p = DPart{q.B[k], q.L[k], q.tiles[k], wg - q.wg0[k], q.a[k], q.b[k], q.c[k], q.o[k], q.sg[k]};
     return p;
 }
 
 __device__ __forceinline__ float lrelu_grad(float g, float y, float slope) { return y > 0.f ? g : g * slope; }
+
+template <bool SG>
+__device__ __forceinline__ f32x4 load_act4(__amdgpu_buffer_rsrc_t rsA, unsigned row, int W, int t, int L) {
+    if (!SG) return load_row4(rsA, row * (unsigned)L, t, L);
+    const unsigned word = load_sign_word(rsA, row * (unsigned)W, t, L);
+    const int sh = t & 31;
+    return (f32x4){sign_as_act(word, sh), sign_as_act(word, sh + 1), sign_as_act(word, sh + 2), sign_as_act(word, sh + 3)};
+}
 
 constexpr int FK = 15, FPAD = 7, FC = 16, FT = 1024;
 
@@ -51,7 +61,9 @@
     const int b = p.wg / p.tiles, tile_t = (p.wg - b * p.tiles) * FT;
     stage_thin_window(xs, p.a, p.B, p.L, b, tile_t);
     const int t0 = tile_t + 4 * threadIdx.x;
-    if (t0 >= p.L) return;
+    if (!p.sg && t0 >= p.L) return;
+    const bool live = t0 < p.L;
+    const int W = (p.L + 31) >> 5;
     float win[20];
 #pragma unroll
     for (int i = 0; i < 5; ++i) {
@@ -81,10 +93,18 @@
             for (int e = 0; e < 4; ++e)
                 if (t0 + e < p.L) yr[e] = v[e];
         }
-    }
-}
-
-__global__ __launch_bounds__(256) void k_dfirst_bwd_data(DParts q, const float* __restrict__ w, float slope) {
+        if (p.sg) {
+            unsigned nib = 0;
+#pragma unroll
+            for (int e = 0; e < 4; ++e) nib |= (t0 + e < p.L && v[e] > 0.f) ? 1u << e : 0u;
+            const unsigned word = or_lanes8(nib << (4 * (threadIdx.x & 7)));
+            if (live && (threadIdx.x & 7) == 0) p.sg[((size_t)b * FC + co) * W + (t0 >> 5)] = word;
+        }
+    }
+}
+
+template <bool SG>
+__device__ __forceinline__ void dfirst_bwd_data_body(const DParts& q, const float* __restrict__ w, float slope) {
     __shared__ float red[4][256 + 4];
     const DPart p = pick_part(q, blockIdx.x);
     const int lane = threadIdx.x & 63, wid = threadIdx.x >> 6;
@@ -92,7 +112,9 @@
     const int t0 = tile_t + 4 * lane;
     const unsigned bytes = 4u * (unsigned)(p.B * FC * p.L);
     const auto rsG = __builtin_amdgcn_make_buffer_rsrc(const_cast<float*>(p.a), 0, bytes, 0x00020000);
-    const auto rsY = __builtin_amdgcn_make_buffer_rsrc(const_cast<float*>(p.b), 0, bytes, 0x00020000);
+    const int W = (p.L + 31) >> 5;
+    const auto rsY = SG ? __builtin_amdgcn_make_buffer_rsrc(p.sg, 0, 4u * (unsigned)(p.B * FC * W), 0x00020000)
+                        : __builtin_amdgcn_make_buffer_rsrc(const_cast<float*>(p.b), 0, bytes, 0x00020000);
     float acc[4] = {0.f, 0.f, 0.f, 0.f};
 #pragma unroll
     for (int cc = 0; cc < 4; ++cc) {
@@ -102,7 +124,7 @@
 #pragma unroll
         for (int i = 0; i < 5; ++i) {
             const f32x4 g = load_row4(rsG, row, t0 - 8 + 4 * i, p.L);
-            const f32x4 y = load_row4(rsY, row, t0 - 8 + 4 * i, p.L);
+            const f32x4 y = load_act4<SG>(rsY, (unsigned)(b * FC + co), W, t0 - 8 + 4 * i, p.L);
 #pragma unroll
             for (int e = 0; e < 4; ++e) win[4 * i + e] = lrelu_grad(g[e], y[e], slope);
         }
@@ -125,7 +147,15 @@
     }
 }
 
-__global__ __launch_bounds__(256) void k_dfirst_wgrad(DParts q, float slope, float* __restrict__ partial) {
+__global__ __launch_bounds__(256) void k_dfirst_bwd_data(DParts q, const float* __restrict__ w, float slope) {
+    dfirst_bwd_data_body<false>(q, w, slope);
+}
+__global__ __launch_bounds__(256) void k_dfirst_bwd_data_signs(DParts q, const float* __restrict__ w, float slope) {
+    dfirst_bwd_data_body<true>(q, w, slope);
+}
+
+template <bool SG>
+__device__ __forceinline__ void dfirst_wgrad_body(const DParts& q, float slope, float* __restrict__ partial) {
     __shared__ __attribute__((aligned(16))) float xs[FT + 16];
     const int lane = threadIdx.x & 63, wid = threadIdx.x >> 6;
     float acc[4][FK], bsum[4];
@@ -143,7 +173,9 @@
         stage_thin_window(xs, p.a, p.B, p.L, b, tile_t);
         const unsigned bytes = 4u * (unsigned)(p.B * FC * p.L);
         const auto rsG = __builtin_amdgcn_make_buffer_rsrc(const_cast<float*>(p.b), 0, bytes, 0x00020000);
-        const auto rsY = __builtin_amdgcn_make_buffer_rsrc(const_cast<float*>(p.c), 0, bytes, 0x00020000);
+        const int W = (p.L + 31) >> 5;
+        const auto rsY = SG ? __builtin_amdgcn_make_buffer_rsrc(p.sg, 0, 4u * (unsigned)(p.B * FC * W), 0x00020000)
+                            : __builtin_amdgcn_make_buffer_rsrc(const_cast<float*>(p.c), 0, bytes, 0x00020000);
 #pragma unroll 1
         for (int pass = 0; pass < FT / 256; ++pass) {
             const int sl = pass * 256 + 4 * lane, t0 = tile_t + sl;
@@ -159,7 +191,7 @@
             for (int cc = 0; cc < 4; ++cc) {
                 const unsigned row = (unsigned)((b * FC + wid * 4 + cc) * p.L);
                 g[cc] = load_row4(rsG, row, t0, p.L);
-                y[cc] = load_row4(rsY, row, t0, p.L);
+                y[cc] = load_act4<SG>(rsY, (unsigned)(b * FC + wid * 4 + cc), W, t0, p.L);
             }
 #pragma unroll
             for (int cc = 0; cc < 4; ++cc)
@@ -184,6 +216,13 @@
         const float r = ms_wave_sum(bsum[cc]);
         if (lane == 0) prow[FC * FK + co] = r;
     }
+}
+
+__global__ __launch_bounds__(256) void k_dfirst_wgrad(DParts q, float slope, float* __restrict__ partial) {
+    dfirst_wgrad_body<false>(q, slope, partial);
+}
+__global__ __launch_bounds__(256) void k_dfirst_wgrad_signs(DParts q, float slope, float* __restrict__ partial) {
+    dfirst_wgrad_body<true>(q, slope, partial);
 }
 
 __global__ __launch_bounds__(256) void k_dparts_reduce(const float* __restrict__ partial, int nslabs, int stride, int nw,
@@ -329,7 +368,7 @@
         q->B[i] = on ? parts->B[i] : 0; q->L[i] = on ? parts->Lin[i] : 1;
         q->tiles[i] = on ? (tile ? ms_ceil_div(parts->Lin[i], tile) : 1) : 1;
         q->wg0[i + 1] = q->wg0[i] + q->B[i] * q->tiles[i];
-        q->a[i] = q->b[i] = q->c[i] = nullptr; q->o[i] = nullptr;
+        q->a[i] = q->b[i] = q->c[i] = nullptr; q->o[i] = nullptr; q->sg[i] = nullptr;
     }
     return true;
 }
@@ -338,6 +377,8 @@
 constexpr int JUDGE_SLABS = 48;
 
 }
+
+bool msd_parts_take_signs(const ConvP& c) { return is_first(c); }
 
 bool msd_parts_applicable(const ConvP& c, const ms_conv1d_parts* parts, int which) {
     if (!ms_switch_on("MSYNTH_DTHIN")) return false;
@@ -364,7 +405,7 @@
     if (!table(c, parts, first ? FT : 0, first ? FC : c.Cin, &q)) return MS_ERR_INVALID_ARG;
     for (int i = 0; i < q.count; ++i) {
         if (!parts->x[i] || !parts->y[i]) return MS_ERR_INVALID_ARG;
-        q.a[i] = parts->x[i]; q.o[i] = parts->y[i];
+        q.a[i] = parts->x[i]; q.o[i] = parts->y[i]; q.sg[i] = first ? parts->y_signs[i] : nullptr;
     }
     if (first) {
         ms_note_kernel(0, "k_dfirst_fwd");
@@ -382,10 +423,14 @@
     const bool first = is_first(c);
     if (!table(c, parts, first ? 256 : 0, first ? FC : c.Cin, &q)) return MS_ERR_INVALID_ARG;
     for (int i = 0; i < q.count; ++i) {
-        if (!parts->gy[i] || !parts->gx[i] || (first && !parts->y_act[i])) return MS_ERR_INVALID_ARG;
+        if (!parts->gy[i] || !parts->gx[i] || (first && !parts->y_act[i] && !parts->y_signs[i])) return MS_ERR_INVALID_ARG;
         q.a[i] = parts->gy[i]; q.b[i] = parts->y_act[i]; q.c[i] = parts->gx_add[i]; q.o[i] = parts->gx[i];
-    }
-    if (first) {
+        q.sg[i] = first ? parts->y_signs[i] : nullptr;
+    }
+    if (first && q.sg[0]) {
+        ms_note_kernel(0, "k_dfirst_bwd_data_signs");
+        hipLaunchKernelGGL(k_dfirst_bwd_data_signs, dim3(q.wg0[q.count]), dim3(256), 0, s, q, w, c.slope);
+    } else if (first) {
         ms_note_kernel(0, "k_dfirst_bwd_data");
         hipLaunchKernelGGL(k_dfirst_bwd_data, dim3(q.wg0[q.count]), dim3(256), 0, s, q, w, c.slope);
     } else {
@@ -407,13 +452,18 @@
     float* partial = (float*)ws;
     if (first) {
         for (int i = 0; i < q.count; ++i) {
-            if (!parts->x[i] || !parts->gy[i] || !parts->y_act[i]) return MS_ERR_INVALID_ARG;
-            q.a[i] = parts->x[i]; q.b[i] = parts->gy[i]; q.c[i] = parts->y_act[i];
+            if (!parts->x[i] || !parts->gy[i] || (!parts->y_act[i] && !parts->y_signs[i])) return MS_ERR_INVALID_ARG;
+            q.a[i] = parts->x[i]; q.b[i] = parts->gy[i]; q.c[i] = parts->y_act[i]; q.sg[i] = parts->y_signs[i];
         }
         const int units = q.wg0[q.count];
         const int grid = units < FIRST_WGS ? units : FIRST_WGS;
-        ms_note_kernel(0, "k_dfirst_wgrad");
-        hipLaunchKernelGGL(k_dfirst_wgrad, dim3(grid), dim3(256), 0, s, q, c.slope, partial);
+        if (q.sg[0]) {
+            ms_note_kernel(0, "k_dfirst_wgrad_signs");
+            hipLaunchKernelGGL(k_dfirst_wgrad_signs, dim3(grid), dim3(256), 0, s, q, c.slope, partial);
+        } else {
+            ms_note_kernel(0, "k_dfirst_wgrad");
+            hipLaunchKernelGGL(k_dfirst_wgrad, dim3(grid), dim3(256), 0, s, q, c.slope, partial);
+        }
         MS_CHECK_LAUNCH();
         const int nw = FC * FK, nb = FC;
         hipLaunchKernelGGL(k_dparts_reduce, dim3(ms_ceil_div(nw + nb, 4)), dim3(256), 0, s, partial, grid, nw + nb, nw, nb, gw, gb,
diff --git a/music-synthesis_amd/csrc/gconv_mfma.h b/music-synthesis_amd/csrc/gconv_mfma.h
--- a/music-synthesis_amd/csrc/gconv_mfma.h
+++ b/music-synthesis_amd/csrc/gconv_mfma.h
@@ -41,6 +41,7 @@
 size_t msg3_parts_bwd_weight_ws(const ConvP& c, const ms_conv1d_parts* parts);
 int msg3_parts_bwd_weight(const ConvP& c, const ms_conv1d_parts* parts, float* gw, float* gb, float beta, void* ws,
                           size_t ws_bytes, hipStream_t s);
+bool msg3_parts_take_signs(const ConvP& c);
 bool ms5_parts_applicable(const ConvP& c, const ms_conv1d_parts* parts, bool backward);
 size_t ms5_parts_ws(const ConvP& c, const ms_conv1d_parts* parts, bool backward);
 int ms5_parts_fwd(const ConvP& c, const ms_conv1d_parts* parts, const void* image, const float* bias, void* ws, size_t ws_bytes,
@@ -52,6 +53,7 @@
 int msw5_parts_bwd_weight(const ConvP& c, const ms_conv1d_parts* parts, float* gw, float* gb, float beta, void* ws,
                           size_t ws_bytes, hipStream_t s);
 bool msd_parts_applicable(const ConvP& c, const ms_conv1d_parts* parts, int which);
+bool msd_parts_take_signs(const ConvP& c);
 size_t msd_parts_bwd_weight_ws(const ConvP& c, const ms_conv1d_parts* parts);
 int msd_parts_fwd(const ConvP& c, const ms_conv1d_parts* parts, const float* w, const float* bias, hipStream_t s);
 int msd_parts_bwd_data(const ConvP& c, const ms_conv1d_parts* parts, const float* w, hipStream_t s);
diff --git a/music-synthesis_amd/csrc/gconv_split.hip b/music-synthesis_amd/csrc/gconv_split.hip
--- a/music-synthesis_amd/csrc/gconv_split.hip
+++ b/music-synthesis_amd/csrc/gconv_split.hip
@@ -41,7 +41,7 @@
                                                const float* __restrict__ x,
                                                const float* __restrict__ w,
                                                const float* __restrict__ bias,
-                                               float* __restrict__ y, int bx, int nbx) {
+                                               float* __restrict__ y, uint32_t* __restrict__ sgn, int bx, int nbx) {
     using C = GF<RB>;
     unsigned char* const lds = g3_smem;
     const int tid = threadIdx.x, lane = tid & 63, wid = tid >> 6;
@@ -225,17 +225,17 @@
         else if (ets >= spr) { ets -= spr; ++eb; }
         const bool eok = ep.seg + sgl < nseg;
         const int t = ets * C::TS + 4 * np;
-        if (eok && t < p.Lout) {
-            float* yr = y + ((size_t)eb * p.Cout + (size_t)g * p.Og + kg * 4) * p.Lout + t;
-#pragma unroll
-            for (int r = 0; r < 4; ++r) {
-                if (!rok[r]) continue;
-                float v[4];
-#pragma unroll
-                for (int s = 0; s < 4; ++s) {
-                    const float pre = fmaf(acc[s][r], kscale, bq[r]);
-                    v[s] = fmaxf(pre, pre * eslope);
-                }
+        const bool lok = eok && t < p.Lout;
+        float* yr = y + ((size_t)eb * p.Cout + (size_t)g * p.Og + kg * 4) * p.Lout + t;
+#pragma unroll
+        for (int r = 0; r < 4; ++r) {
+            float v[4];
+#pragma unroll
+            for (int s = 0; s < 4; ++s) {
+                const float pre = fmaf(acc[s][r], kscale, bq[r]);
+                v[s] = fmaxf(pre, pre * eslope);
+            }
+            if (lok && rok[r]) {
                 if (VOUT) {
                     *reinterpret_cast<float4*>(yr + (size_t)r * p.Lout) = make_float4(v[0], v[1], v[2], v[3]);
                 } else if (t + 3 < p.Lout) {
@@ -244,6 +244,20 @@
 #pragma unroll
                     for (int s = 0; s < 4; ++s)
                         if (t + s < p.Lout) yr[(size_t)r * p.Lout + s] = v[s];
+                }
+            }
+            if (sgn) {
+                unsigned nib = 0;
+#pragma unroll
+                for (int s = 0; s < 4; ++s) nib |= (lok && rok[r] && t + s < p.Lout && v[s] > 0.f) ? 1u << s : 0u;
+                const unsigned part = nib << (4 * (np & 7));
+                const unsigned word = RB == 4 ? or_lanes4(part) : or_lanes8(part);
+                if (lok && rok[r] && (np & 7) == 0) {
+                    const int W = (p.Lout + 31) >> 5;
+                    uint32_t* sr = sgn + ((size_t)eb * p.Cout + (size_t)g * p.Og + kg * 4 + r) * W;
+                    if (RB != 4) sr[t >> 5] = word;
+                    else if (!(ets & 1) && ets == spr - 1) sr[ets >> 1] = word;
+                    else reinterpret_cast<uint16_t*>(sr)[ets] = (uint16_t)word;
                 }
             }
         }
@@ -276,7 +290,7 @@
                                                            const float* __restrict__ w,
                                                            const float* __restrict__ bias,
                                                            float* __restrict__ y) {
-    gconv_fwd_body<RB, VEC, VOUT>(p, spr, nseg, nunits, x, w, bias, y, blockIdx.x, gridDim.x);
+    gconv_fwd_body<RB, VEC, VOUT>(p, spr, nseg, nunits, x, w, bias, y, nullptr, blockIdx.x, gridDim.x);
 }
 
 struct G3Parts {
@@ -288,6 +302,7 @@
     const float* b[MS_CONV_PARTS_MAX];
     const float* c[MS_CONV_PARTS_MAX];
     float* o[MS_CONV_PARTS_MAX];
+    uint32_t* sg[MS_CONV_PARTS_MAX];
 };
 
 __device__ __forceinline__ int g3_part_of(const G3Parts& q, int bx) {
@@ -310,9 +325,9 @@
     const int bx = blockIdx.x, i = g3_part_of(q, bx);
     const ConvP p = g3_part_conv(q, i);
     const int rbx = bx - q.bx0[i], nbx = q.bx0[i + 1] - q.bx0[i];
-    if (i == 0) gconv_fwd_body<RB0, true, true>(p, q.u0[0], q.u1[0], q.u2[0], q.a[0], w, bias, q.o[0], rbx, nbx);
-    else if (i == 1) gconv_fwd_body<RB1, false, false>(p, q.u0[1], q.u1[1], q.u2[1], q.a[1], w, bias, q.o[1], rbx, nbx);
-    else gconv_fwd_body<RB2, false, false>(p, q.u0[2], q.u1[2], q.u2[2], q.a[2], w, bias, q.o[2], rbx, nbx);
+    if (i == 0) gconv_fwd_body<RB0, true, true>(p, q.u0[0], q.u1[0], q.u2[0], q.a[0], w, bias, q.o[0], q.sg[0], rbx, nbx);
+    else if (i == 1) gconv_fwd_body<RB1, false, false>(p, q.u0[1], q.u1[1], q.u2[1], q.a[1], w, bias, q.o[1], q.sg[1], rbx, nbx);
+    else gconv_fwd_body<RB2, false, false>(p, q.u0[2], q.u1[2], q.u2[2], q.a[2], w, bias, q.o[2], q.sg[2], rbx, nbx);
 }
 
 constexpr int WU = 64;
@@ -327,12 +342,12 @@
 template <bool VEC>
 __device__ __forceinline__ void gconv_wgrad_body(const ConvP& p, const float* __restrict__ x,
                                                  const float* __restrict__ gy,
-                                                 const float* __restrict__ y_act,
+                                                 const float* __restrict__ y_act, const uint32_t* __restrict__ sgn,
                                                  float* __restrict__ partial, size_t partial_stride, int bx, int nbx, int slab) {
     unsigned char* const lds = g3_smem;
     const int tid = threadIdx.x, lane = tid & 63, wid = tid >> 6;
     const int g = blockIdx.y;
-    const int kind = y_act ? p.act : MS_ACT_NONE;
+    const int kind = (y_act || sgn) ? p.act : MS_ACT_NONE;
     unsigned char* gimg = lds + wid * W_WAVE;
     unsigned char* ximg = gimg + WNP * WG_PIECE;
 
@@ -351,7 +366,9 @@
     const unsigned g_bytes = 4u * (unsigned)(p.B * p.Cout * p.Lout);
     const auto rsX = __builtin_amdgcn_make_buffer_rsrc(const_cast<float*>(x), 0, 4u * (unsigned)(p.B * p.Cin * p.Lin), 0x00020000);
     const auto rsG = __builtin_amdgcn_make_buffer_rsrc(const_cast<float*>(gy), 0, g_bytes, 0x00020000);
-    const auto rsA = __builtin_amdgcn_make_buffer_rsrc(const_cast<float*>(y_act ? y_act : gy), 0, g_bytes, 0x00020000);
+    const int SW = (p.Lout + 31) >> 5;
+    const auto rsA = sgn ? __builtin_amdgcn_make_buffer_rsrc(const_cast<uint32_t*>(sgn), 0, 4u * (unsigned)(p.B * p.Cout * SW), 0x00020000)
+                         : __builtin_amdgcn_make_buffer_rsrc(const_cast<float*>(y_act ? y_act : gy), 0, g_bytes, 0x00020000);
 
     const int tiles = (p.Lout + WU - 1) / WU;
     const int nunits = p.B * tiles;
@@ -362,6 +379,14 @@
 #pragma unroll
     for (int i = 0; i < 4; ++i) g_c[i] = co0 + 4 * i < p.Og ? (unsigned)((co0 + 4 * i) * p.Lout + 4 * tq) * 4u : OOB;
     f32x4 gv[4], ga[4], xv[5];
+    auto sload = [&](int b, int t0) {
+#pragma unroll
+        for (int i = 0; i < 4; ++i) {
+            const int co = co0 + 4 * i;
+            const unsigned row = (unsigned)((b * p.Cout + g * p.Og + co) * SW);
+            ga[i][0] = __builtin_bit_cast(float, co < p.Og ? load_sign_word(rsA, row, t0 + 4 * tq, p.Lout) : 0u);
+        }
+    };
     auto gload = [&](int b, int ti) {
         const int t0 = ti * WU, u0 = t0 * GS - p.pad;
         const unsigned gbase = (unsigned)((b * p.Cout + g * p.Og) * p.Lout + t0);
@@ -372,8 +397,9 @@
 #pragma unroll
             for (int i = 0; i < 4; ++i) {
                 gv[i] = __builtin_bit_cast(f32x4, __builtin_amdgcn_raw_buffer_load_b128(rsG, g_c[i], gs, 0));
-                ga[i] = __builtin_bit_cast(f32x4, __builtin_amdgcn_raw_buffer_load_b128(rsA, g_c[i], gs, 0));
-            }
+                if (!sgn) ga[i] = __builtin_bit_cast(f32x4, __builtin_amdgcn_raw_buffer_load_b128(rsA, g_c[i], gs, 0));
+            }
+            if (sgn) sload(b, t0);
 #pragma unroll
             for (int i = 0; i < 5; ++i)
                 xv[i] = __builtin_bit_cast(f32x4, __builtin_amdgcn_raw_buffer_load_b128(
@@ -388,17 +414,18 @@
                 const bool ok = co < p.Og && t0 + 4 * tq < p.Lout;
                 const unsigned vo = ok ? off * 4u : OOB;
                 gv[i] = __builtin_bit_cast(f32x4, __builtin_amdgcn_raw_buffer_load_b128(rsG, vo, 0, 0));
-                ga[i] = __builtin_bit_cast(f32x4, __builtin_amdgcn_raw_buffer_load_b128(rsA, vo, 0, 0));
+                if (!sgn) ga[i] = __builtin_bit_cast(f32x4, __builtin_amdgcn_raw_buffer_load_b128(rsA, vo, 0, 0));
             } else {
                 const bool ok = co < p.Og && t0 + 4 * tq < p.Lout;
                 const unsigned vo = ok ? off * 4u : OOB;
                 gv[i] = __builtin_bit_cast(f32x4, __builtin_amdgcn_raw_buffer_load_b128(rsG, vo, 0, 0));
-                ga[i] = __builtin_bit_cast(f32x4, __builtin_amdgcn_raw_buffer_load_b128(rsA, vo, 0, 0));
+                if (!sgn) ga[i] = __builtin_bit_cast(f32x4, __builtin_amdgcn_raw_buffer_load_b128(rsA, vo, 0, 0));
 #pragma unroll
                 for (int e = 1; e < 4; ++e)
-                    if (t0 + 4 * tq + e >= p.Lout) { gv[i][e] = 0.f; ga[i][e] = 0.f; }
-            }
-        }
+                    if (t0 + 4 * tq + e >= p.Lout) { gv[i][e] = 0.f; if (!sgn) ga[i][e] = 0.f; }
+            }
+        }
+        if (sgn) sload(b, t0);
 #pragma unroll
         for (int i = 0; i < 5; ++i) {
             const int Q4 = 4 * ((lane + 64 * i) % WXQ);
@@ -468,7 +495,10 @@
         for (int i = 0; i < 4; ++i) {
             float e[4];
 #pragma unroll
-            for (int k = 0; k < 4; ++k) e[k] = ms_act_grad(gv[i][k], ga[i][k], kind, p.slope);
+            for (int k = 0; k < 4; ++k) {
+                const float ya = sgn ? sign_as_act(__builtin_bit_cast(unsigned, ga[i][0]), 4 * (tq & 7) + k) : ga[i][k];
+                e[k] = ms_act_grad(gv[i][k], ya, kind, p.slope);
+            }
             bsum[i] += (e[0] + e[1]) + (e[2] + e[3]);
             unsigned h0, l0, h1, l1;
             split_pair(e[0] * Sg, e[1] * Sg, h0, l0);
@@ -603,15 +633,15 @@
                                                              const float* __restrict__ gy,
                                                              const float* __restrict__ y_act,
                                                              float* __restrict__ partial, size_t partial_stride) {
-    gconv_wgrad_body<VEC>(p, x, gy, y_act, partial, partial_stride, blockIdx.x, gridDim.x, blockIdx.x);
+    gconv_wgrad_body<VEC>(p, x, gy, y_act, nullptr, partial, partial_stride, blockIdx.x, gridDim.x, blockIdx.x);
 }
 
 __global__ __launch_bounds__(256, 2) void k_gconv_split_wgrad_parts(G3Parts q, float* __restrict__ partial, size_t partial_stride) {
     const int bx = blockIdx.x, i = g3_part_of(q, bx);
     const ConvP p = g3_part_conv(q, i);
     const int rbx = bx - q.bx0[i], nbx = q.bx0[i + 1] - q.bx0[i];
-    if (i == 0) gconv_wgrad_body<true>(p, q.a[0], q.b[0], q.c[0], partial, partial_stride, rbx, nbx, bx);
-    else gconv_wgrad_body<false>(p, q.a[i], q.b[i], q.c[i], partial, partial_stride, rbx, nbx, bx);
+    if (i == 0) gconv_wgrad_body<true>(p, q.a[0], q.b[0], q.c[0], q.sg[0], partial, partial_stride, rbx, nbx, bx);
+    else gconv_wgrad_body<false>(p, q.a[i], q.b[i], q.c[i], q.sg[i], partial, partial_stride, rbx, nbx, bx);
 }
 
 constexpr int BQ = 48;
@@ -624,14 +654,14 @@
 template <bool VEC, bool VOUT>
 __device__ __forceinline__ void gconv_bwd_data_body(const ConvP& p, int tiles, int nunits,
                                                     const float* __restrict__ gy,
-                                                    const float* __restrict__ y_act,
+                                                    const float* __restrict__ y_act, const uint32_t* __restrict__ sgn,
                                                     const float* __restrict__ w,
                                                     const float* __restrict__ gx_add,
                                                     float* __restrict__ gx, int bx, int nbx) {
     unsigned char* const lds = g3_smem;
     const int tid = threadIdx.x, lane = tid & 63, wid = tid >> 6;
     const int g = blockIdx.y;
-    const int kind = y_act ? p.act : MS_ACT_NONE;
+    const int kind = (y_act || sgn) ? p.act : MS_ACT_NONE;
     unsigned char* img = lds + wid * B_WAVE;
     const int n = lane & 15, kg = lane >> 4;
     const int oct = kg >> 1, tp = kg & 1;
@@ -642,7 +672,10 @@
     unsigned char* wr = img + (cq >> 1) * BOCT + (4 * pq) * 16 + (cq & 1) * 8;
     const unsigned g_bytes = 4u * (unsigned)(p.B * p.Cout * p.Lout);
     const auto rsG = __builtin_amdgcn_make_buffer_rsrc(const_cast<float*>(gy), 0, g_bytes, 0x00020000);
-    const auto rsA = __builtin_amdgcn_make_buffer_rsrc(const_cast<float*>(y_act ? y_act : gy), 0, g_bytes, 0x00020000);
+    const int SW = (p.Lout + 31) >> 5;
+    const auto rsA = sgn ? __builtin_amdgcn_make_buffer_rsrc(const_cast<uint32_t*>(sgn), 0, 4u * (unsigned)(p.B * p.Cout * SW), 0x00020000)
+                         : __builtin_amdgcn_make_buffer_rsrc(const_cast<float*>(y_act ? y_act : gy), 0, g_bytes, 0x00020000);
+    int sg_sh = 0;
     unsigned g_c[4];
 #pragma unroll
     for (int k = 0; k < 4; ++k) g_c[k] = (unsigned)((4 * cq + k) * p.Lout + 4 * pq) * 4u;
@@ -650,12 +683,19 @@
     auto gload = [&](int b, int ti) {
         const int ws = ti * BQ - 8;
         const unsigned base = (unsigned)((b * p.Cout + g * 16) * p.Lout);
+        if (sgn) {
+            const int t = ws + 4 * pq;
+            sg_sh = t & 31;
+#pragma unroll
+            for (int k = 0; k < 4; ++k)
+                ga[k][0] = __builtin_bit_cast(float, load_sign_word(rsA, (unsigned)((b * p.Cout + g * 16 + 4 * cq + k) * SW), t, p.Lout));
+        }
         if (ws >= 0 && ws + BNP <= p.Lout) {
             const unsigned sb = (unsigned)__builtin_amdgcn_readfirstlane((int)((base + (unsigned)ws) * 4u));
 #pragma unroll
             for (int k = 0; k < 4; ++k) {
                 gv[k] = __builtin_bit_cast(f32x4, __builtin_amdgcn_raw_buffer_load_b128(rsG, g_c[k], sb, 0));
-                ga[k] = __builtin_bit_cast(f32x4, __builtin_amdgcn_raw_buffer_load_b128(rsA, g_c[k], sb, 0));
+                if (!sgn) ga[k] = __builtin_bit_cast(f32x4, __builtin_amdgcn_raw_buffer_load_b128(rsA, g_c[k], sb, 0));
             }
             return;
         }
@@ -666,14 +706,14 @@
             if (VEC) {
                 const unsigned vo = (t >= 0 && t < p.Lout) ? (off + (unsigned)t) * 4u : OOB;
                 gv[k] = __builtin_bit_cast(f32x4, __builtin_amdgcn_raw_buffer_load_b128(rsG, vo, 0, 0));
-                ga[k] = __builtin_bit_cast(f32x4, __builtin_amdgcn_raw_buffer_load_b128(rsA, vo, 0, 0));
+                if (!sgn) ga[k] = __builtin_bit_cast(f32x4, __builtin_amdgcn_raw_buffer_load_b128(rsA, vo, 0, 0));
             } else {
                 const unsigned vo = (t >= 0 && t < p.Lout) ? (off + (unsigned)t) * 4u : OOB;
                 gv[k] = __builtin_bit_cast(f32x4, __builtin_amdgcn_raw_buffer_load_b128(rsG, vo, 0, 0));
-                ga[k] = __builtin_bit_cast(f32x4, __builtin_amdgcn_raw_buffer_load_b128(rsA, vo, 0, 0));
+                if (!sgn) ga[k] = __builtin_bit_cast(f32x4, __builtin_amdgcn_raw_buffer_load_b128(rsA, vo, 0, 0));
 #pragma unroll
                 for (int e = 1; e < 4; ++e)
-                    if (t + e >= p.Lout) { gv[k][e] = 0.f; ga[k][e] = 0.f; }
+                    if (t + e >= p.Lout) { gv[k][e] = 0.f; if (!sgn) ga[k][e] = 0.f; }
             }
         }
     };
@@ -728,7 +768,10 @@
         for (int j = 0; j < 4; ++j) {
             float e[4];
 #pragma unroll
-            for (int k = 0; k < 4; ++k) e[k] = ms_act_grad(gv[k][j], ga[k][j], kind, p.slope) * S;
+            for (int k = 0; k < 4; ++k) {
+                const float ya = sgn ? sign_as_act(__builtin_bit_cast(unsigned, ga[k][0]), sg_sh + j) : ga[k][j];
+                e[k] = ms_act_grad(gv[k][j], ya, kind, p.slope) * S;
+            }
             unsigned h0, l0, h1, l1;
             split_pair(e[0], e[1], h0, l0);
             split_pair(e[2], e[3], h1, l1);
@@ -826,15 +869,15 @@
                                                                 const float* __restrict__ w,
                                                                 const float* __restrict__ gx_add,
                                                                 float* __restrict__ gx) {
-    gconv_bwd_data_body<VEC, VOUT>(p, tiles, nunits, gy, y_act, w, gx_add, gx, blockIdx.x, gridDim.x);
+    gconv_bwd_data_body<VEC, VOUT>(p, tiles, nunits, gy, y_act, nullptr, w, gx_add, gx, blockIdx.x, gridDim.x);
 }
 
 __global__ __launch_bounds__(256, 2) void k_gconv_split_bwd_data_parts(G3Parts q, const float* __restrict__ w) {
     const int bx = blockIdx.x, i = g3_part_of(q, bx);
     const ConvP p = g3_part_conv(q, i);
     const int rbx = bx - q.bx0[i], nbx = q.bx0[i + 1] - q.bx0[i];
-    if (i == 0) gconv_bwd_data_body<true, true>(p, q.u0[0], q.u1[0], q.a[0], q.b[0], w, q.c[0], q.o[0], rbx, nbx);
-    else gconv_bwd_data_body<false, false>(p, q.u0[i], q.u1[i], q.a[i], q.b[i], w, q.c[i], q.o[i], rbx, nbx);
+    if (i == 0) gconv_bwd_data_body<true, true>(p, q.u0[0], q.u1[0], q.a[0], q.b[0], q.sg[0], w, q.c[0], q.o[0], rbx, nbx);
+    else gconv_bwd_data_body<false, false>(p, q.u0[i], q.u1[i], q.a[i], q.b[i], q.sg[i], w, q.c[i], q.o[i], rbx, nbx);
 }
 
 int pick_rb(int Lout) {
@@ -848,6 +891,8 @@
 }
 
 }
+
+bool msg3_parts_take_signs(const ConvP& c) { return c.act == MS_ACT_LRELU && c.Og == 16; }
 
 bool msg3_fwd_applicable(const ConvP& p) {
     return ms_switch_on("MSYNTH_GCONV3") && p.K == GK && p.stride == GS && p.Cg == GCG && p.dil == 1 && p.pad_mode == MS_PAD_ZERO &&
@@ -913,6 +958,7 @@
         q->B[i] = q->Lin[i] = q->Lout[i] = q->u0[i] = q->u1[i] = q->u2[i] = 0;
         q->a[i] = q->b[i] = q->c[i] = nullptr; q->o[i] = nullptr;
     }
+    for (int i = 0; i < MS_CONV_PARTS_MAX; ++i) q->sg[i] = nullptr;
     return true;
 }
 
@@ -949,7 +995,7 @@
         const int spr = ms_ceil_div(q.Lout[i], ts), nseg = q.B[i] * spr;
         nunits[i] = ms_ceil_div(nseg, rb[i]);
         q.u0[i] = spr; q.u1[i] = nseg; q.u2[i] = nunits[i];
-        q.a[i] = parts->x[i]; q.o[i] = parts->y[i];
+        q.a[i] = parts->x[i]; q.o[i] = parts->y[i]; q.sg[i] = parts->y_signs[i];
         total_units += (long long)nunits[i] * c.groups;
         if (g3_fwd_lds_rt(rb[i]) > lds) lds = g3_fwd_lds_rt(rb[i]);
     }
@@ -1046,6 +1092,7 @@
     for (int i = 0; i < q.count; ++i) {
         q.bx0[i + 1] = q.bx0[i] + cols[i];
         q.a[i] = parts->x[i]; q.b[i] = parts->gy[i]; q.c[i] = c.act == MS_ACT_NONE ? nullptr : parts->y_act[i];
+        q.sg[i] = parts->y_signs[i];
     }
     for (int i = q.count; i < MS_CONV_PARTS_MAX; ++i) q.bx0[i + 1] = q.bx0[q.count];
     ms_note_kernel(3, "k_gconv_split_wgrad_parts");
@@ -1107,7 +1154,7 @@
         nunits[i] = q.B[i] * tiles;
         q.u0[i] = tiles; q.u1[i] = nunits[i]; q.u2[i] = 0;
         q.a[i] = parts->gy[i]; q.b[i] = c.act == MS_ACT_NONE ? nullptr : parts->y_act[i]; q.c[i] = parts->gx_add[i];
-        q.o[i] = parts->gx[i];
+        q.o[i] = parts->gx[i]; q.sg[i] = parts->y_signs[i];
         total_units += (long long)nunits[i] * c.groups;
     }
     const int upw = (int)((total_units + 2047) / 2048);
diff --git a/music-synthesis_amd/csrc/operand_split.h b/music-synthesis_amd/csrc/operand_split.h
--- a/music-synthesis_amd/csrc/operand_split.h
+++ b/music-synthesis_amd/csrc/operand_split.h
@@ -100,4 +100,20 @@
     return v;
 }
 
+__device__ __forceinline__ unsigned load_sign_word(__amdgpu_buffer_rsrc_t rs, unsigned row_words, int t, int L) {
+    const bool any = t >= 0 && t < L;
+    return (unsigned)__builtin_amdgcn_raw_buffer_load_b32(rs, any ? (row_words + (unsigned)(t >> 5)) * 4u : OOB, 0, 0);
 }
+__device__ __forceinline__ float sign_as_act(unsigned word, int bit) { return (word >> bit) & 1u ? 1.f : 0.f; }
+__device__ __forceinline__ unsigned or_lanes4(unsigned v) {
+    v |= (unsigned)__builtin_amdgcn_update_dpp(0, (int)v, 0xB1, 0xF, 0xF, true);
+    v |= (unsigned)__builtin_amdgcn_update_dpp(0, (int)v, 0x4E, 0xF, 0xF, true);
+    return v;
+}
+__device__ __forceinline__ unsigned or_lanes8(unsigned v) {
+    v = or_lanes4(v);
+    v |= (unsigned)__builtin_amdgcn_update_dpp(0, (int)v, 0x141, 0xF, 0xF, true);
+    return v;
+}
+
+}
diff --git a/music-synthesis_amd/featuresynth/_ops/graph.py b/music-synthesis_amd/featuresynth/_ops/graph.py
--- a/music-synthesis_amd/featuresynth/_ops/graph.py
+++ b/music-synthesis_amd/featuresynth/_ops/graph.py
@@ -394,6 +394,7 @@
     return f, b, ev
 
 
+D_SIGN_LAYERS = P.W.D_SIGN_LAYERS
 D_HEAD_PARAM = 10
 
 
@@ -460,16 +461,18 @@
         w, b = params[2 * li], params[2 * li + 1]
         ds = [P.conv_desc(h.shape, w.shape, stride=stride, pad=pad, groups=groups, act=L.ACT_LRELU)[0] for h in hs]
         img = k5_image if (li == 5 and k5_image is not None and P.conv_img_bytes(ds[0])) else None
-        ys = P.conv1d_parts_fwd(hs, w, b, ds[0], image=img)
+        want = P.DSIGNS and li < D_SIGN_LAYERS
+        out = P.conv1d_parts_fwd(hs, w, b, ds[0], image=img, want_signs=want)
+        ys, sgs = out if want else (out, None)
         for s in range(n):
-            tapes[s].append((ds[s], hs[s], ys[s]))
+            tapes[s].append((ds[s], hs[s], ys[s], None if sgs is None else sgs[s]))
             feats[s].append(ys[s])
         hs = ys
     w, b = params[12], params[13]
     djs = [P.conv_desc(h.shape, w.shape, pad=1)[0] for h in hs]
     js = P.conv1d_parts_fwd(hs, w, b, djs[0])
     for s in range(n):
-        tapes[s].append((djs[s], hs[s], js[s]))
+        tapes[s].append((djs[s], hs[s], js[s], None))
     return feats, js, (tapes, xs)
 
 
@@ -487,14 +490,15 @@
     fork = _WgradFork(xs[0].device) if (need_wgrad and mode != "0") else None
     fork2 = _WgradFork(xs[0].device, 1) if (fork is not None and mode == "2" and cut is None) else None
 
-    def wgrad(slot, live, xs_, gys, yas, d, w_shape):
+    def wgrad(slot, live, xs_, gys, yas, d, w_shape, sgs=None):
         gw, gb, acc = sink.pair(slot)
         a, b_, c = [xs_[s] for s in live], [gys[s] for s in live], (None if yas is None else [yas[s] for s in live])
+        sg = None if sgs is None else [sgs[s] for s in live]
 
         def go():
-            sink.put(slot, *P.conv1d_parts_bwd_weight(a, b_, c, d, w_shape, gw, gb, acc))
+            sink.put(slot, *P.conv1d_parts_bwd_weight(a, b_, c, d, w_shape, gw, gb, acc, y_signs=sg))
         if fork is not None:
-            (fork2 if (fork2 is not None and slot < D_HEAD_PARAM) else fork).run(go, *(a + b_ + (c or [])))
+            (fork2 if (fork2 is not None and slot < D_HEAD_PARAM) else fork).run(go, *(a + b_ + (c or []) + (sg or [])))
         else:
             go()
 
@@ -519,12 +523,14 @@
             d = tapes[live[0]][li][0]
             hin = [tapes[s][li][1] for s in range(n)]
             h = [tapes[s][li][2] for s in range(n)]
+            sg = [tapes[s][li][3] for s in range(n)]
             if need_wgrad:
-                wgrad(2 * li, live, hin, g, h, d, params[2 * li].shape)
+                wgrad(2 * li, live, hin, g, h, d, params[2 * li].shape, sg)
             if li > 0 or need_gx:
                 img = k5_bwd if (li == 5 and k5_bwd is not None and P.conv_img_bytes(d)) else None
                 outs = P.conv1d_parts_bwd_data([g[s] for s in live], [h[s] for s in live], params[2 * li], d,
-                                               [hin[s].shape for s in live], gx_adds=[prev[s] for s in live], image_bwd=img)
+                                               [hin[s].shape for s in live], gx_adds=[prev[s] for s in live], image_bwd=img,
+                                               y_signs=[sg[s] for s in live])
                 for s, o in zip(live, outs):
                     g[s] = o
             else:
diff --git a/music-synthesis_amd/featuresynth/_ops/lib.py b/music-synthesis_amd/featuresynth/_ops/lib.py
--- a/music-synthesis_amd/featuresynth/_ops/lib.py
+++ b/music-synthesis_amd/featuresynth/_ops/lib.py
@@ -53,7 +53,8 @@
 class ConvParts(ctypes.Structure):
     _fields_ = [("count", _c_int), ("reserved", _c_int), ("B", _c_int * CONV_PARTS_MAX), ("Lin", _c_int * CONV_PARTS_MAX),
                 ("x", _vp * CONV_PARTS_MAX), ("y", _vp * CONV_PARTS_MAX), ("gy", _vp * CONV_PARTS_MAX),
-                ("y_act", _vp * CONV_PARTS_MAX), ("gx_add", _vp * CONV_PARTS_MAX), ("gx", _vp * CONV_PARTS_MAX)]
+                ("y_act", _vp * CONV_PARTS_MAX), ("gx_add", _vp * CONV_PARTS_MAX), ("gx", _vp * CONV_PARTS_MAX),
+                ("y_signs", _vp * CONV_PARTS_MAX)]
 
 
 WGRAD_MULTI_MAX = 8
@@ -246,6 +247,10 @@
     "ms_band_recompose_bwd": (_c_int, [_vp, _c_int, _c_int, ctypes.POINTER(BandDesc), _vp, _sz, _vp]),
 }
 
+DSIGNS_SIGNATURES = {
+    "ms_conv1d_parts_signs_supported": (_c_int, [ctypes.POINTER(ConvDesc), ctypes.POINTER(ConvParts), _c_int]),
+}
+
 _LIB = None
 
 
@@ -258,7 +263,7 @@
                 "`make -C music-synthesis_amd/csrc` or __graft_entry__.build(). There is no CPU "
                 "or PyTorch fallback for the hot path." % LIB_PATH)
         lib = ctypes.CDLL(LIB_PATH)
-        for name, (res, args) in list(SIGNATURES.items()) + list(BAND_SIGNATURES.items()):
+        for name, (res, args) in list(SIGNATURES.items()) + list(BAND_SIGNATURES.items()) + list(DSIGNS_SIGNATURES.items()):
             fn = getattr(lib, name)
             fn.restype = res
             fn.argtypes = args
diff --git a/music-synthesis_amd/featuresynth/_ops/prims.py b/music-synthesis_amd/featuresynth/_ops/prims.py
--- a/music-synthesis_amd/featuresynth/_ops/prims.py
+++ b/music-synthesis_amd/featuresynth/_ops/prims.py
@@ -174,7 +174,37 @@
     return cost
 
 
-def conv1d_parts_fwd(xs, w, b, d, image=None):
+DSIGNS = W.DSIGNS
+
+_SIGNS_OK = {}
+
+
+def parts_signs_ok(d, parts, which):
+    n = parts.count
+    al = tuple(bool((getattr(parts, f)[i] or 0) % 16 == 0) for f in ("x", "y", "gy", "y_act", "gx_add", "gx") for i in range(n))
+    key = (which, d.Cin, d.Cout, d.K, d.stride, d.pad, d.dil, d.groups, d.act, d.in_act,
+           tuple(parts.B[i] for i in range(n)), tuple(parts.Lin[i] for i in range(n)), al)
+    if key not in _SIGNS_OK:
+        _SIGNS_OK[key] = bool(L.load().ms_conv1d_parts_signs_supported(d, parts, _WHICH[which]))
+    return _SIGNS_OK[key]
+
+
+def sign_words(rows, length, device):
+    return torch.empty((rows, (length + 31) // 32), dtype=torch.int32, device=device)
+
+
+def _use_signs(d, parts, which, y_signs, gys):
+    if y_signs is None or any(s is None for s in y_signs) or d.act == L.ACT_NONE or not parts_signs_ok(d, parts, which):
+        return False
+    for i, (s, gy) in enumerate(zip(y_signs, gys)):
+        if not (isinstance(s, torch.Tensor) and s.is_cuda and s.is_contiguous() and s.dtype == torch.int32 and s.dim() == 2 and
+                s.shape[0] >= gy.shape[0] * d.Cout and s.shape[1] == (gy.shape[2] + 31) // 32):
+            raise RuntimeError("conv1d_parts: sign words of part %d do not cover gradient %s" % (i, tuple(gy.shape)))
+        parts.y_signs[i] = s.data_ptr()
+    return True
+
+
+def conv1d_parts_fwd(xs, w, b, d, image=None, want_signs=False):
     if not 1 <= len(xs) <= L.CONV_PARTS_MAX:
         raise RuntimeError("conv1d_parts: 1 .. %d parts" % L.CONV_PARTS_MAX)
     L.require(w, "conv1d weight")
@@ -195,14 +225,19 @@
         parts.B[i], parts.Lin[i], parts.x[i], parts.y[i] = B, Lin, x.data_ptr(), y.data_ptr()
         ys.append(y); shapes.append((B, Lin))
     lib = L.load()
+    sgs = None
+    if want_signs and image is None and d.act != L.ACT_NONE and parts_signs_ok(d, parts, "fwd"):
+        sgs = [sign_words(y.shape[0] * y.shape[1], y.shape[2], y.device) for y in ys]
+        for i, sg in enumerate(sgs):
+            parts.y_signs[i] = sg.data_ptr()
     nws = lib.ms_conv1d_parts_workspace_bytes(d, parts, 0, 1 if image is not None else 0)
     ws = L.workspace(nws, xs[0].device)
-    L.call("ms_conv1d_parts_fwd", _parts_cost(d, shapes, "fwd", "fwd"), d, parts, w.data_ptr(), L.ptr(b), L.ptr(image),
-           L.ptr(ws), nws, L.stream())
-    return ys
-
-
-def conv1d_parts_bwd_data(gys, y_acts, w, d, in_shapes, gx_adds=None, image_bwd=None):
+    L.call("ms_conv1d_parts_fwd", _parts_cost(d, shapes, "fwd", "fwd", signs=sgs is not None), d, parts, w.data_ptr(), L.ptr(b),
+           L.ptr(image), L.ptr(ws), nws, L.stream())
+    return (ys, sgs) if want_signs else ys
+
+
+def conv1d_parts_bwd_data(gys, y_acts, w, d, in_shapes, gx_adds=None, image_bwd=None, y_signs=None):
     n = len(gys)
     parts = L.ConvParts()
     parts.count = n
@@ -225,15 +260,16 @@
         parts.gy[i], parts.y_act[i], parts.gx_add[i], parts.gx[i] = gy.data_ptr(), L.ptr(ya), L.ptr(ga), gx.data_ptr()
         gxs.append(gx); shapes.append((B, Lin))
     lib = L.load()
+    sg = image_bwd is None and _use_signs(d, parts, "bwd_data", y_signs, gys)
     nws = lib.ms_conv1d_parts_workspace_bytes(d, parts, 1, 1 if image_bwd is not None else 0)
     ws = L.workspace(nws, gys[0].device)
-    L.call("ms_conv1d_parts_bwd_data", _parts_cost(d, shapes, "bwd_data", "bwd_data", act_read=d.act != L.ACT_NONE,
+    L.call("ms_conv1d_parts_bwd_data", _parts_cost(d, shapes, "bwd_data", "bwd_data", act_read=d.act != L.ACT_NONE, signs=sg,
                                                    extra_reads=int(gx_adds is not None and any(g is not None for g in gx_adds))),
            d, parts, w.data_ptr(), L.ptr(image_bwd), L.ptr(ws), nws, L.stream())
     return gxs
 
 
-def conv1d_parts_bwd_weight(xs, gys, y_acts, d, w_shape, gw=None, gb=None, accumulate=False):
+def conv1d_parts_bwd_weight(xs, gys, y_acts, d, w_shape, gw=None, gb=None, accumulate=False, y_signs=None):
     n = len(gys)
     dev_ = gys[0].device
     if gw is None:
@@ -256,9 +292,10 @@
         parts.x[i], parts.gy[i], parts.y_act[i] = x.data_ptr(), gy.data_ptr(), L.ptr(ya)
         shapes.append((B, Lin))
     lib = L.load()
+    sg = _use_signs(d, parts, "bwd_weight", y_signs, gys)
     nws = lib.ms_conv1d_parts_workspace_bytes(d, parts, 2, 0)
     ws = L.workspace(nws, dev_)
-    L.call("ms_conv1d_parts_bwd_weight", _parts_cost(d, shapes, "bwd_weight", "bwd_weight", act_read=d.act != L.ACT_NONE),
+    L.call("ms_conv1d_parts_bwd_weight", _parts_cost(d, shapes, "bwd_weight", "bwd_weight", act_read=d.act != L.ACT_NONE, signs=sg),
            d, parts, gw.data_ptr(), gb.data_ptr(), 1.0 if accumulate else 0.0, L.ptr(ws), nws, L.stream())
     return gw, gb
 
diff --git a/music-synthesis_amd/featuresynth/_workload.py b/music-synthesis_amd/featuresynth/_workload.py
--- a/music-synthesis_amd/featuresynth/_workload.py
+++ b/music-synthesis_amd/featuresynth/_workload.py
@@ -1,3 +1,4 @@
+import os
 
 G_UPS = ((512, 256, 16, 8, 4), (256, 128, 16, 8, 4), (128, 64, 4, 2, 1), (64, 32, 4, 2, 1))
 D_MAIN = ((1, 16, 15, 1, 7, 1), (16, 64, 41, 4, 20, 4), (64, 256, 41, 4, 20, 16),
@@ -10,16 +11,18 @@
 
 
 def conv_cost(B, Cin, Lin, Cout, K, stride, pad, dil, groups, which, extra_reads=0, extra_writes=0,
-              act_read=False):
+              act_read=False, signs=False):
     Lout = conv_out_len(Lin, K, stride, pad, dil)
     macs = B * Cout * Lout * (Cin // groups) * K
     nin, nout, nw = B * Cin * Lin, B * Cout * Lout, Cout * (Cin // groups) * K + Cout
+    nsg = B * Cout * ((Lout + 31) // 32) if signs else 0
+    nact = nsg if signs else (nout if act_read else 0)
     if which == "fwd":
-        elems = nin + nout + nw + (extra_reads + extra_writes) * nout
+        elems = nin + nout + nw + (extra_reads + extra_writes) * nout + nsg
     elif which == "bwd_data":
-        elems = nout + (nout if act_read else 0) + nin + nw + extra_reads * nin
-    else:
-        elems = nin + nout + (nout if act_read else 0) + nw
+        elems = nout + nact + nin + nw + extra_reads * nin
+    else:
+        elems = nin + nout + nact + nw
     return {"flops": 2 * macs, "bytes": F32 * elems}
 
 
@@ -74,7 +77,10 @@
     return out
 
 
-def discriminator_launches(B, L0, mode, need_gx=False, feat_grads=False):
+D_SIGN_LAYERS = 4
+
+
+def discriminator_launches(B, L0, mode, need_gx=False, feat_grads=False, signs=False):
     out = []
     L = L0
     for s in range(3):
@@ -90,7 +96,7 @@
         judge = dict(B=B, Cin=1024, Lin=l, Cout=1, K=3, stride=1, pad=1, dil=1, groups=1)
         if mode == "fwd":
             for i, c in enumerate(geo):
-                out.append(("d.main%d.fwd" % i, conv_cost(which="fwd", **c)))
+                out.append(("d.main%d.fwd" % i, conv_cost(which="fwd", signs=signs and i < D_SIGN_LAYERS, **c)))
             out.append(("d.judge.fwd", conv_cost(which="fwd", **judge)))
         else:
             out.append(("d.judge.bwd_data", conv_cost(which="bwd_data", extra_reads=int(feat_grads), **judge)))
@@ -99,12 +105,12 @@
                     pass
                 if i > 0 or need_gx:
                     out.append(("d.main%d.bwd_data" % i,
-                                conv_cost(which="bwd_data", act_read=True,
+                                conv_cost(which="bwd_data", act_read=True, signs=signs and i < D_SIGN_LAYERS,
                                           extra_reads=int(feat_grads and i > 0), **geo[i])))
     return out
 
 
-def discriminator_wgrad_launches(B, L0):
+def discriminator_wgrad_launches(B, L0, signs=False):
     out = []
     L = L0
     for s in range(3):
@@ -113,7 +119,8 @@
         l = L
         for i, (cin, cout, k, st, p, g) in enumerate(D_MAIN):
             out.append(("d.main%d.bwd_weight" % i,
-                        conv_cost(B, cin, l, cout, k, st, p, 1, g, "bwd_weight", act_read=True)))
+                        conv_cost(B, cin, l, cout, k, st, p, 1, g, "bwd_weight", act_read=True,
+                                  signs=signs and i < D_SIGN_LAYERS)))
             l = conv_out_len(l, k, st, p)
         out.append(("d.judge.bwd_weight", conv_cost(B, 1024, l, 1, 3, 1, 1, 1, 1, "bwd_weight")))
     return out
@@ -160,6 +167,7 @@
 
 
 SIGN_WORDS = 1.0 / 32
+DSIGNS = os.environ.get("MSYNTH_DSIGNS", "1") != "0"
 STACK_FUSED_MAX_C = 64
 
 
@@ -200,9 +208,9 @@
 def fused_d_step_launches(B, mels=80, T=32):
     L0 = T * 256
     out = fused_generator_launches(B, mels, T, "fwd")
-    out += discriminator_launches(2 * B, L0, "fwd")
-    out += discriminator_launches(2 * B, L0, "bwd", need_gx=False)
-    out += discriminator_wgrad_launches(2 * B, L0)
+    out += discriminator_launches(2 * B, L0, "fwd", signs=DSIGNS)
+    out += discriminator_launches(2 * B, L0, "bwd", need_gx=False, signs=DSIGNS)
+    out += discriminator_wgrad_launches(2 * B, L0, signs=DSIGNS)
     nparam = 5637953
     out.append(("adam.D", {"flops": 12 * nparam, "bytes": 7 * F32 * nparam}))
     return out
@@ -211,11 +219,11 @@
 def fused_g_step_launches(B, mels=80, T=32):
     L0 = T * 256
     out = fused_generator_launches(B, mels, T, "fwd_train")
-    out += discriminator_launches(B, L0, "fwd")
-    out += discriminator_launches(B, L0, "fwd")
+    out += discriminator_launches(B, L0, "fwd", signs=DSIGNS)
+    out += discriminator_launches(B, L0, "fwd", signs=DSIGNS)
     fe = feature_elems(B, L0)
     out.append(("loss.l1.fwd_bwd", {"flops": 5 * fe, "bytes": 3 * F32 * fe}))
-    out += discriminator_launches(B, L0, "bwd", need_gx=True, feat_grads=True)
+    out += discriminator_launches(B, L0, "bwd", need_gx=True, feat_grads=True, signs=DSIGNS)
     out += fused_generator_launches(B, mels, T, "bwd")
     nparam = 4519937 + (mels - 80) * 512 * 7
     out.append(("adam.G", {"flops": 12 * nparam, "bytes": 7 * F32 * nparam}))
```

After: 104.0 million samples/s. About the same (-0.8%).
